# erikliland/pyMHT

Hardware: AMD Instinct MI355X
Metric: scans/sec at ~5k+ leaf hypotheses x 500 measurements (per-scan gate + cluster + ILP + N-scan prune) (higher is better)
Workload: dtype f64 state / f32 covariance (the reference's own mix); 1 GPU; BASELINE configs[2]: 500 targets, ~500 meas/scan, N-scan=5, P_d=0.9, eta2=5.99; one independent sector per GPU; targets=499, n_scan=5, ilps_branched=63, blp_dual_iters_max=8, pre_roll_scans=16

## Files before the change

pymht_amd/csrc/mht_blp.hip:

```cpp
#include "mht_kernels.h"
#include "mht_commit.h"
#include <stdlib.h>

namespace mht {

#ifndef MHT_BLP_THREADS
#define MHT_BLP_THREADS 256
#endif
constexpr int BLP_THREADS = MHT_BLP_THREADS;
constexpr int FUSED_K = 8;
constexpr double DINF = 1.0e300;
constexpr int BIG_MAXH = 2048, BIG_MAXR = 1024, BIG_MAXK = 256;

struct Red {
    double d[BLP_THREADS / 64];
    double q[BLP_THREADS / 64][4];
    int i[BLP_THREADS / 64];
};

template <int CTRL, int ROW_MASK> __device__ __forceinline__ double dpp_f64(double v) {
    int lo = __double2loint(v), hi = __double2hiint(v);
    lo = __builtin_amdgcn_update_dpp(0, lo, CTRL, ROW_MASK, 0xf, false);
    hi = __builtin_amdgcn_update_dpp(0, hi, CTRL, ROW_MASK, 0xf, false);
    return __hiloint2double(hi, lo);
}
__device__ __forceinline__ double wave_sum(double v) {
    v += dpp_f64<0x111, 0xf>(v);
    v += dpp_f64<0x112, 0xf>(v);
    v += dpp_f64<0x114, 0xf>(v);
    v += dpp_f64<0x118, 0xf>(v);
    v += dpp_f64<0x142, 0xa>(v);
    v += dpp_f64<0x143, 0xc>(v);
    return __hiloint2double(__builtin_amdgcn_readlane(__double2hiint(v), 63), __builtin_amdgcn_readlane(__double2loint(v), 63));
}

__device__ __forceinline__ double block_sum(double v, Red* r) {
    v = wave_sum(v);
    __syncthreads();
    if ((threadIdx.x & 63) == 0) r->d[threadIdx.x >> 6] = v;
    __syncthreads();
    double s = 0.0;
#pragma unroll
    for (int w = 0; w < BLP_THREADS / 64; ++w) s += r->d[w];
    return s;
}
__device__ __forceinline__ int block_or(int v, Red* r) {
    v = __any(v) ? 1 : 0;
    __syncthreads();
    if ((threadIdx.x & 63) == 0) r->i[threadIdx.x >> 6] = v;
    __syncthreads();
    int s = 0;
#pragma unroll
    for (int w = 0; w < BLP_THREADS / 64; ++w) s |= r->i[w];
    return s;
}
template <int CTRL, int ROW_MASK> __device__ __forceinline__ void dpp_min_value(double& v) {
    const int lo = __double2loint(v), hi = __double2hiint(v);
    const int nlo = __builtin_amdgcn_update_dpp(lo, lo, CTRL, ROW_MASK, 0xf, false);
    const int nhi = __builtin_amdgcn_update_dpp(hi, hi, CTRL, ROW_MASK, 0xf, false);
    v = fmin(v, __hiloint2double(nhi, nlo));
}
__device__ __forceinline__ double row16_min_value(double v) {
    dpp_min_value<0x111, 0xf>(v);
    dpp_min_value<0x112, 0xf>(v);
    dpp_min_value<0x114, 0xf>(v);
    dpp_min_value<0x118, 0xf>(v);
    return v;
}
__device__ __forceinline__ double wave_min_value(double v) {
    v = row16_min_value(v);
    dpp_min_value<0x142, 0xa>(v);
    dpp_min_value<0x143, 0xc>(v);
    return __hiloint2double(__builtin_amdgcn_readlane(__double2hiint(v), 63), __builtin_amdgcn_readlane(__double2loint(v), 63));
}
template <int CTRL, int ROW_MASK> __device__ __forceinline__ void dpp_min_pair(double& v, int& i) {
    const int lo = __double2loint(v), hi = __double2hiint(v);
    const int nlo = __builtin_amdgcn_update_dpp(lo, lo, CTRL, ROW_MASK, 0xf, false);
    const int nhi = __builtin_amdgcn_update_dpp(hi, hi, CTRL, ROW_MASK, 0xf, false);
    const int ni = __builtin_amdgcn_update_dpp(i, i, CTRL, ROW_MASK, 0xf, false);
    const double nv = __hiloint2double(nhi, nlo);
    if (ni >= 0 && (i < 0 || nv < v || (nv == v && ni < i))) { v = nv; i = ni; }
}
__device__ __forceinline__ void row16_min_pair(double& v, int& i) {
    dpp_min_pair<0x111, 0xf>(v, i);
    dpp_min_pair<0x112, 0xf>(v, i);
    dpp_min_pair<0x114, 0xf>(v, i);
    dpp_min_pair<0x118, 0xf>(v, i);
}
__device__ __forceinline__ void wave_min_pair(double& v, int& i) {
    row16_min_pair(v, i);
    dpp_min_pair<0x142, 0xa>(v, i);
    dpp_min_pair<0x143, 0xc>(v, i);
    const int hi = __builtin_amdgcn_readlane(__double2hiint(v), 63), lo = __builtin_amdgcn_readlane(__double2loint(v), 63);
    v = __hiloint2double(hi, lo);
    i = __builtin_amdgcn_readlane(i, 63);
}
__device__ __forceinline__ void block_min_pair(double& v, int& i, Red* r) {
    wave_min_pair(v, i);
    __syncthreads();
    if ((threadIdx.x & 63) == 0) { r->d[threadIdx.x >> 6] = v; r->i[threadIdx.x >> 6] = i; }
    __syncthreads();
    v = r->d[0];
    i = r->i[0];
#pragma unroll
    for (int w = 1; w < BLP_THREADS / 64; ++w) {
        const double ov = r->d[w];
        const int oi = r->i[w];
        if (oi >= 0 && (i < 0 || ov < v || (ov == v && oi < i))) { v = ov; i = oi; }
    }
}

#ifndef MHT_GS_CK
#define MHT_GS_CK 1
#endif
struct GStore {
    const BlpArgs* a; const int32_t* mem; const unsigned long long* uw; int UW, PD; size_t cap;
    double* pu; int32_t* pusage; int32_t* pmark;
    int32_t *best_h, *ub_sel, *ch, *lix; double *best_rc, *cst, *uus, *lrc, *rest, *mn;
    bool ck; const int32_t *cbL, *ceL;
    __device__ __forceinline__ int row(int m) const { return m; }
    __device__ __forceinline__ int col_begin(int k) const { return (MHT_GS_CK && ck) ? cbL[k] : a->tchild[mem[k]]; }
    __device__ __forceinline__ int col_end(int k) const { return (MHT_GS_CK && ck) ? ceL[k] : a->tcend[mem[k]]; }
    __device__ __forceinline__ double cost(int h) const { return a->cost[h]; }
    __device__ __forceinline__ int ent(int d, int h) const { return a->pds ? a->path[(size_t)h * a->pds + d] : a->path[(size_t)d * cap + h]; }
    __device__ __forceinline__ double& u(int m) const { return pu[row(m)]; }
    __device__ __forceinline__ int32_t& usage(int m) const { return pusage[row(m)]; }
    __device__ __forceinline__ int32_t& mark(int m) const { return pmark[row(m)]; }
    __device__ __forceinline__ int to_global(int h) const { return h; }
    static constexpr int FOR_ROWS_FLAT = 256;
    template <typename F> __device__ __forceinline__ void for_rows(F f) const {
        if (UW <= FOR_ROWS_FLAT) {
            for (int m = threadIdx.x; m < UW * 64; m += BLP_THREADS)
                if ((uw[m >> 6] >> (m & 63)) & 1ull) f(m);
            return;
        }
        for (int w = threadIdx.x; w < UW; w += BLP_THREADS) {
            unsigned long long bits = uw[w];
            while (bits) {
                const int m = w * 64 + __ffsll((long long)bits) - 1;
                bits &= bits - 1;
                f(m);
            }
        }
    }
};
struct EnumEnt;
struct LStore {
    double* costL; unsigned short* entL; double* uL; int32_t* usageL; int32_t* markL; int32_t* colb; int32_t* gbase;
    int32_t* gcolL;
    bool reduced;
    double* rcL; unsigned short* membL; unsigned long long* minkey;
    unsigned short* ordL;
    unsigned short* enumL;
    EnumEnt* xL;
    int nH, nR, PD, K;
    int32_t *best_h, *ub_sel, *ch, *lix; double *best_rc, *cst, *uus, *lrc, *rest, *mn;
    __device__ __forceinline__ int col_begin(int k) const { return colb[k]; }
    __device__ __forceinline__ int col_end(int k) const { return colb[k + 1]; }
    __device__ __forceinline__ double cost(int h) const { return costL[h]; }
    __device__ __forceinline__ int ent(int d, int h) const { const int e = entL[h * 8 + d]; return e == nR ? -1 : e; }
    __device__ __forceinline__ double& u(int m) const { return uL[m]; }
    __device__ __forceinline__ int32_t& usage(int m) const { return usageL[m]; }
    __device__ __forceinline__ int32_t& mark(int m) const { return markL[m]; }
    __device__ __forceinline__ int to_global(int h) const {
        if (reduced) return gcolL[h];
        int lo = 0, hi = K;
        while (hi - lo > 1) { const int mid = (lo + hi) >> 1; if (colb[mid] <= h) lo = mid; else hi = mid; }
        return gbase[lo] + (h - colb[lo]);
    }
    template <typename F> __device__ __forceinline__ void for_rows(F f) const {
        for (int m = threadIdx.x; m < nR; m += BLP_THREADS) f(m);
    }
};

#ifndef MHT_ROWS8
#define MHT_ROWS8 1
#endif
__device__ __forceinline__ void rows8(const GStore& s, int h, int (&e)[8]) {
    if (s.a->pds == 8) {
        const int4* p = reinterpret_cast<const int4*>(s.a->path + (size_t)h * 8);
        const int4 q0 = p[0], q1 = p[1];
        e[0] = q0.x; e[1] = q0.y; e[2] = q0.z; e[3] = q0.w; e[4] = q1.x; e[5] = q1.y; e[6] = q1.z; e[7] = q1.w;
    } else {
#pragma unroll
        for (int d = 0; d < 8; ++d) e[d] = (d < s.PD) ? s.ent(d, h) : -1;
    }
}
__device__ __forceinline__ double reduced_cost(const GStore& s, int h) {
    double rc = s.cost(h);
    if (s.PD <= 8 && MHT_ROWS8) {
        int e[8];
        rows8(s, h, e);
        double uv[8];
#pragma unroll
        for (int d = 0; d < 8; ++d) uv[d] = s.u(e[d] >= 0 ? e[d] : 0);
#pragma unroll
        for (int d = 0; d < 8; ++d) rc = (e[d] >= 0) ? rc + uv[d] : rc;
        return rc;
    }
    for (int d = 0; d < s.PD; ++d) {
        const int e = s.ent(d, h);
        if (e >= 0) rc += s.u(e);
    }
    return rc;
}
__device__ __forceinline__ bool compatible(const GStore& s, int h) {
    if (s.PD <= 8 && MHT_ROWS8) {
        int e[8];
        rows8(s, h, e);
        int bad = 0;
#pragma unroll
        for (int d = 0; d < 8; ++d) bad |= (e[d] >= 0) ? s.mark(e[d] >= 0 ? e[d] : 0) : 0;
        return bad == 0;
    }
    for (int d = 0; d < s.PD; ++d) {
        const int e = s.ent(d, h);
        if (e >= 0 && s.mark(e)) return false;
    }
    return true;
}
__device__ __forceinline__ void set_marks(const GStore& s, int h, int value) {
    if ((int)threadIdx.x < s.PD) {
        const int e = s.ent(threadIdx.x, h);
        if (e >= 0) s.mark(e) = value;
    }
    __threadfence_block();
    __syncthreads();
}
__device__ __forceinline__ double priced_part(const GStore& s, int h) {
    if ((int)threadIdx.x < s.PD) {
        const int e = s.ent(threadIdx.x, h);
        if (e >= 0) return s.u(e);
    }
    return 0.0;
}
__device__ __forceinline__ void add_usage(const GStore& s, int k, int d) {
    const int e = s.ent(d, s.best_h[k]);
    if (e >= 0) atomicAdd(&s.usage(e), 1);
}

struct Rows8 { unsigned short e[8]; };
__device__ __forceinline__ Rows8 rows_of(const LStore& s, int h) {
    const uint4 v = reinterpret_cast<const uint4*>(s.entL)[h];
    Rows8 r;
    r.e[0] = v.x & 0xffff; r.e[1] = v.x >> 16; r.e[2] = v.y & 0xffff; r.e[3] = v.y >> 16;
    r.e[4] = v.z & 0xffff; r.e[5] = v.z >> 16; r.e[6] = v.w & 0xffff; r.e[7] = v.w >> 16;
    return r;
}
__device__ __forceinline__ double reduced_cost(const LStore& s, int h) {
    const Rows8 r = rows_of(s, h);
    const double c = s.costL[h];
    const double u0 = s.uL[r.e[0]], u1 = s.uL[r.e[1]], u2 = s.uL[r.e[2]], u3 = s.uL[r.e[3]];
    const double u4 = s.uL[r.e[4]], u5 = s.uL[r.e[5]], u6 = s.uL[r.e[6]], u7 = s.uL[r.e[7]];
    return ((((((((c + u0) + u1) + u2) + u3) + u4) + u5) + u6) + u7);
}
__device__ __forceinline__ bool compatible(const LStore& s, int h) {
    const Rows8 r = rows_of(s, h);
    const int m = s.markL[r.e[0]] | s.markL[r.e[1]] | s.markL[r.e[2]] | s.markL[r.e[3]] | s.markL[r.e[4]] | s.markL[r.e[5]] |
                  s.markL[r.e[6]] | s.markL[r.e[7]];
    return m == 0;
}
__device__ __forceinline__ void set_marks(const LStore& s, int h, int value) {
    if (threadIdx.x < 8) {
// ... 597 lines not shown
                unsigned long long fsig = 0ull;
                while (i < he) {
                    const int idx = i + lane;
                    const bool valid = idx < he;
                    const EnumEnt en = xL[valid ? idx : he - 1];
                    const bool over = !valid || (arc + en.rc + tail > lim);
                    const bool feas = !over && !(en.sig & mask);
                    const unsigned long long mo = __ballot(over);
                    unsigned long long mf = __ballot(feas);
                    if (mo) mf &= (1ull << (__ffsll((long long)mo) - 1)) - 1ull;
                    if (mf) {
                        const int fl = __ffsll((long long)mf) - 1;
                        found = i + fl;
                        frc = __shfl(en.rc, fl);
                        fsig = __shfl(en.sig, fl);
                        break;
                    }
                    if (mo) break;
                    i += 64;
                }
                if (found >= 0) {
                    if (++nodes > ENUM_BUDGET) { if (lane == 0) *s_abort = 1; break; }
                    const double tot = acc + s.costL[s.ordL[found]];
                    if (lane == 0) s_pos[L * ENUM_W + wave] = found;
                    if (L == K - 1) {
                        record(tot, L);
                        i = found + 1;
                        continue;
                    }
                    mask |= fsig;
                    acc = tot;
                    arc = arc + frc;
                    ++L;
                    i = s.colb[s_order[L]];
                    continue;
                }
                --L;
                if (L < 1) break;
                i = s_pos[L * ENUM_W + wave] + 1;
                mask = f0.sig;
                acc = tot0;
                arc = f0.rc;
                for (int q = 1; q < L; ++q) {
                    const int pq = s_pos[q * ENUM_W + wave];
                    const EnumEnt en = xL[pq];
                    mask |= en.sig;
                    acc = acc + s.costL[s.ordL[pq]];
                    arc = arc + en.rc;
                }
            }
        }
        if (lane == 0) { s_bestc[wave] = best; s_nodes[wave] = nodes; }
    }
    __syncthreads();
    ok = ok && !*s_abort;
    if (ok) {
        int w = -1;
        for (int q = 0; q < ENUM_W; ++q) {
            if (!(s_bestc[q] < DINF)) continue;
            bool better = w < 0 || s_bestc[q] < s_bestc[w];
            if (!better && s_bestc[q] == s_bestc[w]) {
                int d = 0;
                for (int l = 0; l < K && d == 0; ++l) d = s_best[l * ENUM_W + q] - s_best[l * ENUM_W + w];
                better = d < 0;
            }
            if (better) w = q;
        }
        ok = w >= 0;
        if (ok) {
            for (int l = tid; l < K; l += BLP_THREADS) s.ub_sel[s_order[l]] = s_best[l * ENUM_W + w];
            int tn = 0;
            for (int q = 0; q < ENUM_W; ++q) tn += s_nodes[q];
            nodes_out = tn;
            ub_known = s_bestc[w];
        }
    }
    for (int m = tid; m < nR; m += BLP_THREADS) { s.usageL[m] = 0; s.markL[m] = 0; }
    __threadfence_block();
    __syncthreads();
    return ok;
}

constexpr int MHT_BLP_REDUCE = -2;
__device__ __forceinline__ bool reducible(const BlpArgs&, const LStore&, int, double, Red*) { return false; }
__device__ __forceinline__ bool reducible(const BlpArgs& a, const GStore& s, int K, double UB, Red* r) {
    if (a.force_hbm || a.no_reduce || K > a.cap_k || a.PD > 8 || !(UB < DINF)) return false;
    const int tid = threadIdx.x;
    compute_minimisers(s, K, r);
    double up = 0.0, rs = 0.0;
    s.for_rows([&](int m) { up += s.u(m); });
    for (int k = tid; k < K; k += BLP_THREADS) rs += s.best_rc[k];
    const double root = block_sum(rs, r) - block_sum(up, r);
    const double lim = UB + 1e-9 * fmax(1.0, fabs(UB));
    int total = 0;
    for (int k = 0; k < K; ++k) {
        const double thr = lim - root + s.best_rc[k];
        double c = 0.0;
        for (int h = s.col_begin(k) + tid; h < s.col_end(k); h += BLP_THREADS) c += (reduced_cost(s, h) <= thr) ? 1.0 : 0.0;
        const int ck = (int)block_sum(c, r);
        if (tid == 0) { s.mn[k] = thr; s.lix[k] = ck; }
        total += ck;
        if (total > a.cap_h) return false;
    }
    for (int k = 0; k < K; ++k) {
        const double thr = lim - root + s.best_rc[k];
        for (int h = s.col_begin(k) + tid; h < s.col_end(k); h += BLP_THREADS)
            if (reduced_cost(s, h) <= thr)
                for (int d = 0; d < s.PD; ++d) { const int e = s.ent(d, h); if (e >= 0) s.mark(e) = 1; }
    }
    __threadfence_block();
    __syncthreads();
    double nr = 0.0;
    s.for_rows([&](int m) { nr += s.mark(m) ? 1.0 : 0.0; s.mark(m) = 0; });
    const int rows = (int)block_sum(nr, r);
    __threadfence_block();
    __syncthreads();
    return rows < a.cap_r - 1;
}

struct Team {
    int q, W; unsigned long long* gub;
    int qg, Wg;
    __device__ Team(int q_, int W_, unsigned long long* g_) : q(q_), W(W_), gub(g_), qg(q_), Wg(W_) {}
    __device__ Team(int q_, int W_, unsigned long long* g_, int qg_, int Wg_) : q(q_), W(W_), gub(g_), qg(qg_), Wg(Wg_) {}
};
#ifndef MHT_TEAM_LEVEL
#define MHT_TEAM_LEVEL 5
#endif
constexpr int TEAM_LEVEL = MHT_TEAM_LEVEL;
#ifndef MHT_TEAM_LEVEL_HBM
#define MHT_TEAM_LEVEL_HBM 3
#endif
__device__ __forceinline__ constexpr int team_level(const LStore&) { return TEAM_LEVEL; }
__device__ __forceinline__ constexpr int team_level(const GStore&) { return MHT_TEAM_LEVEL_HBM; }
__device__ __forceinline__ unsigned team_hash(int c0, int c1) {
    unsigned h = (unsigned)c0 * 0x9E3779B1u ^ ((unsigned)c1 * 0x85EBCA6Bu + 0x7F4A7C15u);
    h ^= h >> 15; h *= 0x2C1B3C6Du; h ^= h >> 12;
    return h;
}
template <typename S> __device__ __forceinline__ void solve_core(const BlpArgs& a, const S& s, int K, Red* r, int& status, int& iters, int& nodes, unsigned long long* stamp,
                                                                 double& ub, const Team tm = Team(0, 1, nullptr)) {
    const int tid = threadIdx.x, lane = tid & 63, wave = tid >> 6;
    double& UB = ub;
    double best_LB = -DINF, theta = 1.0, utot = 0.0;
    int stall = 0;
    status = 0; iters = 0; nodes = 0;
    const int ca_rounds = coordinate_rounds(s, K);
    const int ca_end = a.max_iter < ca_rounds ? a.max_iter : ca_rounds;
    const int it_cap = bb_after_rounds(s, K) ? ca_end : a.max_iter;
    const int enum_after = (s.col_end(K - 1) - s.col_begin(0) > ENUM_WIDE) ? ENUM_AFTER_WIDE : ENUM_AFTER;
    const int enum_at = (ca_end > 0 && K >= 3 && K <= ENUM_MAXK) ? (ca_end < enum_after ? ca_end : enum_after) : -1;
    for (int it = 0; it <= it_cap; ++it) {
        iters = it;
        if (it == enum_at && !a.no_enum) {
            const unsigned long long e0 = wall_clock64();
            const bool solved = enumerate_small(s, K, r, nodes, stamp, UB);
            stamp[5] = wall_clock64() - e0;
            if (solved) { status = MHT_BLP_BRANCHED; return; }
        }
        if (it == ca_end && ca_end > 0 && !bb_after_rounds(s, K)) {
            s.for_rows([&](int m) { s.u(m) = 0.0; });
            __threadfence_block();
            __syncthreads();
        }
        if ((it == 24 || it == 64 || it == 128) && UB < DINF && reducible(a, s, K, UB, r)) { status = MHT_BLP_REDUCE; return; }
        compute_minimisers(s, K, r);
        if (it == 0) stamp[1] = wall_clock64();
        if (!usage_counted_by_minimisers(s, K)) {
            for (int idx = tid; idx < K * s.PD; idx += BLP_THREADS) {
                const int k = idx / s.PD, d = idx - k * s.PD;
                add_usage(s, k, d);
            }
            __threadfence_block();
            __syncthreads();
        }
        if (it == 0) stamp[2] = wall_clock64();
        const bool coord = it < ca_end;
        double nrm = 0.0, usum = 0.0, LB = 0.0;
        int conflict = 0, slack = 0;
        if (coord) {
            s.for_rows([&](int m) {
                const int us = s.usage(m);
                conflict |= (us >= 2);
                slack |= (s.u(m) > 0.0 && us == 0);
            });
            nominate(s, K);
            const int f = (__any(conflict) ? 1 : 0) | (__any(slack) ? 2 : 0);
            if (lane == 0) r->i[wave] = f;
            __threadfence_block();
            __syncthreads();
            int ff = 0;
#pragma unroll
            for (int w = 0; w < BLP_THREADS / 64; ++w) ff |= r->i[w];
            conflict = ff & 1;
            slack = (ff >> 1) & 1;
            if (it == 0) stamp[3] = wall_clock64();
            if (!conflict) {
                bool take = true;
                if (UB < DINF) {
                    double sc = 0.0;
                    for (int k = tid; k < K; k += BLP_THREADS) sc += s.cost(s.best_h[k]);
                    sc = block_sum(sc, r);
                    take = sc < UB;
                    if (take) UB = sc;
                }
                if (take)
                    for (int k = tid; k < K; k += BLP_THREADS) s.ub_sel[k] = s.best_h[k];
                __threadfence_block();
                __syncthreads();
            }
        } else {
            s.for_rows([&](int m) {
                const int us = s.usage(m);
                const double um = s.u(m);
                double g = (double)(us - 1);
                if (um <= 0.0 && g < 0.0) g = 0.0;
                nrm += g * g;
                usum += um;
                conflict |= (us >= 2);
                slack |= (um > 0.0 && us == 0);
            });
            double src = 0.0, sc = 0.0;
            for (int k = tid; k < K; k += BLP_THREADS) { src += s.best_rc[k]; sc += s.cost(s.best_h[k]); }
            {
                const double v0 = wave_sum(nrm), v1 = wave_sum(usum), v2 = wave_sum(src), v3 = wave_sum(sc);
                int f = (__any(conflict) ? 1 : 0) | (__any(slack) ? 2 : 0);
                __syncthreads();
                if (lane == 0) { r->q[wave][0] = v0; r->q[wave][1] = v1; r->q[wave][2] = v2; r->q[wave][3] = v3; r->i[wave] = f; }
                __syncthreads();
                nrm = 0.0; utot = 0.0; src = 0.0; sc = 0.0; f = 0;
#pragma unroll
                for (int w = 0; w < BLP_THREADS / 64; ++w) {
                    nrm += r->q[w][0]; utot += r->q[w][1]; src += r->q[w][2]; sc += r->q[w][3]; f |= r->i[w];
                }
                conflict = f & 1;
                slack = (f >> 1) & 1;
            }
            if (it == 0) stamp[3] = wall_clock64();
            LB = src - utot;
            if (!conflict && sc < UB) {
                UB = sc;
                for (int k = tid; k < K; k += BLP_THREADS) s.ub_sel[k] = s.best_h[k];
                __threadfence_block();
                __syncthreads();
            }
        }
        bool done = false;
        if (!conflict && !slack) { status = MHT_BLP_CERTIFIED; done = true; }
        if (!done && coord && it == 1 && K == 2 && enumerate_pair(s, r)) {
            status = MHT_BLP_CERTIFIED;
            break;
        }
        bool counters_reset = false;
        if (!done && coord) counters_reset = coordinate_step(s, K, conflict != 0, slack != 0);
        if (!done && !coord) {
            if (LB > best_LB + 1e-12) { best_LB = LB; stall = 0; }
            else if (++stall >= 10) { theta *= 0.5; stall = 0; }
            if (UB >= DINF || (conflict && (it % 4) == 0)) {
                const double g = greedy_dive(s, K, s.ch, r);
                if (g < UB) {
                    UB = g;
                    for (int k = tid; k < K; k += BLP_THREADS) s.ub_sel[k] = s.ch[k];
                    __threadfence_block();
                    __syncthreads();
                }
            }
            if (UB - best_LB <= 1e-12 * fmax(1.0, fabs(UB))) { status = MHT_BLP_CERTIFIED; done = true; }
            if (it == it_cap || nrm == 0.0) done = true;
            if (theta < 1.0 / 16.0) done = true;
        }
        if (done && status != 0 && scratch_is_private(s)) break;
        const double step = (done || coord) ? 0.0 : theta * fmax(UB - LB, 1e-6) / nrm;
        if (!counters_reset)
            s.for_rows([&](int m) {
                if (!done && !coord) {
                    const double um = s.u(m);
                    double g = (double)(s.usage(m) - 1);
                    if (um <= 0.0 && g < 0.0) g = 0.0;
                    s.u(m) = fmax(0.0, um + step * g);
                }
                s.usage(m) = 0;
                if (coord) s.mark(m) = 0;
            });
        __threadfence_block();
        __syncthreads();
        if (done) break;
    }
#ifdef MHT_BLP_TRACE
    if (tid == 0 && tm.q == 0) printf("[blp] dual phase: %d iterations, status %d, at %.2f ms\n", iters, status, 1e-5 * (double)(wall_clock64() - stamp[0]));
#endif
    if (status != 0) return;
    if (UB >= DINF) {
        UB = greedy_dive(s, K, s.ch, r);
        for (int k = tid; k < K; k += BLP_THREADS) s.ub_sel[k] = s.ch[k];
        __threadfence_block();
        __syncthreads();
    }
    if (reducible(a, s, K, UB, r)) { status = MHT_BLP_REDUCE; return; }
    int32_t* ord = reinterpret_cast<int32_t*>(s.best_rc);
    int32_t* bh = s.best_h;
    {
        compute_minimisers(s, K, r);
        if (!usage_counted_by_minimisers(s, K)) {
            for (int idx = tid; idx < K * s.PD; idx += BLP_THREADS) add_usage(s, idx / s.PD, idx % s.PD);
            __threadfence_block();
            __syncthreads();
        }
        for (int k = tid; k < K; k += BLP_THREADS) {
            int hot = 0;
            const int h = s.best_h[k];
            for (int d = 0; d < s.PD; ++d) {
                const int e = s.ent(d, h);
                if (e >= 0 && (s.usage(e) >= 2 || s.u(e) > 0.0)) ++hot;
            }
            s.lix[k] = hot;
        }
        __threadfence_block();
        __syncthreads();
        for (int k = tid; k < K; k += BLP_THREADS) {
            const int hk = s.lix[k];
            int rank = 0;
            for (int j = 0; j < K; ++j) { const int hj = s.lix[j]; rank += (hj > hk || (hj == hk && j < k)) ? 1 : 0; }
            ord[rank] = k;
        }
        s.for_rows([&](int m) { s.usage(m) = 0; });
        __threadfence_block();
        __syncthreads();
    }
    int slot = -1;
    if (a.bb_snap && a.bb_busy) {
        if (tid == 0) {
            int got = -1;
            for (int i = 0; i < BB_SLOTS && got < 0; ++i)
                if (atomicCAS(&a.bb_busy[i], 0, 1) == 0) got = i;
            r->i[0] = got;
        }
        __syncthreads();
        slot = r->i[0];
        __syncthreads();
    }
    double* snap = slot >= 0 ? a.bb_snap + (size_t)slot * BB_RE_LEVELS * a.bb_snap_rows : nullptr;
    if (tid == 0) s.cst[0] = 0.0;
    __threadfence_block();
    __syncthreads();
    int level = 0;
    bool enter = true;
#ifdef MHT_BLP_TRACE
    int tr_eval = 0, tr_upper = 0;
    unsigned long long tr_t[8] = {0, 0, 0, 0, 0, 0, 0, 0}, tr_q = 0, tr_n = wall_clock64();
#define TR_MARK(i) do { const unsigned long long _n = wall_clock64(); tr_t[i] += _n - tr_q; tr_q = _n; } while (0)
#else
#define TR_MARK(i) do {} while (0)
#endif
    status = MHT_BLP_BRANCHED;
    double own = UB;
    const bool team = tm.Wg > 1 && tm.gub != nullptr;
    if (team && tid == 0 && UB < DINF) atomicMin(tm.gub, enum_key(UB));
    while (true) {
        if (team && enter && level >= 1) {
            __syncthreads();
            if (tid == 0) r->q[0][0] = enum_val(__hip_atomic_load(tm.gub, __ATOMIC_RELAXED, __HIP_MEMORY_SCOPE_AGENT));
            __syncthreads();
            const double g = r->q[0][0];
            __syncthreads();
            if (g < UB) UB = g;
        }
        const double eps = 1e-12 * fmax(1.0, fabs(UB));
        if (enter) {
            if (++nodes > a.node_limit) { status = MHT_BLP_NODE_LIMIT; break; }
            if (a.time_limit > 0 && (nodes & 63) == 0 && block_or(wall_clock64() - stamp[0] > (unsigned long long)a.time_limit ? 1 : 0, r)) {
                status = MHT_BLP_NODE_LIMIT;
                break;
            }
            if (level == K) {
                if (s.cst[K] < UB - eps) {
                    UB = own = s.cst[K];
                    if (team && tid == 0) atomicMin(tm.gub, enum_key(UB));
                    for (int p = tid; p < K; p += BLP_THREADS) s.ub_sel[ord[p]] = s.ch[p];
                    __threadfence_block();
                    __syncthreads();
                }
// ... 106 lines not shown
                    const double step = step_on ? fmax(UB - lb, 1e-6) / nrm : 0.0;
                    s.for_rows([&](int m) {
                        if (redo) {
                            s.u(m) = sl[m];
                        } else if (!s.mark(m) && step_on) {
                            const double um = s.u(m);
                            double g = (double)(s.usage(m) - 1);
                            if (um <= 0.0 && g < 0.0) g = 0.0;
                            s.u(m) = fmax(0.0, um + step * g);
                        }
                        s.usage(m) = 0;
                    });
                    __threadfence_block();
                    __syncthreads();
                }
                TR_MARK(5);
#ifdef MHT_BLP_TRACE
                tr_n = wall_clock64();
#endif
                if (redo) { final_eval = true; continue; }
                if (stop || !step_on) break;
            }
            if (pruned) {
                if (level == 0) break;
                --level;
                set_marks(s, s.ch[level], 0);
                enter = false;
                continue;
            }
            if (tid == 0) { s.rest[level] = rs_all - s.mn[level]; s.uus[level] = usumU; s.lrc[level] = -DINF; s.lix[level] = -1; }
            __threadfence_block();
            __syncthreads();
            enter = false;
        } else if (snap && level + 1 < BB_RE_LEVELS) {
            const double* slr = snap + (size_t)level * a.bb_snap_rows;
            s.for_rows([&](int m) { s.u(m) = slr[m]; });
            __threadfence_block();
            __syncthreads();
        }
        double bv;
        int bi;
        argmin_member(s, ord[level], true, s.lrc[level], s.lix[level], bv, bi, r);
        if (bi < 0 || s.cst[level] + bv + s.rest[level] - s.uus[level] >= UB - eps) {
            if (level == 0) break;
            --level;
            set_marks(s, s.ch[level], 0);
            continue;
        }
        bool foreign = false;
        if (team && level == team_level(s)) {
            unsigned hsh = 0x9E3779B9u;
            for (int l = 0; l < team_level(s); ++l) hsh = team_hash((int)hsh, s.to_global(s.ch[l]));
            hsh = team_hash((int)hsh, s.to_global(bi));
            foreign = hsh % (unsigned)tm.Wg != (unsigned)tm.qg;
        }
        if (foreign) {
            __syncthreads();
            if (tid == 0) { s.lrc[level] = bv; s.lix[level] = bi; }
            __threadfence_block();
            __syncthreads();
            continue;
        }
        if (tid == 0) {
            s.lrc[level] = bv;
            s.lix[level] = bi;
            s.ch[level] = bi;
            s.cst[level + 1] = s.cst[level] + s.cost(bi);
        }
        set_marks(s, bi, 1);
        ++level;
        enter = true;
    }
#ifdef MHT_BLP_TRACE
    if (tid == 0 && team) printf("[blp] member %d of %d: %d nodes (%d at or above the deal-out level), %d evaluations, left at %.2f ms; us per evaluation: sweep %.1f sums %.1f usage %.1f rows %.1f keep %.1f step %.1f outside %.1f\n", tm.q, tm.W, nodes, tr_upper, tr_eval,
                                 1e-5 * (double)(wall_clock64() - stamp[0]), 1e-2 * tr_t[0] / tr_eval, 1e-2 * tr_t[1] / tr_eval, 1e-2 * tr_t[2] / tr_eval, 1e-2 * tr_t[3] / tr_eval,
                                 1e-2 * tr_t[4] / tr_eval, 1e-2 * tr_t[5] / tr_eval, 1e-2 * tr_t[6] / tr_eval);
#endif
    ub = own;
    for (int l = 0; l < level; ++l) set_marks(s, s.ch[l], 0);
    if (slot >= 0 && tid == 0) atomicExch(&a.bb_busy[slot], 0);
}

struct TgtPre { int j, rscan, rnode, id, lab, cb, ce; double rootc; uint8_t rootf; };
__device__ __forceinline__ TgtPre load_target(const BlpArgs& a, int t) {
    TgtPre p;
    const int dg = a.t_depth[t] + 1, w = a.t_window[t] & 0xff;
    p.j = dg > w ? dg - w : 0;
    p.rscan = a.t_root_scan[t]; p.rnode = a.t_root_node[t]; p.id = a.t_id[t]; p.lab = a.t_label[t];
    p.cb = a.tchild[t]; p.ce = a.tcend[t];
    p.rootc = a.t_root_cnllr[t]; p.rootf = a.t_root_f32[t];
    return p;
}
template <typename T> __device__ __forceinline__ const T* ring_ptr(const T* base0, size_t stride, int k) {
    return reinterpret_cast<const T*>(reinterpret_cast<const char*>(base0) + (size_t)k * stride);
}
constexpr int KEY_DEAD = -1, KEY_ALL = -2;
__device__ __forceinline__ void blp_publish(const BlpArgs& a, int t, int key, int j, int rf, int count, int first) {
    if (!a.rec0) return;
    asm volatile("s_waitcnt vmcnt(0)" ::: "memory");
    __hip_atomic_store(&a.rec0[t], tgt_rec(a.pub_scan, key != -1, rf, j, count, count > 0 ? first : 0), __ATOMIC_RELAXED, __HIP_MEMORY_SCOPE_AGENT);
}
__device__ __forceinline__ int finish_target(const BlpArgs& a, int t, int s, const TgtPre& p, bool store, int* rf_out = nullptr) {
    const int kc = a.kc;
    const double cn = a.cnllr[s];
    const uint8_t fl = a.flags[s];
    const int smeas = ring_ptr(a.ring0.meas, a.ring_stride, kc)[s];
    double sx[NX];
#pragma unroll
    for (int k = 0; k < NX; ++k) sx[k] = a.x[(size_t)k * a.cap + s];
    const double sx0 = sx[0], sx1 = sx[1];
    const int j = p.j;
    const int anc_l = a.apath[(size_t)s * a.pds + (j > 0 ? j - 1 : 0)];
    const int anc = (j > 0) ? anc_l : -1;
    const bool f32score = (fl & F_SCORE_F32) && p.rootf;
    const double score = f32score ? (double)((float)cn - (float)p.rootc) : cn - p.rootc;
    int status = 0;
    if (isfinite(a.radar_range)) {
        const double dx = sx0 - a.radar_x, dy = sx1 - a.radar_y;
        if (sqrt(dx * dx + dy * dy) > a.radar_range) status = 1;
    }
    if (!status) {
        const double per = f32score ? (double)((float)score / (float)(a.Nwin + 1)) : score / (double)(a.Nwin + 1);
        if (per > a.score_limit) status = 2;
        else if (cn > a.cnllr_limit) status = 3;
    }
    int rscan = p.rscan, rnode = p.rnode;
    const bool moved = status == 0 && j > 0;
    if (moved) { rscan += j; rnode = anc; }
    const int kr = rscan % a.R;
    const double* rx = ring_ptr(a.ring0.x, a.ring_stride, kr);
    const double rc_l = ring_ptr(a.ring0.cnllr, a.ring_stride, kr)[rnode];
    const uint8_t rf_l = ring_ptr(a.ring0.flags, a.ring_stride, kr)[rnode];
    double rxv[NX];
#pragma unroll
    for (int k = 0; k < NX; ++k) rxv[k] = rx[(size_t)k * a.cap + rnode];
    const int rmeas = ring_ptr(a.ring0.meas, a.ring_stride, kr)[rnode];
    const double rc = moved ? rc_l : p.rootc;
    const uint8_t rf = moved ? (uint8_t)((rf_l & F_SCORE_F32) ? 1 : 0) : p.rootf;
    if (store) {
        a.t_alive[t] = status;
        a.t_jdrop[t] = j;
        a.t_score[t] = score;
        a.w_root_scan[t] = rscan; a.w_root_node[t] = rnode; a.w_root_f32[t] = rf;
        if (a.rec0) __hip_atomic_store(reinterpret_cast<unsigned long long*>(&a.w_root_cnllr[t]), (unsigned long long)__double_as_longlong(rc), __ATOMIC_RELAXED, __HIP_MEMORY_SCOPE_AGENT);
        else a.w_root_cnllr[t] = rc;
        mht_target_report& r = a.rec[t];
        r.id = p.id;
        r.status = status;
        r.sel_node = s;
        r.sel_meas = smeas;
        r.root_scan = rscan;
        r.root_node = rnode;
#pragma unroll
        for (int k = 0; k < NX; ++k) r.sel_x[k] = sx[k];
        r.sel_cnllr = cn;
        r.score = score;
        r.root_cnllr = rc;
#pragma unroll
        for (int k = 0; k < NX; ++k) r.root_x[k] = rxv[k];
        r.root_meas = rmeas;
        r.cluster = p.lab;
    }
    if (rf_out) *rf_out = rf;
    return status ? KEY_DEAD : (j > 0 ? anc : KEY_ALL);
}

__device__ __forceinline__ int sweep_prefetch(const BlpArgs& a, int j, int cb, int ce, int lane) {
    return (j > 0 && cb + lane < ce) ? a.apath[(size_t)(cb + lane) * a.pds + (j - 1)] : -1;
}
__device__ __forceinline__ void sweep_survivors(const BlpArgs& a, int t, int j, int cb, int ce, int key, int va0, int lane, int rf = -1) {
    int count = 0, first = 0x7fffffff;
    if (key == KEY_ALL) {
        count = ce - cb;
        if (count > 0) first = cb;
    } else if (key != KEY_DEAD) {
        for (int c0 = cb; c0 < ce; c0 += 64) {
            const int c = c0 + lane;
            const int v = (c0 == cb) ? va0 : (c < ce ? a.apath[(size_t)c * a.pds + (j - 1)] : -1);
            const unsigned long long m = __ballot(c < ce && v == key);
            if (m && first == 0x7fffffff) first = c0 + __ffsll((long long)m) - 1;
            count += __popcll(m);
        }
    }
    if (lane == 0) {
        a.t_count[t] = count; a.t_firstsurv[t] = first;
        if (a.rec0) blp_publish(a, t, key, j, rf >= 0 ? rf : (int)a.w_root_f32[t], count, first);
    }
}

__device__ __forceinline__ void prune_members(const BlpArgs& a, const int32_t* mem, int K, const int32_t* key) {
    if (!a.t_alive) return;
    __threadfence_block();
    __syncthreads();
    const int lane = threadIdx.x & 63;
    for (int k = threadIdx.x >> 6; k < K; k += BLP_THREADS / 64) {
        const int t = mem[k];
        const int j = a.t_jdrop[t], cb = a.tchild[t], ce = a.tcend[t];
        sweep_survivors(a, t, j, cb, ce, key[k], sweep_prefetch(a, j, cb, ce, lane), lane);
    }
}

struct ClRef { int c, p0, K, root; };
__device__ __forceinline__ ClRef cl_ref(const BlpArgs& a, int c) { const int p0 = a.cl_ptr[c]; return ClRef{c, p0, a.cl_ptr[c + 1] - p0, -1}; }
__device__ __forceinline__ TgtPre load_target_cr(const BlpArgs& a, int t, const ClRef& cr) {
    TgtPre p = load_target(a, t);
    if (a.uf_epoch) p.lab = cr.root;
    return p;
}
__device__ __forceinline__ void solve_cluster(const BlpArgs& a, const ClRef cr, unsigned long long* uw, Red* r, unsigned char* lds,
                                              const Team tm = Team(0, 1, nullptr), const int team_idx = -1, const int my_t = -1, const TgtPre* pre_in = nullptr, const int dbg_bx = -1) {
    const int tid = threadIdx.x;
    const int c = cr.c;
    const int K = cr.K;
    const int32_t* mem = a.cl_members + cr.p0;
    const int slot = cr.p0 + c;
    const int UW = (a.n_mnodes + 63) >> 6;
    const unsigned long long t_begin = wall_clock64();
    const unsigned long long c_begin = clock64();
    TgtPre pre = {};
    const bool pre_ok = a.t_alive && K <= BLP_THREADS;
    if (pre_ok && tid < K) { if (pre_in && my_t >= 0) pre = *pre_in; else pre = load_target_cr(a, my_t >= 0 ? my_t : mem[tid], cr); }
    LStore s;
    unsigned char* q = lds;
    const int L_MAXH = a.cap_h, L_MAXR = a.cap_r, L_MAXK = a.cap_k, L_KPAD = a.cap_k + 4;
    int* s_wbase = reinterpret_cast<int*>(q); q += (size_t)a.cap_uw * 4;
    int* s_scal = reinterpret_cast<int*>(q); q += 16;
    int& s_nR = s_scal[0];
    int& s_nH = s_scal[1];
    s.entL = reinterpret_cast<unsigned short*>(q); q += (size_t)L_MAXH * 16;
    s.costL = reinterpret_cast<double*>(q); q += (size_t)L_MAXH * 8;
    s.rcL = reinterpret_cast<double*>(q); q += (size_t)L_MAXH * 8;
    s.uL = reinterpret_cast<double*>(q); q += (size_t)L_MAXR * 8;
    s.minkey = reinterpret_cast<unsigned long long*>(q); q += (size_t)L_KPAD * 8;
    s.best_rc = reinterpret_cast<double*>(q); q += (size_t)L_KPAD * 8;
    s.cst = reinterpret_cast<double*>(q); q += (size_t)L_KPAD * 8;
    s.uus = reinterpret_cast<double*>(q); q += (size_t)L_KPAD * 8;
    s.lrc = reinterpret_cast<double*>(q); q += (size_t)L_KPAD * 8;
    s.rest = reinterpret_cast<double*>(q); q += (size_t)L_KPAD * 8;
    s.mn = reinterpret_cast<double*>(q); q += (size_t)L_KPAD * 8;
    s.usageL = reinterpret_cast<int32_t*>(q); q += (size_t)L_MAXR * 4;
    s.markL = reinterpret_cast<int32_t*>(q); q += (size_t)L_MAXR * 4;
    s.colb = reinterpret_cast<int32_t*>(q); q += (size_t)L_KPAD * 4;
    s.gbase = reinterpret_cast<int32_t*>(q); q += (size_t)L_KPAD * 4;
    s.best_h = reinterpret_cast<int32_t*>(q); q += (size_t)L_KPAD * 4;
    s.ub_sel = reinterpret_cast<int32_t*>(q); q += (size_t)L_KPAD * 4;
    s.ch = reinterpret_cast<int32_t*>(q); q += (size_t)L_KPAD * 4;
    s.lix = reinterpret_cast<int32_t*>(q); q += (size_t)L_KPAD * 4;
    s.membL = reinterpret_cast<unsigned short*>(q); q += (size_t)L_MAXH * 2;
    s.ordL = reinterpret_cast<unsigned short*>(q); q += (size_t)L_MAXH * 2;
    s.enumL = reinterpret_cast<unsigned short*>(q); q += ENUM_LDS;
    s.xL = reinterpret_cast<EnumEnt*>(q); q += (size_t)L_MAXH * 16;
    s.gcolL = reinterpret_cast<int32_t*>(q); q += (size_t)L_MAXH * 4;
    s.reduced = false;
    const bool small_k = K <= L_MAXK;
    for (int w = tid; w < UW; w += BLP_THREADS) uw[w] = 0ull;
    if (small_k) {
        if (tid < 64) {
            int carry = 0;
            for (int base = 0; base < K; base += 64) {
                const int k = base + tid;
                int gb = 0, n = 0;
                if (k < K) {
                    if (pre_ok && K <= 64) { gb = pre.cb; n = pre.ce - gb; }
                    else { const int t = mem[k]; gb = a.tchild[t]; n = a.tcend[t] - gb; }
                }
                int incl = n;
#pragma unroll
                for (int o = 1; o < 64; o <<= 1) {
                    const int v = __shfl_up(incl, o);
                    if (tid >= o) incl += v;
                }
                if (k < K) { s.colb[k] = carry + incl - n; s.gbase[k] = gb; if (pre_ok && K <= 64) s.lix[k] = pre.j; }
                carry += __shfl(incl, 63);
            }
            if (tid == 0) { s.colb[K] = carry; s_nH = carry; }
        }
    } else if (tid == 0) {
        int acc = 0;
        for (int k = 0; k < K; ++k) acc += a.tcend[mem[k]] - a.tchild[mem[k]];
        s_nH = acc;
    }
    __syncthreads();
    const int nH = s_nH;
    if (a.tier == 1 && !(K <= a.t1_k && nH <= a.t1_h)) {
        if (tid == 0) a.big_list[atomicAdd(a.big_count, 1)] = c;
        __syncthreads();
        return;
    }
    const bool lds_cols = small_k && nH <= L_MAXH && a.PD <= 8 && !a.force_hbm;
    const bool anc_pf = lds_cols && pre_ok && K <= 64 && a.t_alive && a.pds == 8;
    s.nH = nH; s.PD = a.PD; s.K = K;
    if (lds_cols) {
        for (int h0 = tid; h0 < nH; h0 += 2 * BLP_THREADS) {
            int g[2], ev[2][8], jm[2], an[2];
            double cs[2];
#pragma unroll
            for (int q = 0; q < 2; ++q) {
                const int h = h0 + q * BLP_THREADS;
                g[q] = -1; jm[q] = 0;
                if (h < nH) {
                    int lo = 0, hi = K;
                    while (hi - lo > 1) { const int mid = (lo + hi) >> 1; if (s.colb[mid] <= h) lo = mid; else hi = mid; }
                    g[q] = s.gbase[lo] + (h - s.colb[lo]);
                    s.membL[h] = (unsigned short)lo;
                    if (anc_pf) jm[q] = s.lix[lo];
                }
            }
#pragma unroll
            for (int q = 0; q < 2; ++q) {
                const int gq = g[q] >= 0 ? g[q] : 0;
                cs[q] = a.cost[gq];
                an[q] = -1;
                if (anc_pf) an[q] = a.apath[(size_t)gq * 8 + (jm[q] > 0 ? jm[q] - 1 : 0)];
                if (a.pds) {
                    const int4* rec = reinterpret_cast<const int4*>(a.path + (size_t)gq * a.pds);
                    const int4 r0 = rec[0], r1 = rec[1];
                    const int rv[8] = {r0.x, r0.y, r0.z, r0.w, r1.x, r1.y, r1.z, r1.w};
#pragma unroll
                    for (int d = 0; d < 8; ++d) ev[q][d] = g[q] >= 0 ? rv[d] : -1;
                } else {
#pragma unroll
                    for (int d = 0; d < 8; ++d) {
                        const int v = (d < a.PD) ? a.path[(size_t)d * a.cap + gq] : -1;
                        ev[q][d] = g[q] >= 0 ? v : -1;
                    }
                }
            }
#pragma unroll
            for (int q = 0; q < 2; ++q) {
                const int h = h0 + q * BLP_THREADS;
                if (g[q] < 0) continue;
                s.costL[h] = cs[q];
                if (anc_pf) s.gcolL[h] = an[q];
#pragma unroll
                for (int d = 0; d < 8; ++d) {
                    s.entL[h * 8 + d] = (unsigned short)(ev[q][d] < 0 ? 0xffff : ev[q][d]);
                    if (ev[q][d] >= 0) atomicOr(&uw[ev[q][d] >> 6], 1ull << (ev[q][d] & 63));
                }
            }
        }
    } else {
        for (int k = 0; k < K; ++k) {
            const int t = mem[k];
            for (int d = 0; d < a.PD; ++d)
                for (int h = a.tchild[t] + tid; h < a.tcend[t]; h += BLP_THREADS) {
                    const int e = a.pds ? a.path[(size_t)h * a.pds + d] : a.path[(size_t)d * a.cap + h];
                    if (e >= 0) atomicOr(&uw[e >> 6], 1ull << (e & 63));
                }
        }
    }
    auto row_prefix = [&]() {
        __syncthreads();
        if (tid < 64) {
            int carry = 0;
            for (int base = 0; base < UW; base += 64) {
                const int w = base + tid;
                const int pc = (w < UW) ? __popcll(uw[w]) : 0;
                int incl = pc;
#pragma unroll
                for (int o = 1; o < 64; o <<= 1) {
                    const int v = __shfl_up(incl, o);
                    if (tid >= o) incl += v;
                }
                if (w < UW) s_wbase[w] = carry + incl - pc;
                carry += __shfl(incl, 63);
            }
            if (tid == 0) s_nR = carry;
        }
        __syncthreads();
    };
    row_prefix();
    int nR = s_nR;
    int status, iters, nodes;
    unsigned long long stamp[6] = {t_begin, 0, 0, 0, 0, 0};
    const unsigned long long t_setup = wall_clock64();
    bool use_lds = lds_cols && nR < L_MAXR;
    bool team = tm.Wg > 1 && use_lds;
    const bool team_hbm = tm.Wg > 1 && !use_lds && a.tm_sm > 0 && K <= TEAM_SEL;
    if (tm.q > 0 && !team && !team_hbm) return;
    const int32_t* final_sel = nullptr;
    int nHl = nH;
    double ub_reduced = DINF;
    double best_io = DINF;
    auto team_file = [&](const Team& tmm, int tidx, int Kk, auto sel_of, double ubv, int& st_io, int& it_io, int& nd_io, const int32_t*& fsel) -> bool {
        TeamResult* res = a.team_res + (size_t)tidx * TEAM_W;
        TeamResult& me = res[tmm.q];
        for (int k = tid; k < Kk; k += BLP_THREADS) me.sel[k] = sel_of(k);
        if (tid == 0) { me.ub = ubv; me.status = st_io; me.nodes = nd_io; me.iters = it_io; }
        __threadfence();
        __syncthreads();
        if (tid == 0) r->i[0] = atomicAdd(&a.team_state[tidx].done, 1);
        __syncthreads();
        const int before = r->i[0];
        __syncthreads();
        if (before != tmm.W - 1) return false;
        __threadfence();
        if (tid == 0) {
            int bq = 0, any_limit = 0, nsum = 0, itmax = 0;
            double bub = DINF;
            for (int q = 0; q < tmm.W; ++q) {
                const double u = __longlong_as_double((long long)__hip_atomic_load(reinterpret_cast<unsigned long long*>(&res[q].ub), __ATOMIC_RELAXED, __HIP_MEMORY_SCOPE_AGENT));
                const int st = __hip_atomic_load(&res[q].status, __ATOMIC_RELAXED, __HIP_MEMORY_SCOPE_AGENT);
                nsum += __hip_atomic_load(&res[q].nodes, __ATOMIC_RELAXED, __HIP_MEMORY_SCOPE_AGENT);
                const int itq = __hip_atomic_load(&res[q].iters, __ATOMIC_RELAXED, __HIP_MEMORY_SCOPE_AGENT);
                itmax = itq > itmax ? itq : itmax;
                any_limit |= (st == MHT_BLP_NODE_LIMIT);
                if (u < bub) { bub = u; bq = q; }
            }
            r->i[0] = bq; r->i[1] = any_limit; r->i[2] = nsum; r->i[3] = itmax; r->d[0] = bub;
        }
        __syncthreads();
        fsel = res[r->i[0]].sel;
        best_io = r->d[0];
        st_io = r->i[1] ? MHT_BLP_NODE_LIMIT : MHT_BLP_BRANCHED;
        nd_io = r->i[2];
        it_io = r->i[3];
        __syncthreads();
        return true;
    };
    const bool xteam = tm.Wg != tm.W && a.shard_team != nullptr && team_idx >= 0 && K <= TEAM_SEL;
    auto xteam_out = [&](auto sel_of, double value) {
        int32_t* o = a.shard_team + ((size_t)a.shard_i * TEAM_MAX + team_idx) * XT_WORDS;
        for (int k = tid; k < K; k += BLP_THREADS) { const int h = sel_of(k); a.sel[mem[k]] = h; o[4 + k] = h - a.tchild[mem[k]]; }
        if (tid == 0) {
            const unsigned long long key = enum_key(value);
            o[0] = (int32_t)(key >> 42); o[1] = (int32_t)((key >> 21) & 0x1fffffu); o[2] = (int32_t)(key & 0x1fffffu); o[3] = K;
        }
    };
    if (!use_lds) {
        GStore gs;
        gs.a = &a; gs.mem = mem; gs.uw = uw; gs.UW = UW; gs.PD = a.PD; gs.cap = (size_t)a.cap;
        const size_t om = team_hbm ? (size_t)tm.q * a.tm_sm : 0, os = (team_hbm ? (size_t)tm.q * a.tm_ss : 0) + (size_t)slot;
        gs.pu = a.u + om; gs.pusage = a.usage + om; gs.pmark = a.mark + om;
        gs.ck = small_k;
        gs.cbL = s.gbase; gs.ceL = s.lix;
        if (gs.ck) {
            for (int k = tid; k < K; k += BLP_THREADS) s.lix[k] = s.gbase[k] + (s.colb[k + 1] - s.colb[k]);
            __syncthreads();
        }
        gs.best_h = a.best_h + os; gs.best_rc = a.best_rc + os; gs.ub_sel = a.bb_best + os; gs.ch = a.bb_ch + os;
        gs.cst = a.bb_cost + os; gs.uus = a.bb_uused + os; gs.lrc = a.bb_last_rc + os; gs.lix = a.bb_last_idx + os;
        gs.rest = a.bb_rest + os; gs.mn = a.bb_min + os;
        gs.for_rows([&](int m) { gs.u(m) = 0.0; gs.usage(m) = 0; gs.mark(m) = 0; });
        __threadfence_block();
        __syncthreads();
        double ub = DINF;
        solve_core(a, gs, K, r, status, iters, nodes, stamp, ub, team_hbm ? tm : Team(0, 1, nullptr));
        ub_reduced = ub;
#ifdef MHT_BLP_TRACE
        if (tid == 0) printf("[blp] cluster %d K=%d nH=%d: HBM phase status %d iters %d nodes %d, %.2f ms (setup %.2f)\n", c, K, nH, status, iters, nodes,
                             1e-5 * (double)(wall_clock64() - t_begin), 1e-5 * (double)(t_setup - t_begin));
#endif
        if (status == MHT_BLP_REDUCE) {
            gs.ck = false;
            if (tid == 0) {
                int acc = 0;
                for (int k = 0; k < K; ++k) { s.colb[k] = acc; acc += gs.lix[k]; }
                s.colb[K] = acc;
                s_nH = acc;
            }
            for (int w = tid; w < UW; w += BLP_THREADS) uw[w] = 0ull;
            __syncthreads();
            nHl = s_nH;
            const int lane = tid & 63, wave = tid >> 6;
            for (int k = 0; k < K; ++k) {
                const double thr = gs.mn[k];
                int run = 0;
                for (int base = gs.col_begin(k); base < gs.col_end(k); base += BLP_THREADS) {
                    const int h = base + tid;
                    const bool keep = h < gs.col_end(k) && reduced_cost(gs, h) <= thr;
                    const unsigned long long bal = __ballot(keep);
                    if (lane == 0) r->i[wave] = __popcll(bal);
                    __syncthreads();
                    int off = run;
                    for (int w = 0; w < wave; ++w) off += r->i[w];
                    int tot = 0;
                    for (int w = 0; w < BLP_THREADS / 64; ++w) tot += r->i[w];
                    if (keep) {
                        const int pos = s.colb[k] + off + __popcll(bal & ((1ull << lane) - 1ull));
                        s.gcolL[pos] = h;
                        if (h == gs.ub_sel[k]) s.ub_sel[k] = pos;
                        s.membL[pos] = (unsigned short)k;
                        s.costL[pos] = a.cost[h];
                        for (int d = 0; d < 8; ++d) {
                            const int e = d < a.PD ? gs.ent(d, h) : -1;
                            s.entL[pos * 8 + d] = (unsigned short)(e < 0 ? 0xffff : e);
                            if (e >= 0) atomicOr(&uw[e >> 6], 1ull << (e & 63));
                        }
                    }
                    run += tot;
                    __syncthreads();
                }
            }
            row_prefix();
            nR = s_nR;
            s.reduced = true;
            s.nH = nHl;
            use_lds = true;
            team = team_hbm;
        } else {
            if (team_hbm && status == MHT_BLP_CERTIFIED) {
                if (tm.q > 0) return;
            } else if (team_hbm) {
                if (!team_file(tm, team_idx, K, [&](int k) { return gs.ub_sel[k]; }, ub, status, iters, nodes, final_sel)) return;
            }
            stamp[4] = wall_clock64();
            if (xteam) {
                xteam_out([&](int k) { return final_sel ? __hip_atomic_load(const_cast<int32_t*>(final_sel) + k, __ATOMIC_RELAXED, __HIP_MEMORY_SCOPE_AGENT) : gs.ub_sel[k]; },
                          final_sel ? best_io : ub);
            } else
            for (int k = tid; k < K; k += BLP_THREADS) {
                const int h = final_sel ? __hip_atomic_load(const_cast<int32_t*>(final_sel) + k, __ATOMIC_RELAXED, __HIP_MEMORY_SCOPE_AGENT) : gs.ub_sel[k];
                a.sel[mem[k]] = h;
                if (a.sel_rel) a.sel_rel[mem[k]] = h - a.tchild[mem[k]];
                if (a.t_alive) gs.ch[k] = finish_target(a, mem[k], h, pre_ok ? pre : load_target_cr(a, mem[k], cr), true);
            }
            if (!xteam) prune_members(a, mem, K, gs.ch);
        }
    }
    if (use_lds) {
        s.nR = nR;
        for (int m = tid; m <= nR; m += BLP_THREADS) { s.uL[m] = 0.0; s.usageL[m] = 0; s.markL[m] = 0; }
        for (int h = tid; h < nHl; h += BLP_THREADS) {
            const Rows8 g8 = rows_of(s, h);
            unsigned o[8];
#pragma unroll
            for (int d = 0; d < 8; ++d) {
                const unsigned e = g8.e[d];
                o[d] = (e == 0xffffu) ? (unsigned)nR
                                      : (unsigned)(s_wbase[e >> 6] + __popcll(uw[e >> 6] & ((1ull << (e & 63)) - 1ull)));
            }
            reinterpret_cast<uint4*>(s.entL)[h] = make_uint4(o[0] | (o[1] << 16), o[2] | (o[3] << 16), o[4] | (o[5] << 16), o[6] | (o[7] << 16));
        }
        __syncthreads();
        double ub = s.reduced ? ub_reduced : DINF;
#ifdef MHT_BLP_TRACE
        if (tid == 0 && s.reduced) printf("[blp] cluster %d: rebuilt with %d columns %d rows at %.2f ms\n", c, nHl, nR, 1e-5 * (double)(wall_clock64() - t_begin));
#endif
        solve_core(a, s, K, r, status, iters, nodes, stamp, ub, team ? tm : Team(0, 1, nullptr));
#ifdef MHT_BLP_TRACE
        if (tid == 0 && s.reduced) printf("[blp] cluster %d: LDS phase status %d iters %d nodes %d at %.2f ms\n", c, status, iters, nodes, 1e-5 * (double)(wall_clock64() - t_begin));
#endif
        if (team && status == MHT_BLP_CERTIFIED) {
            if (tm.q > 0) return;
        } else if (team) {
            if (!team_file(tm, team_idx, K, [&](int k) { return s.to_global(s.ub_sel[k]); }, ub, status, iters, nodes, final_sel)) return;
        }
        stamp[4] = wall_clock64();
        int rf_mine = -1;
        if (xteam) {
            xteam_out([&](int k) { return final_sel ? __hip_atomic_load(const_cast<int32_t*>(final_sel) + k, __ATOMIC_RELAXED, __HIP_MEMORY_SCOPE_AGENT) : s.to_global(s.ub_sel[k]); },
                      final_sel ? best_io : ub);
        } else
        for (int k = tid; k < K; k += BLP_THREADS) {
            const int h = final_sel ? __hip_atomic_load(const_cast<int32_t*>(final_sel) + k, __ATOMIC_RELAXED, __HIP_MEMORY_SCOPE_AGENT) : s.to_global(s.ub_sel[k]);
            a.sel[mem[k]] = h;
            if (a.sel_rel) a.sel_rel[mem[k]] = h - a.tchild[mem[k]];
            if (a.t_alive) {
                const TgtPre q = pre_ok ? pre : load_target_cr(a, mem[k], cr);
                s.ch[k] = finish_target(a, mem[k], h, q, true, &rf_mine);
                s.ub_sel[k] = q.j;
                s.lix[k] = 0;
                s.best_h[k] = 0x7fffffff;
            }
        }
        if (a.t_alive && s.reduced) {
            __syncthreads();
            prune_members(a, mem, K, s.ch);
        } else if (a.t_alive) {
            __syncthreads();
            for (int h = tid; h < nH; h += BLP_THREADS) {
                const int m = s.membL[h];
                const int key = s.ch[m];
                if (key == KEY_DEAD) continue;
                const int g = s.gbase[m] + (h - s.colb[m]);
                const bool sv = key == KEY_ALL || (anc_pf ? s.gcolL[h] : a.apath[(size_t)g * a.pds + (s.ub_sel[m] - 1)]) == key;
                if (sv) { atomicAdd(&s.lix[m], 1); atomicMin(&s.best_h[m], g); }
            }
            __syncthreads();
            for (int k = tid; k < K; k += BLP_THREADS) {
                a.t_count[mem[k]] = s.lix[k];
                a.t_firstsurv[mem[k]] = s.best_h[k];
                blp_publish(a, mem[k], s.ch[k], s.ub_sel[k], rf_mine, s.lix[k], s.best_h[k]);
            }
        }
    }
    if (tid == 0 && a.dbg && dbg_bx >= 0 && dbg_bx < 3900 && tm.q == 0) {
        unsigned long long* g = a.dbg + 32 + (size_t)dbg_bx * 16;
        g[8] = t_begin; g[9] = t_setup; g[10] = stamp[4]; g[11] = wall_clock64();
    }
    if (tid == 0) {
        a.cl_status[c] = status;
        a.cl_iters[c] = iters;
        a.cl_nodes[c] = nodes;
        if (a.cl_time) {
            a.cl_time[8 * c] = (int)(t_setup - t_begin);
            a.cl_time[8 * c + 1] = (int)(wall_clock64() - t_begin);
            for (int q = 1; q <= 4; ++q) a.cl_time[8 * c + 1 + q] = (int)(stamp[q] - t_begin);
            a.cl_time[8 * c + 6] = (int)(clock64() - c_begin);
            a.cl_time[8 * c + 7] = (int)stamp[5];
        }
    }
    __threadfence_block();
    __syncthreads();
}

constexpr size_t RED_SLOT = BLP_THREADS <= 512 ? 512 : 1024;
static_assert(sizeof(Red) <= RED_SLOT, "Red must fit its LDS slot");
static size_t blp_lds_bytes(int cap_h, int cap_r, int cap_k, int cap_uw) {
    const size_t kpad = (size_t)cap_k + 4;
    return (size_t)cap_uw * 8 + RED_SLOT + (size_t)cap_uw * 4 + 16 + (size_t)cap_h * 16 + (size_t)cap_h * 8 * 2 + (size_t)cap_r * 8 + 7 * kpad * 8 +
           2 * (size_t)cap_r * 4 + 6 * kpad * 4 + (size_t)cap_h * 2 * 2 + ENUM_LDS + (size_t)cap_h * 16 + (size_t)cap_h * 4;
}

struct UfPersist {
    int nT, nC, nMulti, nSingle, nTeam, my_t, pad[2];
    ClRef own[4];
    ClRef team[TEAM_MAX];
    unsigned short single[BLP_THREADS / 64][8];
};
constexpr size_t BLP_UF_PERSIST = (sizeof(UfPersist) + 15) & ~(size_t)15;
constexpr int UF_SPEC = 4;
__host__ __device__ constexpr size_t uf_prologue_bytes(size_t T) { return ((T + 7) & ~(size_t)7) * 18 + 256; }

struct UfFetch { int s_over, nT; unsigned long long nif; unsigned long long pw[UF_SPEC]; };
struct UfHead { const DevStatus* status; const int32_t* nT_dev; const unsigned long long* ni_flag; const unsigned long long* uf_parent; int uf_cap, uf_ovl; };
__device__ __forceinline__ UfFetch uf_prefetch(const UfHead& a) {
    UfFetch f;
    int z;
    asm volatile("v_mov_b32 %0, 0" : "=v"(z));
    const int32_t* sp = a.status ? &a.status->overflow : a.nT_dev;
    const int so = sp[z];
    f.nT = a.nT_dev[z];
    const unsigned long long nif = (a.uf_ovl ? a.ni_flag : a.uf_parent)[z];
#pragma unroll
    for (int q = 0; q < UF_SPEC; ++q) {
        const int t = (int)threadIdx.x + q * BLP_THREADS;
        f.pw[q] = a.uf_parent[((t < a.uf_cap) ? t : 0) + z];
    }
    f.s_over = a.status ? so : 0;
    f.nif = a.uf_ovl ? nif : 0ull;
    return f;
}
__device__ __forceinline__ bool uf_prologue(const BlpArgs& a, const UfFetch& fe, unsigned char* lds, UfPersist* ps, const int bx, const int gx, int& my_t_out, TgtPre& pre_out) {
    const int tid = threadIdx.x, lane = tid & 63, wave = tid >> 6;
#define UF_STAMP(k) do { if (a.dbg && tid == 0 && bx < 3900) a.dbg[32 + (size_t)bx * 16 + (k)] = wall_clock64(); } while (0)
    UF_STAMP(0);
    const int s_over = __builtin_amdgcn_readfirstlane(fe.s_over);
    const int nT = __builtin_amdgcn_readfirstlane(fe.nT);
    const unsigned long long nif = ((unsigned long long)(unsigned)__builtin_amdgcn_readfirstlane((int)(fe.nif >> 32)) << 32) | (unsigned)__builtin_amdgcn_readfirstlane((int)fe.nif);
    const unsigned epoch = (a.uf_ovl && (unsigned)nif == (a.uf_epoch >> 1) - 1u && ((nif >> 32) & 1ull)) ? (a.uf_epoch | 1u) : a.uf_epoch;
    unsigned long long pw[UF_SPEC];
#pragma unroll
    for (int q = 0; q < UF_SPEC; ++q) pw[q] = fe.pw[q];
    if (s_over) return false;
    const int Tp = (nT + 7) & ~7;
    unsigned short* par = reinterpret_cast<unsigned short*>(lds);
    unsigned short* lab = par + Tp;
    unsigned short* hp = lab + Tp;
    unsigned short* tmp = hp + Tp;
    unsigned short* ms = tmp + Tp;
    unsigned short* ml = ms + Tp;
    unsigned short* sl = ml + Tp / 2;
    int* cnt = reinterpret_cast<int*>(sl + Tp);
    unsigned long long* s_w = reinterpret_cast<unsigned long long*>(cnt + Tp);
    int* s_tl = reinterpret_cast<int*>(s_w + 8);
#pragma unroll
    for (int q = 0; q < UF_SPEC; ++q) {
        const int t = tid + q * BLP_THREADS;
        if (t < nT) { par[t] = (unsigned short)(((unsigned)(pw[q] >> 32) == epoch) ? 0xffffffffu - (unsigned)pw[q] : (unsigned)t); cnt[t] = 0; }
    }
    for (int t = tid + UF_SPEC * BLP_THREADS; t < nT; t += BLP_THREADS) {
        const unsigned long long w = a.uf_parent[t];
        par[t] = (unsigned short)(((unsigned)(w >> 32) == epoch) ? 0xffffffffu - (unsigned)w : (unsigned)t);
        cnt[t] = 0;
    }
    __syncthreads();
    UF_STAMP(1);
    for (int t = tid; t < nT; t += BLP_THREADS) {
        int r = t, p = par[r];
        while (p != r) { r = p; p = par[r]; }
        lab[t] = (unsigned short)r;
        atomicAdd(&cnt[r], 1);
    }
    __syncthreads();
    UF_STAMP(2);
    const int E = (nT + BLP_THREADS - 1) / BLP_THREADS;
    auto pack_of = [&](int t) -> unsigned long long {
        if (t >= nT || lab[t] != t) return 0ull;
        const unsigned long long K = (unsigned long long)cnt[t];
        return 1ull | ((K >= 2 ? 1ull : 0ull) << 14) | ((K == 1 ? 1ull : 0ull) << 27) | (K << 41) | ((K >= (unsigned long long)TEAM_MIN_K ? 1ull : 0ull) << 55);
    };
    unsigned long long mine = 0ull;
    for (int e = 0; e < E; ++e) mine += pack_of(tid * E + e);
    unsigned long long incl = mine;
#pragma unroll
    for (int o = 1; o < 64; o <<= 1) {
        const unsigned long long v = __shfl_up(incl, o);
        if (lane >= o) incl += v;
    }
    if (lane == 63) s_w[wave] = incl;
    __syncthreads();
    UF_STAMP(3);
    unsigned long long run = incl - mine, total = 0ull;
#pragma unroll
    for (int w = 0; w < BLP_THREADS / 64; ++w) { const unsigned long long v = s_w[w]; if (w < wave) run += v; total += v; }
    const int nC = (int)(total & 0x3fffu), nMulti = (int)((total >> 14) & 0x1fffu), nSingle = (int)((total >> 27) & 0x3fffu);
    const int nTeamAll = (int)(total >> 55), nTeam = (a.team_list && nTeamAll > 0) ? (nTeamAll < TEAM_MAX ? nTeamAll : TEAM_MAX) : 0;
    for (int e = 0; e < E; ++e) {
        const int t = tid * E + e;
        const unsigned long long pk = pack_of(t);
        if (pk) {
            const int c = (int)(run & 0x3fffu), mr = (int)((run >> 14) & 0x1fffu), sr = (int)((run >> 27) & 0x3fffu), p0 = (int)((run >> 41) & 0x3fffu), tr = (int)(run >> 55);
            const int K = cnt[t];
            par[t] = (unsigned short)c;
            hp[t] = (unsigned short)p0;
            if (K >= 2) ml[mr] = (unsigned short)t; else sl[sr] = (unsigned short)t;
            if (K >= TEAM_MIN_K && tr < TEAM_MAX) s_tl[tr] = t;
            run += pk;
        }
    }
    __syncthreads();
    UF_STAMP(4);
    const int writer = nMulti < gx - 1 ? nMulti : gx - 1;
    const int own_root = bx < nMulti ? (int)ml[bx] : 0;
    const int own_K = bx < nMulti ? (cnt[own_root] & 0xffff) : 0;
    const bool full = bx == writer || nTeam > 0 || bx + gx < nMulti || own_K > 64;
    auto ref_of = [&](int h) { return ClRef{(int)par[h], (int)hp[h], cnt[h] & 0xffff, h}; };
    int32_t* gmem = const_cast<int32_t*>(a.cl_members);
    if (tid == 0) { ps->nT = nT; ps->nC = nC; ps->nMulti = nMulti; ps->nSingle = nSingle; ps->nTeam = nTeam; ps->my_t = -1; }
    if (tid >= 64 && tid < 64 + BLP_THREADS / 64 * 8) {
        const int w = (tid - 64) >> 3, j = (tid - 64) & 7;
        const int i = (gx - 1 - bx) * (BLP_THREADS / 64) + w + j * gx * (BLP_THREADS / 64);
        ps->single[w][j] = (i < nSingle) ? sl[i] : (unsigned short)0xffff;
    }
    int my_t = -1;
    if (full) {
        for (int t = tid; t < nT; t += BLP_THREADS) {
            const int h = lab[t];
            const int K = cnt[h] & 0xffff;
            if (K == 1) ms[hp[h]] = (unsigned short)t;
            else tmp[hp[h] + (atomicAdd(&cnt[h], 1 << 16) >> 16)] = (unsigned short)t;
        }
        __syncthreads();
        UF_STAMP(5);
        for (int t = tid; t < nT; t += BLP_THREADS) {
            const int h = lab[t];
            const int K = cnt[h] & 0xffff, base = hp[h];
            if (K == 1) continue;
            int rank = 0;
            for (int i = 0; i < K; ++i) rank += (tmp[base + i] < t) ? 1 : 0;
            ms[base + rank] = (unsigned short)t;
        }
        __syncthreads();
        UF_STAMP(6);
        for (int q = 0; q < 4; ++q) {
            const int i = bx + q * gx;
            if (i >= nMulti) break;
            const ClRef cr = ref_of(ml[i]);
            if (tid == 0) ps->own[q] = cr;
            for (int k = tid; k < cr.K; k += BLP_THREADS) gmem[cr.p0 + k] = ms[cr.p0 + k];
        }
        for (int q = 0; q < nTeam; ++q) {
            const ClRef cr = ref_of(s_tl[q]);
            if (tid == 0) ps->team[q] = cr;
            if (bx >= nMulti) for (int k = tid; k < cr.K; k += BLP_THREADS) gmem[cr.p0 + k] = ms[cr.p0 + k];
        }
        if (bx == writer) {
            int32_t* t_label = const_cast<int32_t*>(a.t_label);
            int32_t* cl_ptr = const_cast<int32_t*>(a.cl_ptr);
            int32_t* multi = const_cast<int32_t*>(a.multi_list);
            int32_t* single = const_cast<int32_t*>(a.single_list);
            int32_t* counts = const_cast<int32_t*>(a.counts);
            for (int t = tid; t < nT; t += BLP_THREADS) {
                const int h = lab[t];
                t_label[t] = h;
                if (a.t_cluster) a.t_cluster[t] = par[h];
                gmem[t] = ms[t];
                if (h == t) cl_ptr[par[h]] = hp[h];
            }
            for (int i = tid; i < nMulti; i += BLP_THREADS) multi[i] = par[ml[i]];
            for (int i = tid; i < nSingle; i += BLP_THREADS) single[i] = sl[i];
            if (a.team_list && tid < nTeam) const_cast<int32_t*>(a.team_list)[tid] = par[s_tl[tid]];
            if (tid == 0) {
                cl_ptr[nC] = nT;
                counts[0] = nC; counts[1] = nMulti; counts[2] = nSingle; counts[3] = 0; counts[4] = 0; counts[5] = nTeam;
            }
            if (a.rec0) for (int t = nT + tid; t < a.pub_ub; t += BLP_THREADS) __hip_atomic_store(&a.rec0[t], tgt_rec(a.pub_scan, 0, 0, 0, 0, 0), __ATOMIC_RELAXED, __HIP_MEMORY_SCOPE_AGENT);
            if (a.alloc_reset && tid >= 64 && tid < 64 + FG_REGIONS) a.alloc_reset[(tid - 64) * 32] = 0u;
        }
        if (bx < nMulti && tid < own_K) my_t = ms[hp[own_root] + tid];
    } else if (wave == 0 && bx < nMulti) {
        const int p0 = hp[own_root];
        int n = 0;
        for (int t0 = 0; t0 < nT && n < own_K; t0 += 64) {
            const int t = t0 + lane;
            const bool m = t < nT && lab[t] == own_root;
            const unsigned long long bal = __ballot(m);
            if (m) ms[p0 + n + __popcll(bal & ((1ull << lane) - 1ull))] = (unsigned short)t;
            n += __popcll(bal);
        }
        __builtin_amdgcn_fence(__ATOMIC_ACQ_REL, "wavefront");
        __builtin_amdgcn_wave_barrier();
        if (lane == 0) ps->own[0] = ref_of(own_root);
        if (lane < own_K) { my_t = ms[p0 + lane]; gmem[p0 + lane] = my_t; }
    }
    if (my_t >= 0) { pre_out = load_target(a, my_t); pre_out.lab = own_root; }
    __threadfence_block();
    __syncthreads();
    UF_STAMP(7);
    my_t_out = my_t;
    return true;
}

template <bool UF> __device__ __forceinline__ void blp_singles(const BlpArgs& a, const int bx, const int gx, const int nSingle, const UfPersist* ps = nullptr);
__device__ __forceinline__ void blp_stamp_begin(const BlpArgs& a, int bx);
template <bool UF = false>
__device__ __forceinline__ void blp_body(const BlpArgs& a, unsigned char* lds, const int bx, const int gx, UfPersist* ps = nullptr, const UfFetch* fe = nullptr) {
    unsigned long long* uw = reinterpret_cast<unsigned long long*>(lds);
    Red* red = reinterpret_cast<Red*>(lds + (size_t)a.cap_uw * 8);
    if (!UF && a.dbg && threadIdx.x == 0 && bx < 3900) a.dbg[32 + (size_t)bx * 16 + 12] = wall_clock64();
    if (!UF && a.status && a.status->overflow) return;
    const bool rest = !UF && a.tier == 2;
    const int32_t* work = rest ? a.big_list : a.multi_list;
    int nMulti = UF ? 0 : (rest ? *a.big_count : a.counts[1]), nSingle = UF ? 0 : (rest ? 0 : a.counts[2]);
    int my_t = -1;
    TgtPre my_pre_v = {};
    const TgtPre* my_pre = UF ? &my_pre_v : nullptr;
    const bool xteams = a.shard_n > 1 && a.shard_team != nullptr;
    bool teams_on = a.team_list && a.tier != 1 && (xteams || (a.shard_n <= 1 && gx > nMulti));
    int nTeam = teams_on ? (UF ? 0 : a.counts[5]) : 0;
    int nIdle = gx - nMulti;
    auto team_W = [&](int ti) { const int w = nIdle > ti ? 1 + (nIdle - ti + nTeam - 1) / nTeam : 1; return w < TEAM_W ? w : TEAM_W; };
    int own_i = bx, own_q = 0;
    for (int stage = UF ? -1 : 0; stage < 3; ) {
        ClRef cr = ClRef{-1, 0, 0, -1};
        int ti = -1, mt = -1;
        Team tm = Team(0, 1, nullptr);
        if (UF && stage == -1) {
            stage = 0;
            if (!uf_prologue(a, *fe, lds, ps, bx, gx, my_t, my_pre_v)) return;
            blp_stamp_begin(a, bx);
            if (a.dbg && threadIdx.x == 0 && bx < 3900) a.dbg[32 + (size_t)bx * 16 + 12] = wall_clock64();
            nMulti = ps->nMulti; nSingle = ps->nSingle;
            teams_on = a.team_list && a.tier != 1 && (xteams || (a.shard_n <= 1 && gx > nMulti));
            nTeam = teams_on ? ps->nTeam : 0;
            nIdle = gx - nMulti;
            continue;
        } else if (stage == 0) {
            if (own_i >= nMulti) { stage = 1; continue; }
            if (UF) { cr = ps->own[own_q]; mt = own_q == 0 ? my_t : -1; ++own_q; }
            else cr = cl_ref(a, work[own_i]);
            own_i += gx;
            if (nTeam > 0 && cr.K >= TEAM_MIN_K)
                for (int q = 0; q < nTeam; ++q) if ((UF ? ps->team[q].c : a.team_list[q]) == cr.c) ti = q;
            const bool xt = xteams && ti >= 0 && cr.K <= TEAM_SEL;
            if (a.shard_n > 1 && !xt && (a.cl_owner ? a.cl_owner[cr.c] : cr.c % a.shard_n) != a.shard_i) continue;
            if (xt) tm = Team(0, team_W(ti), &a.team_state[ti].gub, a.shard_i, team_W(ti) * a.shard_n);
            else if (ti >= 0 && team_W(ti) > 1) tm = Team(0, team_W(ti), &a.team_state[ti].gub);
            else ti = -1;
        } else if (stage == 1) {
            stage = 2;
            blp_singles<UF>(a, bx, gx, nSingle, ps);
            continue;
        } else {
            stage = 3;
            if (!(nTeam > 0 && bx >= nMulti)) break;
            const int j = bx - nMulti, q = 1 + j / nTeam;
            ti = j % nTeam;
            if (q >= team_W(ti)) break;
            __syncthreads();
            cr = UF ? ps->team[ti] : cl_ref(a, a.team_list[ti]);
            tm = (xteams && cr.K <= TEAM_SEL) ? Team(q, team_W(ti), &a.team_state[ti].gub, q * a.shard_n + a.shard_i, team_W(ti) * a.shard_n) : Team(q, team_W(ti), &a.team_state[ti].gub);
        }
        if (a.dbg && threadIdx.x == 0 && bx < 3900 && stage == 0) a.dbg[32 + (size_t)bx * 16 + 13] = wall_clock64();
        solve_cluster(a, cr, uw, red, lds + (size_t)a.cap_uw * 8 + RED_SLOT, tm, ti, mt, mt >= 0 ? my_pre : nullptr, bx);
    }
}

template <bool UF>
__device__ __forceinline__ void blp_singles(const BlpArgs& a, const int bx, const int gx, const int nSingle, const UfPersist* ps) {
    const int lane = threadIdx.x & 63;
    const int gw = (gx - 1 - bx) * (BLP_THREADS / 64) + (threadIdx.x >> 6);
    int j = 0;
    for (int i = gw; i < nSingle; i += gx * (BLP_THREADS / 64), ++j) {
        const int t = UF ? (int)ps->single[threadIdx.x >> 6][j & 7] : a.single_list[i];
        if (a.shard_n > 1 && t % a.shard_n != a.shard_i) continue;
        TgtPre pre = {};
        int cb, ce;
        if (a.t_alive) { pre = load_target(a, t); if (UF) pre.lab = t; cb = pre.cb; ce = pre.ce; }
        else { cb = a.tchild[t]; ce = a.tcend[t]; }
        double bv = DINF;
        int bi = -1;
        for (int h = cb + lane; h < ce; h += 64) {
            const double v = a.cnllr[h];
            if (a.skip_dead && (a.flags[h] & F_DEAD)) continue;
            if (bi < 0 || v <= bv) { bv = v; bi = h; }
        }
        const int va0 = a.t_alive ? sweep_prefetch(a, pre.j, cb, ce, lane) : -1;
#pragma unroll
        for (int o = 32; o > 0; o >>= 1) {
            const double ov = __shfl_xor(bv, o);
            const int oi = __shfl_xor(bi, o);
            if (oi >= 0 && (bi < 0 || ov < bv || (ov == bv && oi > bi))) { bv = ov; bi = oi; }
        }
        if (lane == 0) { a.sel[t] = bi; if (a.sel_rel) a.sel_rel[t] = bi - cb; }
        if (a.t_alive) {
            int rf = 0;
            const int key = finish_target(a, t, bi, pre, lane == 0, &rf);
            sweep_survivors(a, t, pre.j, cb, ce, key, va0, lane, rf);
        }
    }
}

constexpr int LIGHT_MAXK = 8;
__device__ __forceinline__ void blp_light(const BlpArgs& a, const int bx, const int gx, const int nMulti) {
    const int lane = threadIdx.x & 63;
    const int gw = bx * (BLP_THREADS / 64) + (threadIdx.x >> 6), nw = gx * (BLP_THREADS / 64);
    for (int i = gw; i < nMulti; i += nw) {
        const int c = a.multi_list[i];
        const int p0 = a.cl_ptr[c], K = a.cl_ptr[c + 1] - p0;
        if (K > LIGHT_MAXK || a.pds != 8 || a.force_hbm) {
            if (lane == 0) a.big_list[atomicAdd(a.big_count, 1)] = c;
            continue;
        }
        const int tk = a.cl_members[p0 + (lane < K ? lane : 0)];
        const TgtPre pre = load_target(a, tk);
        double v[LIGHT_MAXK];
        int cbk[LIGHT_MAXK], cek[LIGHT_MAXK];
#pragma unroll
        for (int k = 0; k < LIGHT_MAXK; ++k) {
            cbk[k] = __shfl(pre.cb, k < K ? k : 0);
            cek[k] = __shfl(pre.ce, k < K ? k : 0);
            const int h = cbk[k] + lane;
            v[k] = a.cost[(k < K && h < cek[k]) ? h : cbk[0]];
        }
        int best = -1;
#pragma unroll
        for (int k = 0; k < LIGHT_MAXK; ++k) {
            if (k >= K) break;
            const int h0 = cbk[k] + lane;
            double bv = (h0 < cek[k]) ? v[k] : DINF;
            int bi = (h0 < cek[k]) ? h0 : -1;
            for (int h = h0 + 64; h < cek[k]; h += 64) {
                const double w = a.cost[h];
                if (bi < 0 || w < bv) { bv = w; bi = h; }
            }
#pragma unroll
            for (int o = 32; o > 0; o >>= 1) {
                const double ov = __shfl_xor(bv, o);
                const int oi = __shfl_xor(bi, o);
                if (oi >= 0 && (bi < 0 || ov < bv || (ov == bv && oi < bi))) { bv = ov; bi = oi; }
            }
            if (lane == k) best = bi;
        }
        const int mk = lane >> 3;
        const int hk = __shfl(best, mk < K ? mk : 0);
        int e = -1;
        if (mk < K && hk >= 0) e = a.path[(size_t)hk * 8 + (lane & 7)];
        int va[LIGHT_MAXK];
#pragma unroll
        for (int k = 0; k < LIGHT_MAXK; ++k) {
            const int jk = __shfl(pre.j, k < K ? k : 0);
            va[k] = (k < K) ? sweep_prefetch(a, jk, cbk[k], cek[k], lane) : -1;
        }
        bool clash = false;
        for (int q = 0; q < K * 8; ++q) {
            const int eq = __shfl(e, q);
            clash = clash || (eq >= 0 && eq == e && (q >> 3) != mk);
        }
        if (__any(clash) || __any(lane < K && best < 0)) {
            if (lane == 0) a.big_list[atomicAdd(a.big_count, 1)] = c;
            continue;
        }
        int key = KEY_DEAD;
        if (lane < K) {
            a.sel[tk] = best;
            if (a.sel_rel) a.sel_rel[tk] = best - pre.cb;
            key = finish_target(a, tk, best, pre, true);
        }
#pragma unroll
        for (int k = 0; k < LIGHT_MAXK; ++k) {
            if (k >= K) break;
            sweep_survivors(a, __shfl(tk, k), __shfl(pre.j, k), cbk[k], cek[k], __shfl(key, k), va[k], lane);
        }
        if (lane == 0) { a.cl_status[c] = MHT_BLP_CERTIFIED; a.cl_iters[c] = 0; a.cl_nodes[c] = 0; }
    }
}

__device__ __forceinline__ void blp_stamp_begin(const BlpArgs& a, int bx) {
    if (a.status && bx == 0 && threadIdx.x == 0) {
        DevStatus* st = const_cast<DevStatus*>(a.status);
        if (st->t[2] == 0) st->t[2] = wall_clock64();
    }
}
__device__ __forceinline__ void blp_stamp_end(const BlpArgs& a) {
    if (a.status && threadIdx.x == 0) atomicMax(&const_cast<DevStatus*>(a.status)->t[4], (unsigned long long)wall_clock64());
}

__global__ __launch_bounds__(BLP_THREADS) void blp_kernel(const BlpArgs a) {
    extern __shared__ __attribute__((aligned(16))) unsigned char lds[];
    if (a.dbg && threadIdx.x == 0 && blockIdx.x < 3900) a.dbg[32 + (size_t)blockIdx.x * 16] = wall_clock64();
    blp_stamp_begin(a, blockIdx.x);
    blp_body(a, lds, blockIdx.x, gridDim.x);
    blp_stamp_end(a);
    if (a.dbg && threadIdx.x == 0 && blockIdx.x < 3900) a.dbg[32 + (size_t)blockIdx.x * 16 + 15] = wall_clock64();
}
__global__ __launch_bounds__(BLP_THREADS) void blp_uf_kernel(const BlpArgs a_in) {
    extern __shared__ __attribute__((aligned(16))) unsigned char lds[];
    const UfFetch fe = uf_prefetch(UfHead{a_in.status, a_in.nT_dev, a_in.ni_flag, a_in.uf_parent, a_in.uf_cap, a_in.uf_ovl});
    typedef const __attribute__((address_space(4))) BlpArgs* KArgP;
    KArgP kp = (KArgP)__builtin_amdgcn_kernarg_segment_ptr();
    asm volatile("" : "+s"(kp) : : "memory");
    BlpArgs a;
    __builtin_memcpy(&a, kp, sizeof(BlpArgs));
    UfPersist* ps = reinterpret_cast<UfPersist*>(lds + a.uf_lds_off);
    if (a.status && blockIdx.x == 0 && threadIdx.x == 0) const_cast<DevStatus*>(a.status)->t[1] = wall_clock64();
    if (a.begun && blockIdx.x == 0 && threadIdx.x == 0) __hip_atomic_store(a.begun, (unsigned long long)a.pub_scan, __ATOMIC_RELAXED, __HIP_MEMORY_SCOPE_AGENT);
    const int gx = (int)gridDim.x, pb = (int)blockIdx.x, bx = pb;
    blp_body<true>(a, lds, bx, gx, ps, &fe);
    if (!fe.s_over) blp_stamp_end(a);
    if (a.blp_done) {
        __syncthreads();
        if (threadIdx.x == 0) {
            __builtin_amdgcn_fence(__ATOMIC_RELEASE, "agent");
            asm volatile("s_waitcnt vmcnt(0)" ::: "memory");
            atomicAdd(a.blp_done, 1ull);
        }
    }
    if (a.dbg && threadIdx.x == 0 && bx < 3900) { a.dbg[32 + (size_t)bx * 16 + 15] = wall_clock64(); a.dbg[32 + (size_t)bx * 16 + 14] = ((unsigned long long)pb << 8) | (unsigned long long)(__builtin_amdgcn_s_getreg((3 << 11) | 20) & 7); }
}
__global__ __launch_bounds__(BLP_THREADS) void blp_batch_kernel(const PBatch av) {
    extern __shared__ __attribute__((aligned(16))) unsigned char lds[];
    BlpArgs a;
    const int n = gridDim.y, lin = blockIdx.y * gridDim.x + blockIdx.x;
    const int sector = lin % n, bx = lin / n;
    load_args(a, static_cast<const BlpArgs*>(av.p[sector]));
    blp_stamp_begin(a, bx);
    blp_body(a, lds, bx, gridDim.x);
    blp_stamp_end(a);
}

__global__ __launch_bounds__(BLP_THREADS) void blp_light_batch_kernel(const PBatch av) {
    BlpArgs a;
    const int n = gridDim.y, lin = blockIdx.y * gridDim.x + blockIdx.x;
    const int sector = lin % n, bx = lin / n;
    load_args(a, static_cast<const BlpArgs*>(av.p[sector]));
    blp_stamp_begin(a, bx);
    if (!(a.status && a.status->overflow)) {
        blp_light(a, bx, gridDim.x, a.counts[1]);
        blp_singles<false>(a, bx, gridDim.x, a.counts[2]);
    }
    blp_stamp_end(a);
}
int launch_blp_light_batch(mht_ctx* ctx, const PBatch& av, int n_sectors, int grid_x) {
    return launch_kernel(ctx, K_BLP_LIGHT_BATCH, blp_light_batch_kernel, dim3(grid_x, n_sectors), dim3(BLP_THREADS), 0, false, av);
}

__global__ __launch_bounds__(TEAM_SEL) void shard_team_resolve_kernel(const BlpArgs a, const int shard_n) {
    if (a.status && a.status->overflow) return;
    const int ti = blockIdx.x;
    if (ti >= a.counts[5]) return;
    const ClRef cr = cl_ref(a, a.team_list[ti]);
    int best = -1;
    unsigned long long bk = ~0ull;
    for (int d = 0; d < shard_n; ++d) {
        const int32_t* o = a.shard_team + ((size_t)d * TEAM_MAX + ti) * XT_WORDS;
        if (o[3] != cr.K) continue;
        const unsigned long long key = ((unsigned long long)(unsigned)o[0] << 42) | ((unsigned long long)(unsigned)o[1] << 21) | (unsigned long long)(unsigned)o[2];
        if (best < 0 || key < bk) { best = d; bk = key; }
    }
    if (best < 0) return;
    const int32_t* o = a.shard_team + ((size_t)best * TEAM_MAX + ti) * XT_WORDS;
    for (int k = threadIdx.x; k < cr.K; k += blockDim.x) a.sel_rel[a.cl_members[cr.p0 + k]] = o[4 + k];
}

int launch_shard_team_resolve(mht_ctx* ctx, const BlpArgs& a, int shard_n) {
    hipLaunchKernelGGL(shard_team_resolve_kernel, dim3(TEAM_MAX), dim3(TEAM_SEL), 0, ctx->stream, a, shard_n);
    MHT_HIP_CHECK(hipGetLastError());
    return MHT_OK;
}

__global__ __launch_bounds__(BLP_THREADS) void blp_epilogue_kernel(const BlpArgs a, const int32_t* nT_dev) {
    if (a.status && a.status->overflow) return;
    const int nT = *nT_dev, lane = threadIdx.x & 63;
    for (int t = blockIdx.x * (BLP_THREADS / 64) + (threadIdx.x >> 6); t < nT; t += gridDim.x * (BLP_THREADS / 64)) {
        const TgtPre pre = load_target(a, t);
        const int s = pre.cb + a.sel_rel[t];
        if (lane == 0) a.sel[t] = s;
        const int va0 = sweep_prefetch(a, pre.j, pre.cb, pre.ce, lane);
        const int key = finish_target(a, t, s, pre, lane == 0);
        sweep_survivors(a, t, pre.j, pre.cb, pre.ce, key, va0, lane);
    }
    blp_stamp_end(a);
}

int launch_blp_epilogue(mht_ctx* ctx, const BlpArgs& a, const int32_t* nT_dev, int n_targets_ub) {
    int grid = (n_targets_ub + BLP_THREADS / 64 - 1) / (BLP_THREADS / 64);
    if (grid < 1) grid = 1;
    hipLaunchKernelGGL(blp_epilogue_kernel, dim3(grid), dim3(BLP_THREADS), 0, ctx->stream, a, nT_dev);
    MHT_HIP_CHECK(hipGetLastError());
    return MHT_OK;
}

int launch_blp_batch(mht_ctx* ctx, const PBatch& av, int n_sectors, int grid_x, size_t lds) {
    return launch_kernel(ctx, K_BLP_BATCH, blp_batch_kernel, dim3(grid_x, n_sectors), dim3(BLP_THREADS), lds, false, av);
}

static size_t blp_set_tier_bytes(const BlpArgs& a) { return blp_lds_bytes(a.cap_h, a.cap_r, a.cap_k, a.cap_uw); }
size_t blp_set_tier(BlpArgs& a, int tier) {
    const int uw = (((a.n_mnodes + 63) / 64) + 1) & ~1;
    a.tier = tier;
    a.t1_h = 512; a.t1_k = 16;
    if (tier == 1) { a.cap_h = a.t1_h; a.cap_r = 256; a.cap_k = a.t1_k; }
    else { a.cap_h = BIG_MAXH; a.cap_r = BIG_MAXR; a.cap_k = BIG_MAXK; }
    if (tier == 0) {
        static int eh = -1, er = 0, ek = 0;
        if (eh < 0) { const char* e = getenv("MHT_BLP_CAPS"); eh = 0; if (e) sscanf(e, "%d,%d,%d", &eh, &er, &ek); }
        if (eh > 0) { a.cap_h = eh; a.cap_r = er; a.cap_k = ek; }
    }
    a.cap_uw = uw;
    return blp_lds_bytes(a.cap_h, a.cap_r, a.cap_k, a.cap_uw);
}

bool blp_uf_fits(int Tcap, int n_mnodes) {
    BlpArgs b = {};
    b.n_mnodes = n_mnodes;
    const size_t lds = blp_set_tier(b, 0), pro = uf_prologue_bytes((size_t)Tcap);
    return Tcap <= 8192 && (((lds > pro ? lds : pro) + 15) & ~(size_t)15) + BLP_UF_PERSIST <= 158 * 1024;
}

int launch_blp(mht_ctx* ctx, const BlpArgs& a, int grid) {
    BlpArgs b = a;
    const size_t lds = blp_set_tier(b, 0);
    if (lds > 158 * 1024) {
        set_error("blp: %d measurement nodes do not fit the solver's LDS tables", a.n_mnodes);
        return MHT_E_CAPACITY;
    }
    if (b.uf_epoch) {
        size_t body = lds > uf_prologue_bytes((size_t)b.uf_cap) ? lds : uf_prologue_bytes((size_t)b.uf_cap);
        body = (body + 15) & ~(size_t)15;
        b.uf_lds_off = (unsigned)body;
        const size_t lds_uf = body + BLP_UF_PERSIST;
        if (lds_uf > 158 * 1024) {
            set_error("blp: the union-find prologue of %d targets does not fit the launch's LDS (%zu bytes)", b.uf_cap, lds_uf);
            return MHT_E_CAPACITY;
        }
        return launch_kernel(ctx, K_BLP_UF, blp_uf_kernel, dim3(grid), dim3(BLP_THREADS), lds_uf, false, b);
    }
    return launch_kernel(ctx, K_BLP, blp_kernel, dim3(grid), dim3(BLP_THREADS), lds, false, b);
}

__global__ void blp_objective_kernel(const int32_t* sel, const double* cost, int nT, const int32_t* st, const int32_t* it,
                                     const int32_t* nd, double* out) {
    if (threadIdx.x || blockIdx.x) return;
    double s = 0.0;
    for (int t = 0; t < nT; ++t) s += cost[sel[t]];
    out[0] = s;
    out[1] = (double)st[0];
    out[2] = (double)it[0];
    out[3] = (double)nd[0];
}
}

using namespace mht;

extern "C" int mht_solve_blp(mht_ctx* ctx, int32_t nHyp, int32_t nT, int32_t nRows, int32_t depth, const int32_t* group_ptr,
                             const int32_t* rows, const double* cost, int32_t max_iter, int32_t node_limit,
                             int32_t* selected, double* objective, int32_t* status, int32_t* iterations, int32_t* nodes) {
    MHT_REQUIRE(ctx && group_ptr && cost && selected, "mht_solve_blp: null argument");
    MHT_REQUIRE(nT >= 1 && nHyp >= nT && nRows >= 0 && depth >= 0 && depth <= MAXPD, "mht_solve_blp: bad sizes");
    MHT_REQUIRE(rows || depth == 0, "mht_solve_blp: rows is null");
    MHT_HIP_CHECK(hipSetDevice(ctx->device));
    bool seam_team = nT >= TEAM_MIN_K && nT <= TEAM_SEL;
    { const char* e = getenv("MHT_BLP_NO_TEAMS"); if (e && e[0] == '1') seam_team = false; }
    const size_t W1 = seam_team ? (size_t)TEAM_W : 1;
    const size_t S1 = (size_t)2 * nT + 2, nR1 = (size_t)(nRows > 0 ? nRows : 1);
    const size_t S = S1 * W1;
    const size_t nR = nR1 * W1;
    const size_t snap_rows = nR1 > (size_t)BIG_MAXR ? nR1 : (size_t)BIG_MAXR;
    const size_t n_d = nR + 6 * S + 4 + (size_t)BB_SLOTS * BB_RE_LEVELS * snap_rows;
    const size_t n_i = 2 * nR + 4 * S + 2 + nT + 2 + 8 + 3 + BB_SLOTS;
    int rc = ctx->hitmask.ensure(n_d * 8 + n_i * 4 + 64);
    if (rc) return rc;
    double* d = static_cast<double*>(ctx->hitmask.ptr);
    int32_t* q = reinterpret_cast<int32_t*>(d + n_d);
    MHT_HIP_CHECK(hipMemsetAsync(ctx->hitmask.ptr, 0, n_d * 8 + n_i * 4, ctx->stream));
    BlpArgs a = {};
    a.u = d; a.best_rc = d + nR; a.bb_cost = a.best_rc + S; a.bb_uused = a.bb_cost + S; a.bb_last_rc = a.bb_uused + S;
    a.bb_rest = a.bb_last_rc + S; a.bb_min = a.bb_rest + S;
    double* out = a.bb_min + S;
    a.bb_snap = out + 4; a.bb_snap_rows = (int)snap_rows;
    a.usage = q; a.mark = q + nR; a.best_h = a.mark + nR; a.bb_ch = a.best_h + S; a.bb_best = a.bb_ch + S; a.bb_last_idx = a.bb_best + S;
    int32_t* cl_ptr = a.bb_last_idx + S;
    int32_t* members = cl_ptr + 2;
    int32_t* multi = members + nT;
    int32_t* single = multi + 1;
    int32_t* counts = single + 1;
    int32_t* st = counts + 8;
    a.cl_ptr = cl_ptr; a.cl_members = members; a.multi_list = multi; a.single_list = single; a.counts = counts;
    a.cl_status = st; a.cl_iters = st + 1; a.cl_nodes = st + 2;
    a.bb_busy = st + 3;
    a.tchild = group_ptr; a.tcend = group_ptr + 1; a.cost = cost; a.cnllr = cost; a.path = rows; a.cap = nHyp; a.PD = depth; a.n_mnodes = (int)nR1;
    if (seam_team) { a.tm_sm = nR1; a.tm_ss = S1; }
    a.sel = selected;
    a.max_iter = max_iter < 0 ? 200 : max_iter;
    { const char* e = getenv("MHT_BLP_NO_ENUM"); a.no_enum = (e && e[0] == '1') ? 1 : 0; }
    { const char* e = getenv("MHT_BLP_NO_REDUCE"); a.no_reduce = (e && e[0] == '1') ? 1 : 0; }
    a.node_limit = node_limit <= 0 ? (1 << 20) : node_limit;
    { const char* e = getenv("MHT_BLP_TIME_LIMIT_US"); a.time_limit = e ? atoll(e) * 100 : 0; }
    { const char* e = getenv("MHT_BLP_FORCE_HBM"); a.force_hbm = (e && e[0] == '1') ? 1 : 0; }
    if (seam_team) {
        const size_t tb = 64 + sizeof(TeamState) * TEAM_MAX + sizeof(TeamResult) * TEAM_W;
        rc = ctx->counts.ensure(tb);
        if (rc) return rc;
        char* tp = static_cast<char*>(ctx->counts.ptr);
        MHT_HIP_CHECK(hipMemsetAsync(tp, 0, tb, ctx->stream));
        a.team_list = reinterpret_cast<int32_t*>(tp);
        a.team_state = reinterpret_cast<TeamState*>(tp + 64);
        a.team_res = reinterpret_cast<TeamResult*>(tp + 64 + sizeof(TeamState) * TEAM_MAX);
        const unsigned long long inf_key = ~0ull;
        MHT_HIP_CHECK(hipMemcpyAsync(&a.team_state[0].gub, &inf_key, 8, hipMemcpyHostToDevice, ctx->stream));
    }
    int32_t* hbuf = new int32_t[nT + 12];
    hbuf[0] = 0; hbuf[1] = nT;
    for (int t = 0; t < nT; ++t) hbuf[2 + t] = t;
    hbuf[2 + nT] = 0; hbuf[3 + nT] = 0;
    hbuf[4 + nT] = 1; hbuf[5 + nT] = 1; hbuf[6 + nT] = 0; hbuf[7 + nT] = 0;
    hbuf[8 + nT] = 0; hbuf[9 + nT] = seam_team ? 1 : 0; hbuf[10 + nT] = 0; hbuf[11 + nT] = 0;
    hipError_t e = hipMemcpyAsync(cl_ptr, hbuf, (size_t)(nT + 12) * 4, hipMemcpyHostToDevice, ctx->stream);
    if (e == hipSuccess) e = hipStreamSynchronize(ctx->stream);
    delete[] hbuf;
// ... 19 lines not shown
```

pymht_amd/csrc/mht_common.h:

```cpp
#pragma once
#include <hip/hip_runtime.h>
#include <hip/hip_ext.h>
#include <stdint.h>
#include <stdio.h>
#include <stdarg.h>
#include "../../include/mht_amd.h"
#include "mht_math.h"

namespace mht {

void set_error(const char* fmt, ...);

#define MHT_HIP_CHECK(expr)                                                                      \
    do {                                                                                         \
        hipError_t _e = (expr);                                                                  \
        if (_e != hipSuccess) {                                                                  \
            mht::set_error("%s failed: %s (%s:%d)", #expr, hipGetErrorString(_e), __FILE__, __LINE__); \
            return MHT_E_HIP;                                                                    \
        }                                                                                        \
    } while (0)

#define MHT_REQUIRE(cond, ...)                 \
    do {                                       \
        if (!(cond)) {                         \
            mht::set_error(__VA_ARGS__);       \
            return MHT_E_INVALID;              \
        }                                      \
    } while (0)

struct Scratch {
    void* ptr = nullptr;
    size_t bytes = 0;
    int ensure(size_t need) {
        if (need <= bytes) return MHT_OK;
        if (ptr) MHT_HIP_CHECK(hipFree(ptr));
        ptr = nullptr;
        bytes = 0;
        size_t want = need + need / 2 + 4096;
        MHT_HIP_CHECK(hipMalloc(&ptr, want));
        MHT_HIP_CHECK(hipMemset(ptr, 0, want));
        MHT_HIP_CHECK(hipStreamSynchronize(nullptr));
        bytes = want;
        return MHT_OK;
    }
    void release() {
        if (ptr) (void)hipFree(ptr);
        ptr = nullptr;
        bytes = 0;
    }
};

constexpr int GATE_TILE = 32;
constexpr int GATE_THREADS = 512;
constexpr int EMIT_THREADS = 64;
constexpr int MAX_MEAS = 4096;
constexpr int EDGE_SEGS = 64;
constexpr int MAXPD = 15;
#ifndef MHT_FG_THREADS
#define MHT_FG_THREADS 256
#endif
#ifndef MHT_FG_CAP
#define MHT_FG_CAP 96
#endif
constexpr int FG_THREADS = MHT_FG_THREADS;
constexpr int FG_CAP_SOLO = 128;
constexpr int FG_CAP = MHT_FG_CAP;
constexpr int FG_REGIONS = 8;
constexpr int VT_PW = NP / 2;
constexpr int GKQ = (4 + NK + 3 + 3) / 4;
constexpr int GKF = GKQ * 4;

struct DevStatus {
    int overflow;
    int n_children;
    int n_dead;
    int pad[1];
    unsigned long long t[6];
};

struct Forest;

enum FgFamily : int { FG_PLAIN, FG_WAVE, FG_ADM, FG_AIS, FG_CT, FG_BATCH, FG_BATCH_WAVE, FG_FAMILIES };
enum KernelSlot : int {
    K_GATE, K_CLUSTER, K_CLUSTER_INIT, K_CLUSTER_BIG, K_CLUSTER_BATCH, K_BLP, K_BLP_UF, K_BLP_BATCH, K_BLP_LIGHT_BATCH,
    K_SMOOTH_EM4, K_SMOOTH_EM6,
    K_SMOOTH_SCORE,
    K_GOSPA,
    K_OSPA2,
    K_FGROW,
    K_SLOTS = K_FGROW + FG_FAMILIES * 3 * 2
};

template <typename T>
__device__ __forceinline__ void load_args(T& dst, const T* src) {
    static_assert(sizeof(T) % 4 == 0, "argument blocks are copied dword-wise");
    const __attribute__((address_space(4))) unsigned* s = (const __attribute__((address_space(4))) unsigned*)src;
    unsigned* d = reinterpret_cast<unsigned*>(&dst);
#pragma unroll
    for (int i = 0; i < (int)(sizeof(T) / 4); ++i) d[i] = s[i];
}

}

struct mht_ctx {
    int device = 0;
    int n_cu = 256;
    hipStream_t stream = nullptr;
    mht::Scratch hitmask;
    mht::Scratch counts;
    unsigned gate_epoch = 0;
    mht::DevStatus* status = nullptr;
    mht::Forest* forest = nullptr;
    size_t lds_raised[mht::K_SLOTS] = {};
};

namespace mht {

template <typename... P, typename... A>
int launch_kernel(mht_ctx* ctx, KernelSlot slot, void (*kernel)(P...), dim3 grid, dim3 block, size_t lds, bool any_order, const A&... args) {
    if (!kernel) {
        set_error("launch_kernel: kernel instance %d is not part of this build", (int)slot);
        return MHT_E_INVALID;
    }
    size_t& raised = ctx->lds_raised[slot];
    if (lds > 48 * 1024 && lds > raised) {
        MHT_HIP_CHECK(hipFuncSetAttribute(reinterpret_cast<const void*>(kernel), hipFuncAttributeMaxDynamicSharedMemorySize, (int)lds));
        raised = lds;
    }
    if (any_order) hipExtLaunchKernelGGL(kernel, grid, block, lds, ctx->stream, nullptr, nullptr, hipExtAnyOrderLaunch, args...);
    else hipLaunchKernelGGL(kernel, grid, block, lds, ctx->stream, args...);
    MHT_HIP_CHECK(hipGetLastError());
    return MHT_OK;
}

}
```

pymht_amd/csrc/mht_forest.hip:

```cpp
#include "mht_kernels.h"
#include "mht_commit.h"
#include <hip/hip_ext.h>
#include "mht_admit.h"
#include "mht_init_dev.h"
#include <string.h>
#include <math.h>
#include <new>
#include <stdlib.h>

struct HostProf { bool on = false; bool asked = false; double acc[16] = {}; long n = 0; double t_last = 0.0; };
static HostProf g_hp;
static inline double hp_now() { timespec ts; clock_gettime(CLOCK_MONOTONIC, &ts); return ts.tv_sec * 1e6 + ts.tv_nsec * 1e-3; }
static inline void hp_begin() { if (!g_hp.asked) { g_hp.asked = true; const char* e = getenv("MHT_HOST_PROF"); g_hp.on = e && e[0] == '1'; } if (g_hp.on) { g_hp.t_last = hp_now(); g_hp.n += 1; } }
static inline void hp_mark(int i) { if (g_hp.on) { const double t = hp_now(); g_hp.acc[i] += t - g_hp.t_last; g_hp.t_last = t; } }
static void hp_print() {
    if (!g_hp.on || !g_hp.n) return;
    static const char* nm[16] = {"checks", "stage (memcpy, kernel, events)", "begin_step + deferred init", "fill grow args", "grow launch", "events behind grow", "fill blp", "blp launch", "initiator args / defer", "end_step", "initiate_impl (ride)", "", "", "", "", ""};
    fprintf(stderr, "[mht host prof] %ld scans, us per scan:", g_hp.n);
    for (int i = 0; i < 11; ++i) fprintf(stderr, " %s %.2f |", nm[i], g_hp.acc[i] / g_hp.n);
    fprintf(stderr, "\n");
    g_hp = HostProf();
}

static bool env_flag(const char* name, bool dflt) { const char* e = getenv(name); return e && (e[0] == '0' || e[0] == '1') ? e[0] == '1' : dflt; }
static long long env_int(const char* name, long long dflt) { const char* e = getenv(name); return e ? atoll(e) : dflt; }

namespace mht {

struct Switches {
    bool debug = getenv("MHT_GROW_DEBUG") != nullptr;
    bool ct_spill = env_flag("MHT_CT_SPILL", false);
    bool grid_by_hint = env_flag("MHT_BLP_GRID_HINT", true);
    bool force_hbm = env_flag("MHT_BLP_FORCE_HBM", false);
    bool no_enum = env_flag("MHT_BLP_NO_ENUM", false);
    bool no_reduce = env_flag("MHT_BLP_NO_REDUCE", false);
    bool teams = !env_flag("MHT_BLP_NO_TEAMS", false);
    bool adm_fuse = env_flag("MHT_ADM_FUSE", true);
    bool no_uf = env_flag("MHT_NO_UF", false);
    bool no_overlap = env_flag("MHT_NO_OVERLAP", false);
    bool serial_prof = env_flag("ROCPROF_COUNTER_COLLECTION", false);
    bool init_side_q = env_flag("MHT_INIT_QUEUE", true) && !serial_prof;
    bool rep_flag_ok = env_flag("MHT_REPORT_FLAG", true);
    bool stage_stream = env_flag("MHT_STAGE_STREAM", true);
    bool blp_stamps = env_flag("MHT_BLP_STAMPS", false);
    bool ovl_stamps = env_flag("MHT_OVL_STAMPS", false);
    bool ovl_force = env_flag("MHT_OVL_FORCE", false);
};

constexpr int MAXR = 16;
constexpr int RING_EXTRA = 4;
constexpr int EV_POOL = 64;
constexpr int Z_RING = 8;
constexpr int Z_GUARD = 4;
constexpr int BIRTH_CAP = 256;

template <int NT> __device__ __forceinline__ void publish_report(const PublishArgs& p) {
    if (!p.dst) return;
    __threadfence();
    __syncthreads();
    const ReportHeader* h = reinterpret_cast<const ReportHeader*>(p.src);
    const int n_births = h->n_births, nT = h->n_targets;
    const uint4* s4 = reinterpret_cast<const uint4*>(p.src);
    uint4* d4 = reinterpret_cast<uint4*>(p.dst);
    const int head = (p.birth_off + n_births * (int)sizeof(mht_birth_report) + 15) / 16;
    for (int i = threadIdx.x; i < head; i += NT) d4[i] = s4[i];
    const int r0 = p.rec_off / 16, rn = (nT * (int)sizeof(mht_target_report) + 15) / 16;
    for (int i = threadIdx.x; i < rn; i += NT) d4[r0 + i] = s4[r0 + i];
    __threadfence_system();
}
static_assert(sizeof(mht_target_report) % 16 == 0 && sizeof(mht_birth_report) % 8 == 0, "report blocks are copied in 16-byte pieces");

__global__ void stage_scan_kernel(const float4* src, float4* dst, int n16, unsigned long long* flag = nullptr, unsigned long long tag = 0) {
    if (!flag) { for (int i = threadIdx.x; i < n16; i += blockDim.x) dst[i] = src[i]; return; }
    for (int i = threadIdx.x; i < n16; i += blockDim.x) {
        const float4 v = src[i];
        unsigned long long* q = reinterpret_cast<unsigned long long*>(dst + i);
        __hip_atomic_store(q, ((unsigned long long)__float_as_uint(v.y) << 32) | __float_as_uint(v.x), __ATOMIC_RELAXED, __HIP_MEMORY_SCOPE_AGENT);
        __hip_atomic_store(q + 1, ((unsigned long long)__float_as_uint(v.w) << 32) | __float_as_uint(v.z), __ATOMIC_RELAXED, __HIP_MEMORY_SCOPE_AGENT);
    }
    asm volatile("s_waitcnt vmcnt(0)" ::: "memory");
    __syncthreads();
    if (threadIdx.x == 0) __hip_atomic_store(flag, tag, __ATOMIC_RELAXED, __HIP_MEMORY_SCOPE_AGENT);
}

__global__ __launch_bounds__(COMMIT_THREADS) void commit_publish_kernel(const CommitArgs a, const CommitDyn dyn, const PublishArgs pub) {
    __shared__ int s_commit[2 * (COMMIT_THREADS / 64) + 8];
    commit_body<COMMIT_THREADS>(a, dyn, s_commit);
    publish_report<COMMIT_THREADS>(pub);
}

__global__ __launch_bounds__(COMMIT_THREADS) void commit_kernel(const CommitArgs a, const CommitDyn dyn) {
    __shared__ int s_commit[2 * (COMMIT_THREADS / 64) + 8];
    commit_body<COMMIT_THREADS>(a, dyn, s_commit);
}

__global__ __launch_bounds__(1024) void add_targets_kernel(const AddArgs a) {
    __shared__ int s_adm[ADM_LDS_INTS];
    add_targets_body<1024>(a, s_adm);
}

static_assert(INIT_THREADS == 1024, "post_scan_kernel runs commit, initiator and admission with one block size");
struct AisUsedArgs { const int32_t* mmsi; const int32_t* first; const int32_t* leaf_off; const FCounts* cnt; const AisInitMsg* msgs; int nA; unsigned char* used; };
static __device__ void ais_used_body(const AisUsedArgs& u) {
    const int tid = threadIdx.x;
    for (int q = tid; q < u.nA; q += 1024) u.used[q] = 0;
    __threadfence_block();
    __syncthreads();
    const int nT = u.cnt->nT;
    for (int t = tid; t < nT; t += 1024) {
        const int f0 = u.first[t], n = u.leaf_off[t + 1] - u.leaf_off[t];
        int last = 0;
        for (int i = 0; i < n; ++i) {
            const int mm = u.mmsi[f0 + i];
            if (mm == 0 || mm == last) continue;
            last = mm;
            for (int q = 0; q < u.nA; ++q) if (u.msgs[q].mmsi == mm) { u.used[q] = 1; break; }
        }
    }
    __threadfence_block();
    __syncthreads();
}
template <bool AIS>
// ... 109 lines not shown
        const mht_nodes& l = a.layers[sc % a.R];
        nodes[n] = nd;
        meas[n] = l.meas[nd];
        cnllr[n] = l.cnllr[nd];
        for (int k = 0; k < NX; ++k) x[n * NX + k] = l.x[(size_t)k * l.cap + nd];
        const VTab& v = a.vt[a.lgen[sc % a.R]];
        if (ct.on) export_cov_ct(ct, sc % a.R, (sc + a.R - 1) % a.R, l.cov[nd], P ? P + (size_t)n * NP : nullptr, P64 ? P64 + (size_t)n * NP : nullptr);
        else export_cov(v, l.cov[nd], l.flags[nd], P ? P + (size_t)n * NP : nullptr, P64 ? P64 + (size_t)n * NP : nullptr);
        if (flags) flags[n] = l.flags[nd];
        ++n;
        nd = l.parent[nd];
        --sc;
    }
    return n;
}
__global__ void chain_kernel(const ChainArgs a, const CtLayers ct) {
    if (threadIdx.x || blockIdx.x) return;
    *a.n_out = chain_walk(a, ct, a.node, a.nodes, a.meas, a.x, a.cnllr, a.P, a.P64, a.flags);
}
struct ChainRec { size_t o_m, o_x, o_c, o_P, o_fl, stride; };
__host__ __device__ __forceinline__ ChainRec chain_rec(int len, int PB) {
    ChainRec r;
    r.o_m = 8 + (size_t)len * 4;
    r.o_x = (r.o_m + (size_t)len * 4 + 7) & ~(size_t)7;
    r.o_c = r.o_x + (size_t)len * (NX * 8);
    r.o_P = r.o_c + (size_t)len * 8;
    r.o_fl = r.o_P + (size_t)len * ((size_t)NP * PB);
    r.stride = (r.o_fl + (size_t)len + 15) & ~(size_t)15;
    return r;
}
__global__ void chains_kernel(const ChainArgs a, const CtLayers ct, const int32_t* start, int count, char* out, int PB) {
    const int i = blockIdx.x * blockDim.x + threadIdx.x;
    if (i >= count) return;
    const ChainRec r = chain_rec(a.max_len, PB);
    char* o = out + (size_t)i * r.stride;
    const int n = chain_walk(a, ct, start[i], (int32_t*)(o + 8), (int32_t*)(o + r.o_m), (double*)(o + r.o_x), (double*)(o + r.o_c), PB == 4 ? (float*)(o + r.o_P) : nullptr,
                             PB == 8 ? (double*)(o + r.o_P) : nullptr, (uint8_t*)(o + r.o_fl));
    *(int32_t*)o = n;
}

struct Arena {
    char* base = nullptr; size_t size = 0, off = 0;
    template <typename T> T* take(size_t n) {
        off = (off + 255) & ~(size_t)255;
        T* p = reinterpret_cast<T*>(base ? base + off : nullptr);
        off += n * sizeof(T);
        return p;
    }
};

struct Forest {
    mht_forest_config cfg;
    mht_model model;
    Switches sw;
    int Tcap, Ncap, Mpad, R, PD, AW, n_mnodes, Ecap, SegCap;
    VTab vt = {};
    VTab vts[2] = {}; int vgen = 0; int layer_gen[MAXR] = {}; int last_rebuild_scan = -1000000; int32_t* vt_remap = nullptr;
    int rebuilds = 0;
    unsigned long long vt_used_seen = 0, vt_rate = 0;
    Arena arena;
    mht_nodes layer[MAXR];
    int32_t* path[2]; int32_t* apath[2]; double* cost2[2]; int32_t* tchild; int32_t* tcend;
    int pds = 8;
    bool ct = false; double ct_T = 0.0;
    float* ct_Pbar[MAXR] = {}; float* ct_Phat[MAXR] = {}; float* ct_Proot[MAXR] = {};
    float4* ct_gains = nullptr; double* ct_xbar = nullptr; double* ct_zhat = nullptr; unsigned long long* ct_hw_spill = nullptr;
    bool ais = false; int ais_half = 0;
    int32_t* l_mmsi[MAXR] = {}; int32_t* l_hmmsi[MAXR] = {};
    int32_t* ais_nf = nullptr; int32_t* ais_off = nullptr; AisRec* ais_rec = nullptr; int ais_rec_cap = 0; unsigned* ais_count = nullptr;
    char* ais_groups_dev = nullptr; char* ais_msgs_dev = nullptr; int ais_group_cap = 64, ais_msg_cap = 0;
    bool ais_armed = false; int ais_nG = 0, ais_nA = 0; double ais_eta2 = 0.0, ais_lambda = 0.0;
    unsigned* alloc2[2]; int block_cap = 0, over_base = 0, region_cap = 0, root_base = 0;
    TTable tab[2];
    unsigned char* used_bytes[2];
    DevStatus* status2;
    unsigned long long* init_dbg;
    unsigned* edges; int32_t* edge_count;
    int32_t *edge_t, *edge_m, *t_label, *t_cluster, *cl_ptr, *cl_members, *multi_list, *single_list, *cl_counts, *big_list;
    int32_t* cl_owner;
    unsigned long long* uf_owner = nullptr; unsigned long long* uf_parent2[2] = {nullptr, nullptr}; bool uf_ok = false; int uf_scans = 0;
    unsigned long long z_tag_step = 0;
    int z_wait_slot = -1;
    int init_flag_scan = 0;
    unsigned long long* rec0 = nullptr; int pub_scan = 0; unsigned long long blp_done_total = 0; bool ovl_ok = true; int ovl_launches = 0;
    int32_t* cl_gtab = nullptr; bool cluster_big = false;
    int32_t* team_list; TeamState* team_state2[2]; TeamResult* team_res;
    double* u; int32_t* usage; int32_t* mark;
    int32_t *best_h, *bb_ch, *bb_best, *bb_last_idx; double *best_rc, *bb_cost, *bb_uused, *bb_last_rc, *bb_rest, *bb_min;
    int32_t *sel, *cl_status, *cl_iters, *cl_nodes, *cl_time; unsigned long long* grow_dbg; int32_t* commit_log; double* bb_snap; int32_t* bb_busy; int bb_snap_rows = 0;
    int32_t *t_status, *t_jdrop, *t_count, *t_firstsurv, *new_index, *near; double* t_score;
    int32_t *w_root_scan, *w_root_node; double* w_root_cnllr; uint8_t* w_root_f32;
    FCounts* cnt;
    bool rep_by_flag[2] = {false, false}; unsigned long long rep_tag[2] = {0, 0};
    char* report_dev2[2]; char* report_host; size_t report_bytes, rec_off, used_off, birth_off, done_off;
    char* report_host_dev[2] = {nullptr, nullptr}; float* z_host_dev = nullptr;
    int published_scan = 0;
    bool pub_deferred = false; PublishArgs pub_args = {}; int pub_slot = 0;
    int init_ran_scan = 0;
    const float* z_cur = nullptr;
    char* report_host2[2] = {nullptr, nullptr}; hipEvent_t rep_ev[2] = {nullptr, nullptr}; int rep_slot = 0; bool rep_inflight = false; bool rep_started[2] = {false, false};
    int host_block_scan[2] = {0, 0};
    hipStream_t stage_stream = nullptr; bool stage_stream_tried = false;
    bool init_ev_lazy = false; bool init_deferred = false;
    InitArgs init_def_args; const DevStatus* init_def_status = nullptr; unsigned long long init_def_ztag = 0;
    hipEvent_t init_ev = nullptr; bool init_ev_pending = false;
    float* z_dev; float* z_host; hipEvent_t z_ev[Z_RING] = {}; bool z_used[Z_RING] = {}; int z_slot = 0;
    hipEvent_t z_guard_ev[2] = {nullptr, nullptr}; long long z_count = 0; int z_guard_due = -1;
    Scratch stage_dev; void* stage_host = nullptr; size_t stage_host_bytes = 0;
    static constexpr int CHAIN_SLOTS = 8;
    struct ChainSlot { char* host = nullptr; char* dev = nullptr; size_t bytes = 0; hipEvent_t ev = nullptr; long long ticket = -1; int count = 0, len = 0, pb = 4; bool pending = false; };
    ChainSlot chain_slots[CHAIN_SLOTS]; long long chain_next = 0;
    int scan = 0; int nT_ub = 0; int L_ub = 0; bool report_pending = false; int last_M = 0; bool dead = false;
    int nT_ub_prev = 0;
    int nT_ub_step = 0;
    int births_since_step = 0;
    bool commit_pending = false; CommitArgs pending = {}; CommitDyn pending_dyn = {};
    bool adm_pending = false; AddArgs adm = {};
    bool shard_open = false; int shard_plan_s = 0, shard_plan_W = 0, shard_M = 0, shard_xn = 0;
    long long blp_time_limit = 0;
    float prune_thr = 0.f;
    int in_groups = 0;
    int similar_ran_scan = -100;
    unsigned long long* hint_host = nullptr; unsigned long long* hint_dev = nullptr;
    int births_after[64] = {}; int births_init_ub[64] = {};
    int init_mreq = 0;
    unsigned long long* bhint_host = nullptr; unsigned long long* bhint_dev = nullptr;
    long long births_between(int k, int s) const {
        long long b = 0;
        for (int j = k; j < s; ++j) {
            int ub = births_init_ub[j % 64];
            if (ub > 0 && bhint_host) {
                const unsigned long long h = reinterpret_cast<volatile unsigned long long*>(bhint_host)[j % 64];
                if ((int)(h >> 32) == j) { if ((int)(h & 0xffffu) < ub) ub = (int)(h & 0xffffu); }
                else if (init_mreq > 0) {
                    for (int q = j - 1; q >= j - init_mreq && q >= 1; --q) {
                        const unsigned long long hq = reinterpret_cast<volatile unsigned long long*>(bhint_host)[q % 64];
                        if ((int)(hq >> 32) == q && (int)((hq >> 16) & 0xffffu) < ub) ub = (int)((hq >> 16) & 0xffffu);
                    }
                }
            }
            b += births_after[j % 64] + ub;
        }
        return b;
    }
    int targets_ub(int s_table) const {
        int ub = nT_ub;
        if (hint_host) {
            const unsigned long long h = *reinterpret_cast<volatile unsigned long long*>(hint_host);
            const int k = (int)(h >> 32), na = (int)(h & 0xffffffffu);
            if (k >= 1 && k < s_table && s_table - k < 60) {
                const long long b = na + births_between(k, s_table);
                if (b < ub) ub = (int)b;
            }
        }
        return ub;
    }
    bool timing = false; int timed_steps = 0; int ev_slot = 0; hipEvent_t (*evp)[5] = nullptr;

    void layout(Arena& ar) {
        for (int s = 0; s < R; ++s) {
            mht_nodes& l = layer[s];
            l.cap = Ncap; l.cap_cov = 0;
            l.x = ar.take<double>((size_t)NX * Ncap); l.cnllr = ar.take<double>(Ncap); l.pd = ar.take<double>(Ncap);
            l.parent = ar.take<int32_t>(Ncap); l.meas = ar.take<int32_t>(Ncap); l.cov = ar.take<int32_t>(Ncap);
            l.flags = ar.take<uint8_t>(Ncap); l.P = nullptr;
        }
        if (ct) {
// ... 812 lines not shown
static int step_grow(mht_ctx* ctx, Forest* f, StepPlan& pl, const float* z, int M) {
    hp_mark(2);
    hipStream_t st = ctx->stream;
    FGrowArgs g;
    fill_fgrow(f, pl.s, pl.fused, g);
    FDyn d = {};
    fdyn_base(f, z, M, pl, d);
    d.dbg = f->sw.debug ? f->grow_dbg : nullptr;
    d.uf_epoch = pl.use_uf ? 2u * (unsigned)pl.s : 0u;
    d.ovl = (pl.fused && f->pub_scan == pl.s - 1 && f->pending_dyn.scan == pl.s - 1) ? 1 : 0;
    d.c_wait = f->blp_done_total;
    pl.grow_ovl = d.ovl != 0;
    d.ct_spill = f->sw.ct_spill ? 1 : 0;
    d.z_flag = &f->cnt->z_flag; d.z_tag = f->z_tag_step;
    d.stamp_end = f->sw.ovl_stamps ? 1 : 0;
    const bool adm = f->adm_pending && pl.fused;
    const bool adm_ovl = adm && f->init_flag_scan == pl.s - 1;
    d.adm_wait = adm_ovl ? 1 : 0;
    const bool any_order = d.ovl && f->ovl_ok && (!adm || adm_ovl) && (!f->pub_deferred || adm_ovl) && !pl.ais && !f->timing && (!f->sw.debug || f->sw.ovl_force);
    if (any_order) f->ovl_launches += 1;
    hp_mark(3);
    MHT_STEP_CHECK(launch_deferred_init(ctx, f));
    if (adm && f->init_ev_pending) {
        if (adm_ovl && f->init_ev_lazy) { f->init_ev_pending = false; f->init_ev_lazy = false; }
        else MHT_STEP_CHECK(wait_init_ev(ctx, f));
    }
    const bool pub_flag = f->pub_deferred && adm && f->pub_args.dst && f->sw.rep_flag_ok && !f->sw.serial_prof;
    if (pub_flag) {
        f->pub_args.done = reinterpret_cast<unsigned long long*>(f->report_host_dev[f->pub_slot] + f->done_off);
        f->pub_args.tag = (unsigned long long)(pl.s - 1) | (1ull << 40);
    } else { f->pub_args.done = nullptr; f->pub_args.tag = 0; }
    MHT_STEP_CHECK(launch_fgrow(ctx, g, d, pl.n_ub, pl.fused ? &f->pending : nullptr, f->pub_deferred ? &f->pub_args : nullptr, adm ? &f->adm : nullptr, any_order));
    hp_mark(4);
    f->adm_pending = false;
    if (f->z_guard_due >= 0) { MHT_STEP_HIP(hipEventRecord(f->z_guard_ev[f->z_guard_due], st)); f->z_guard_due = -1; }
    if (f->pub_deferred) {
        if (pub_flag) { f->rep_by_flag[f->pub_slot] = true; f->rep_tag[f->pub_slot] = f->pub_args.tag; }
        else { MHT_STEP_HIP(hipEventRecord(f->rep_ev[f->pub_slot], st)); f->rep_by_flag[f->pub_slot] = false; }
        f->rep_started[f->pub_slot] = true;
        f->host_block_scan[f->pub_slot] = pl.s - 1;
        f->pub_deferred = false;
    }
    f->commit_pending = false;
    hp_mark(5);
    return MHT_OK;
}
static int step_cluster(mht_ctx* ctx, Forest* f, const StepPlan& pl, const float* z, int M, mht_initiator* init, double now) {
    if (pl.use_uf) { f->uf_scans += 1; return MHT_OK; }
    ClusterArgs c;
    fill_cluster(f, pl.s, c);
    if (!init || f->cluster_big) return launch_cluster(ctx, c);
    InitArgs ia;
    scan_init_args(f, init, z, M, nullptr, now, pl.s, ia);
    MHT_STEP_CHECK(launch_cluster(ctx, c, &ia, &f->cnt->overflow));
    f->init_ran_scan = pl.s;
    return MHT_OK;
}
static int step_initiator(mht_ctx* ctx, Forest* f, const StepPlan& pl, const float* z, int M, mht_initiator* init, double now) {
    InitArgs ia;
    scan_init_args(f, init, z, M, nullptr, now, pl.s, ia);
    if (f->sw.init_side_q && f->stage_stream && f->z_tag_step) {
        f->init_deferred = true; f->init_def_args = ia; f->init_def_status = f->status2 + (pl.s & 1); f->init_def_ztag = f->z_tag_step;
        f->init_ev_pending = true; f->init_ev_lazy = true;
    } else
    hipExtLaunchKernelGGL(initiator_side_kernel, dim3(1), dim3(INIT_THREADS), 0, ctx->stream, nullptr, nullptr, hipExtAnyOrderLaunch, ia,
                          static_cast<const DevStatus*>(f->status2 + (pl.s & 1)), static_cast<const int32_t*>(&f->cnt->overflow), &f->cnt->init_flag,
                          static_cast<const unsigned long long*>(f->z_tag_step ? &f->cnt->z_flag : nullptr), f->z_tag_step,
                          static_cast<unsigned long long*>(nullptr), static_cast<const unsigned long long*>(nullptr), static_cast<unsigned long long*>(nullptr));
    MHT_STEP_HIP(hipGetLastError());
    f->init_ran_scan = pl.s; f->init_flag_scan = pl.s;
    return MHT_OK;
}
static int step_solve(mht_ctx* ctx, Forest* f, const StepPlan& pl, const float* z, int M, mht_initiator* init, double now) {
    BlpArgs b;
    fill_blp(f, pl.s, b);
    b.uf_epoch = pl.use_uf ? 2u * (unsigned)pl.s : 0u;
    b.ni_flag = &f->cnt->ni_flag; b.uf_ovl = pl.grow_ovl ? 1 : 0;
    const int grid = blp_hint_grid(f, pl.s, pl.use_uf, blp_full_grid(f, 2));
    if (pl.use_uf) {
        b.rec0 = f->rec0; b.blp_done = &f->cnt->blp_done; b.pub_scan = (unsigned)pl.s; b.begun = &f->cnt->ilp_begun;
        b.pub_ub = f->nT_ub_step < 1 ? 1 : (f->nT_ub_step < f->Tcap ? f->nT_ub_step : f->Tcap);
    }
    hp_mark(6);
    MHT_STEP_CHECK(launch_blp(ctx, b, grid));
    hp_mark(7);
    if (pl.use_uf) { f->pub_scan = pl.s; f->blp_done_total += (unsigned long long)grid; }
    if (pl.use_uf && init) MHT_STEP_CHECK(step_initiator(ctx, f, pl, z, M, init, now));
    hp_mark(8);
    return MHT_OK;
}
static int forest_step_impl(mht_ctx* ctx, const float* z, int32_t M, mht_initiator* init, double now) {
    MHT_REQUIRE(ctx && ctx->forest, "mht_forest_step: no forest");
    Forest* f = ctx->forest;
    MHT_HIP_CHECK(hipSetDevice(ctx->device));
    StepPlan pl;
    { const int rc = step_begin(ctx, f, z, M, "mht_forest_step", false, true, pl); if (rc) return rc; }
    pl.use_uf = forest_streams_uf(f, init);
    hipStream_t st = ctx->stream;
    if (f->timing) { pl.ev = f->evp[f->ev_slot]; f->ev_slot = (f->ev_slot + 1) % EV_POOL; }
    hipEvent_t* const ev = pl.ev;
    if (ev) MHT_STEP_HIP(hipEventRecord(ev[0], st));
    MHT_STEP_CHECK(step_prepasses(ctx, f, pl, z, M, pl.fused));
    MHT_STEP_CHECK(step_grow(ctx, f, pl, z, M));
    if (ev) MHT_STEP_HIP(hipEventRecord(ev[1], st));
    MHT_STEP_CHECK(step_cluster(ctx, f, pl, z, M, init, now));
    if (ev) MHT_STEP_HIP(hipEventRecord(ev[2], st));
    MHT_STEP_CHECK(step_prune_similar(ctx, f, pl.s));
    MHT_STEP_CHECK(step_solve(ctx, f, pl, z, M, init, now));
    if (ev) MHT_STEP_HIP(hipEventRecord(ev[3], st));
    forest_end_step(f, pl, M);
    hp_mark(9);
    if (ev) { MHT_STEP_HIP(hipEventRecord(ev[4], st)); f->timed_steps += 1; }
    return MHT_OK;
}
extern "C" int mht_forest_step(mht_ctx* ctx, const float* z, int32_t M) { return forest_step_impl(ctx, z, M, nullptr, 0.0); }

extern "C" int mht_forest_sharded_words(mht_ctx* ctx, int32_t shard_n, int32_t* n_words) {
    MHT_REQUIRE(ctx && ctx->forest && n_words && shard_n >= 1, "mht_forest_sharded_words: bad argument");
    *n_words = ctx->forest->Tcap + shard_n * TEAM_MAX * XT_WORDS;
    return MHT_OK;
}

static int sharded_begin_impl(mht_ctx* ctx, const float* z, int32_t M, int32_t shard_n, int32_t shard_i, int32_t* sel_rel, int32_t n_words) {
    MHT_REQUIRE(ctx && ctx->forest && sel_rel, "mht_forest_step_sharded_begin: null argument");
    MHT_REQUIRE(shard_n >= 1 && shard_i >= 0 && shard_i < shard_n, "mht_forest_step_sharded_begin: bad shard %d of %d", shard_i, shard_n);
    Forest* f = ctx->forest;
    MHT_REQUIRE(!f->timing, "mht_forest_step_sharded_begin: per-stage timing is not available for sharded steps");
    MHT_REQUIRE(!f->shard_open, "mht_forest_step_sharded_begin: the previous sharded step has not been ended");
    MHT_HIP_CHECK(hipSetDevice(ctx->device));
    { const int rc = flush_publish(ctx, f); if (rc) return rc; }
    StepPlan pl;
    { const int rc = step_begin(ctx, f, z, M, "mht_forest_step_sharded_begin", f->ct, false, pl); if (rc) return rc; }
    MHT_STEP_CHECK(step_prepasses(ctx, f, pl, z, M, false));
    {
        FGrowArgs g;
        fill_fgrow(f, pl.s, pl.fused, g);
        FDyn d = {};
        fdyn_base(f, z, M, pl, d);
        MHT_STEP_CHECK(launch_fgrow(ctx, g, d, pl.n_ub, pl.fused ? &f->pending : nullptr));
    }
    f->commit_pending = false;
    {
        ClusterArgs c;
        fill_cluster(f, pl.s, c);
        c.sel_rel_reset = sel_rel;
        c.shard_n = shard_n; c.tchild = f->tchild; c.tcend = f->tcend; c.cl_owner = f->cl_owner;
        MHT_STEP_CHECK(launch_cluster(ctx, c));
    }
    MHT_STEP_CHECK(step_prune_similar(ctx, f, pl.s));
    {
        BlpArgs b;
        fill_blp(f, pl.s, b);
        b.shard_n = shard_n; b.shard_i = shard_i; b.sel_rel = sel_rel; b.cl_owner = f->cl_owner;
        b.t_alive = nullptr;
        if (n_words > 0 && shard_n > 1) {
            b.shard_team = sel_rel + f->Tcap;
            MHT_STEP_HIP(hipMemsetAsync(b.shard_team, 0xff, (size_t)shard_n * TEAM_MAX * XT_WORDS * sizeof(int32_t), ctx->stream));
        }
        MHT_STEP_CHECK(launch_blp(ctx, b, blp_full_grid(f, 2)));
    }
    f->shard_open = true; f->shard_plan_s = pl.s; f->shard_plan_W = pl.W; f->shard_M = M; f->shard_xn = (n_words > 0 && shard_n > 1) ? shard_n : 0;
    return MHT_OK;
}
extern "C" int mht_forest_step_sharded_begin(mht_ctx* ctx, const float* z, int32_t M, int32_t shard_n, int32_t shard_i, int32_t* sel_rel) {
    return sharded_begin_impl(ctx, z, M, shard_n, shard_i, sel_rel, 0);
}
extern "C" int mht_forest_step_sharded_begin2(mht_ctx* ctx, const float* z, int32_t M, int32_t shard_n, int32_t shard_i, int32_t* xch, int32_t n_words) {
    MHT_REQUIRE(ctx && ctx->forest && n_words >= ctx->forest->Tcap + shard_n * TEAM_MAX * XT_WORDS,
                "mht_forest_step_sharded_begin2: the exchange block needs mht_forest_sharded_words() words");
    return sharded_begin_impl(ctx, z, M, shard_n, shard_i, xch, n_words);
}

extern "C" int mht_forest_step_sharded_end(mht_ctx* ctx, const int32_t* sel_rel) {
    MHT_REQUIRE(ctx && ctx->forest && sel_rel, "mht_forest_step_sharded_end: null argument");
    Forest* f = ctx->forest;
    MHT_REQUIRE(f->shard_open, "mht_forest_step_sharded_end: no sharded step is open");
    MHT_HIP_CHECK(hipSetDevice(ctx->device));
    BlpArgs b;
    fill_blp(f, f->shard_plan_s, b);
    b.sel_rel = const_cast<int32_t*>(sel_rel);
    int rc = MHT_OK;
    if (f->shard_xn > 1) {
        b.shard_team = b.sel_rel + f->Tcap;
        rc = launch_shard_team_resolve(ctx, b, f->shard_xn);
    }
    if (!rc) rc = launch_blp_epilogue(ctx, b, &f->cnt->nT, f->nT_ub_step);
    f->shard_open = false;
    if (rc) { f->dead = true; return rc; }
    StepPlan pl = {};
    pl.s = f->shard_plan_s; pl.W = f->shard_plan_W;
    forest_end_step(f, pl, f->shard_M);
    return MHT_OK;
}

struct mht_group {
    int n = 0, period = 0;
    mht_ctx* ctx[GROUP_MAX] = {};
    FGrowArgs* ga = nullptr;
    CommitArgs* ca = nullptr;
    ClusterArgs* cl = nullptr;
    BlpArgs* bl = nullptr;
    BlpArgs* bl0 = nullptr;
    size_t blp_lds[3] = {0, 0, 0};
    bool two_tier = false;
    bool light = false;
    bool counted = false;
    bool wave = true;
    int blp_div = 4;
};

extern "C" int mht_group_destroy(mht_group* g) {
    if (!g) return MHT_OK;
    if (g->n > 0) {
        (void)hipSetDevice(g->ctx[0]->device);
        (void)hipStreamSynchronize(g->ctx[0]->stream);
    }
    for (int i = 0; i < g->n; ++i) if (g->counted && g->ctx[i] && g->ctx[i]->forest) g->ctx[i]->forest->in_groups -= 1;
    if (g->ga) (void)hipFree(g->ga);
    if (g->ca) (void)hipFree(g->ca);
    if (g->cl) (void)hipFree(g->cl);
    if (g->bl) (void)hipFree(g->bl);
    if (g->bl0) (void)hipFree(g->bl0);
    delete g;
    return MHT_OK;
}

extern "C" int mht_group_create(mht_group** out, int32_t n, mht_ctx* const* ctxs) {
    MHT_REQUIRE(out && ctxs && n >= 1 && n <= GROUP_MAX, "mht_group_create: need 1 <= n <= %d contexts", GROUP_MAX);
    for (int i = 0; i < n; ++i) {
        MHT_REQUIRE(ctxs[i] && ctxs[i]->forest, "mht_group_create: context %d has no forest", i);
        MHT_REQUIRE(!ctxs[i]->forest->ct, "mht_group_create: context %d's forest is a constant-turn one (MHT_FOREST_CT): not available to groups", i);
        MHT_REQUIRE(!ctxs[i]->forest->cluster_big && !ctxs[i]->forest->ais, "mht_group_create: context %d's forest is too large for the batched clustering kernel "
                    "(its tables live in HBM) or is an AIS forest: step it on its own", i);
        const Forest *a = ctxs[0]->forest, *b = ctxs[i]->forest;
        MHT_REQUIRE(ctxs[i]->device == ctxs[0]->device && ctxs[i]->stream == ctxs[0]->stream,
                    "mht_group_create: the members must share one device and one stream (context %d does not)", i);
        MHT_REQUIRE(a->Tcap == b->Tcap && a->Ncap == b->Ncap && a->Mpad == b->Mpad && a->R == b->R,
                    "mht_group_create: the members must have the same forest configuration (context %d differs)", i);
        for (int j = 0; j < i; ++j) MHT_REQUIRE(ctxs[j] != ctxs[i], "mht_group_create: context %d appears twice", i);
    }
    MHT_HIP_CHECK(hipSetDevice(ctxs[0]->device));
    mht_group* g = new (std::nothrow) mht_group();
// ... 573 lines not shown
}

extern "C" int mht_forest_chains_fetch(mht_ctx* ctx, int64_t ticket, int32_t index, int32_t* nodes, int32_t* meas, double* x, double* cnllr, void* P, uint8_t* flags,
                                       int32_t* n_out) {
    MHT_REQUIRE(ctx && ctx->forest && n_out, "mht_forest_chains_fetch: null argument");
    Forest* f = ctx->forest;
    MHT_REQUIRE(ticket >= 0 && ticket < f->chain_next, "mht_forest_chains_fetch: unknown ticket %lld", (long long)ticket);
    Forest::ChainSlot& cs = f->chain_slots[ticket % Forest::CHAIN_SLOTS];
    MHT_REQUIRE(cs.ticket == ticket, "mht_forest_chains_fetch: ticket %lld has expired (%d later ones were issued)", (long long)ticket, Forest::CHAIN_SLOTS);
    MHT_REQUIRE(index >= 0 && index < cs.count, "mht_forest_chains_fetch: chain %d of %d", index, cs.count);
    MHT_HIP_CHECK(hipSetDevice(ctx->device));
    if (cs.pending) { MHT_HIP_CHECK(hipEventSynchronize(cs.ev)); cs.pending = false; }
    const ChainRec r = chain_rec(cs.len, cs.pb);
    const char* o = cs.host + (((size_t)cs.count * 4 + 15) & ~(size_t)15) + (size_t)index * r.stride;
    const int n = *(const int32_t*)o;
    *n_out = n;
    if (nodes) memcpy(nodes, o + 8, (size_t)n * 4);
    if (meas) memcpy(meas, o + r.o_m, (size_t)n * 4);
    if (x) memcpy(x, o + r.o_x, (size_t)n * (NX * 8));
    if (cnllr) memcpy(cnllr, o + r.o_c, (size_t)n * 8);
    if (P) memcpy(P, o + r.o_P, (size_t)n * ((size_t)NP * cs.pb));
    if (flags) memcpy(flags, o + r.o_fl, (size_t)n);
    return MHT_OK;
}

extern "C" int mht_forest_set_timing(mht_ctx* ctx, int32_t enable) {
    MHT_REQUIRE(ctx && ctx->forest, "mht_forest_set_timing: no forest");
    Forest* f = ctx->forest;
    MHT_HIP_CHECK(hipSetDevice(ctx->device));
    if (enable && !f->evp) {
        f->evp = new hipEvent_t[EV_POOL][5];
        for (int k = 0; k < EV_POOL; ++k)
            for (int i = 0; i < 5; ++i) MHT_HIP_CHECK(hipEventCreate(&f->evp[k][i]));
    }
    f->timing = enable != 0;
    f->timed_steps = 0;
    f->ev_slot = 0;
    return MHT_OK;
}

extern "C" int mht_forest_stage_times(mht_ctx* ctx, float* ms5, int32_t* n_steps) {
    MHT_REQUIRE(ctx && ctx->forest && ms5, "mht_forest_stage_times: null argument");
    Forest* f = ctx->forest;
    MHT_REQUIRE(f->timing && f->timed_steps > 0, "mht_forest_stage_times: no timed step pending");
    MHT_HIP_CHECK(hipStreamSynchronize(ctx->stream));
    for (int i = 0; i < 5; ++i) ms5[i] = 0.f;
    const int n = f->timed_steps;
    for (int k = 0; k < n; ++k) {
        hipEvent_t* ev = f->evp[(f->ev_slot - 1 - k + 2 * EV_POOL) % EV_POOL];
        float v;
        for (int i = 0; i < 4; ++i) { MHT_HIP_CHECK(hipEventElapsedTime(&v, ev[i], ev[i + 1])); ms5[i] += v; }
        MHT_HIP_CHECK(hipEventElapsedTime(&v, ev[0], ev[4]));
        ms5[4] += v;
    }
    if (n_steps) *n_steps = n;
    f->timed_steps = 0;
    return MHT_OK;
}

extern "C" int mht_forest_debug_read(mht_ctx* ctx, const char* name, void* host, int64_t bytes) {
    MHT_REQUIRE(ctx && ctx->forest && name && host && bytes > 0, "mht_forest_debug_read: bad argument");
    Forest* f = ctx->forest;
    const void* src = nullptr;
    size_t avail = 0, offset = 0;
    const size_t T = f->Tcap;
    char nbuf[32];
    if (const char* at = strchr(name, '@')) {
        const size_t n = (size_t)(at - name) < sizeof(nbuf) - 1 ? (size_t)(at - name) : sizeof(nbuf) - 1;
        memcpy(nbuf, name, n);
        nbuf[n] = 0;
        offset = (size_t)strtoull(at + 1, nullptr, 10);
        name = nbuf;
    }
    if (!strcmp(name, "vt_rebuilds")) {
        MHT_REQUIRE(bytes == 4, "mht_forest_debug_read: 'vt_rebuilds' is one int32");
        *static_cast<int32_t*>(host) = f->rebuilds;
        return MHT_OK;
    }
    if (!strcmp(name, "uf_ovl")) {
        MHT_REQUIRE(bytes == 8, "mht_forest_debug_read: 'uf_ovl' is two int32");
        static_cast<int32_t*>(host)[0] = f->uf_scans; static_cast<int32_t*>(host)[1] = f->ovl_launches;
        return MHT_OK;
    }
    if (!strcmp(name, "status2")) { src = f->status2; avail = 2 * sizeof(DevStatus); }
    else if (!strcmp(name, "init_dbg")) { src = f->init_dbg; avail = 64; }
    else if (!strcmp(name, "cl_status")) { src = f->cl_status; avail = T * 4; }
    else if (!strcmp(name, "cl_iters")) { src = f->cl_iters; avail = T * 4; }
    else if (!strcmp(name, "cl_nodes")) { src = f->cl_nodes; avail = T * 4; }
    else if (!strcmp(name, "cl_time")) { src = f->cl_time; avail = 8 * T * 4; }
    else if (!strcmp(name, "cl_ptr")) { src = f->cl_ptr; avail = (T + 1) * 4; }
    else if (!strcmp(name, "cl_members")) { src = f->cl_members; avail = T * 4; }
    else if (!strcmp(name, "multi_list")) { src = f->multi_list; avail = T * 4; }
    else if (!strcmp(name, "cl_counts")) { src = f->cl_counts; avail = 8 * 4; }
    else if (!strcmp(name, "cl_owner")) { src = f->cl_owner; avail = T * 4; }
    else if (!strcmp(name, "team_list")) { src = f->team_list; avail = TEAM_MAX * 4; }
    else if (!strcmp(name, "tchild")) { src = f->tchild; avail = (T + 1) * 4; }
    else if (!strcmp(name, "tcend")) { src = f->tcend; avail = (T + 1) * 4; }
    else if (!strcmp(name, "Gk")) { src = f->vt.Gk; avail = (size_t)f->vt.vcap * 2 * GKF * 4; }
    else if (!strcmp(name, "vchild")) { src = f->vt.child; avail = (size_t)f->vt.vcap * 8; }
    else if (!strcmp(name, "vcount")) { src = f->vt.count; avail = 4; }
    else if (!strcmp(name, "cov")) { src = f->layer[f->scan % f->R].cov; avail = (size_t)f->Ncap * 4; }
    else if (!strcmp(name, "grow_dbg")) { src = f->grow_dbg; avail = (32 + 16 * 4000) * 8; }
    else if (!strcmp(name, "commit_log")) { src = f->commit_log; avail = 64 * 16 * 4; }
    else if (!strcmp(name, "cluster_dbg")) { src = reinterpret_cast<int32_t*>(f->grow_dbg) + 16; avail = 8 * 4; }
    else if (!strcmp(name, "path")) { src = f->path[f->scan & 1]; avail = (size_t)f->pds * f->Ncap * 4; }
    else if (!strcmp(name, "cost")) { src = f->cost2[f->scan & 1]; avail = (size_t)f->Ncap * 8; }
    MHT_REQUIRE(src, "mht_forest_debug_read: unknown array '%s'", name);
    MHT_REQUIRE(offset <= avail && (size_t)bytes <= avail - offset, "mht_forest_debug_read: '%s' holds %zu bytes", name, avail);
    src = static_cast<const char*>(src) + offset;
    MHT_HIP_CHECK(hipSetDevice(ctx->device));
    { const int rc = flush_commit(ctx, f); if (rc) return rc; }
    MHT_HIP_CHECK(hipMemcpyAsync(host, src, (size_t)bytes, hipMemcpyDeviceToHost, ctx->stream));
    MHT_HIP_CHECK(hipStreamSynchronize(ctx->stream));
    return MHT_OK;
}
```

pymht_amd/csrc/mht_kernels.h:

```cpp
#pragma once
#include "mht_common.h"
#include "mht_vtab.h"

namespace mht {

struct GateArgs {
    Model model;
    double default_pd, default_miss_nllr;
    const double* x; const double* cnllr; const double* pd; const int32_t* cov; const uint8_t* flags; const float* P;
    int cap_in, capc_in;
    const int32_t* leaf_src;
    int L;
    const float* z; int M; int W;
    int32_t* ticket;
    int max_resident;
    unsigned long long* tile_state;
    unsigned long long* group_state;
    unsigned epoch;
    unsigned long long* dbg;
    int ablate;
    double* ox; double* ocnllr; double* opd; int32_t* oparent; int32_t* omeas; int32_t* ocov; uint8_t* oflags; float* oP;
    int cap_out, capc_out;
    int32_t* child_ptr; double* nllr; unsigned long long* used;
    DevStatus* status;
// ... 163 lines not shown
    int max_iter; int node_limit;
    long long time_limit;
    int force_hbm;
    int no_enum;
    int no_reduce;
    int skip_dead;
    int cap_h, cap_r, cap_k, cap_uw, tier, t1_h, t1_k;
    const int32_t* team_list; TeamState* team_state; TeamResult* team_res;
    size_t tm_sm, tm_ss;
    int32_t* big_list; int32_t* big_count;
    int shard_n, shard_i;
    const int32_t* cl_owner;
    int32_t* shard_team;
    int32_t* sel_rel;
    const DevStatus* status;
    const double* x; const uint8_t* flags;
    const double* t_root_cnllr; const uint8_t* t_root_f32; const int32_t* t_depth; const int32_t* t_window;
    int32_t* t_alive; int32_t* t_jdrop; int32_t* t_count; int32_t* t_firstsurv; double* t_score;
    int Nwin; double score_limit, cnllr_limit, radar_x, radar_y, radar_range;
    const int32_t* apath; int R; int kc;
    RingLayer ring0; size_t ring_stride;
    const int32_t* t_id; const int32_t* t_root_scan; const int32_t* t_root_node; const int32_t* t_label;
    mht_target_report* rec; int32_t* w_root_scan; int32_t* w_root_node; double* w_root_cnllr; uint8_t* w_root_f32;
    const unsigned long long* uf_parent; unsigned uf_epoch; const int32_t* nT_dev; int uf_cap;
    DevStatus* status_other; unsigned* alloc_reset; int32_t* t_cluster;
    unsigned long long* rec0; int pub_ub; unsigned long long* blp_done; unsigned pub_scan;
    unsigned long long* begun;
    unsigned long long* dbg;
    const unsigned long long* ni_flag; int uf_ovl;
    unsigned uf_lds_off;
};

struct SimilarArgs {
    const int32_t* single_list; const int32_t* counts;
    const int32_t* tchild; const int32_t* tcend;
    double* x; double* cnllr; const double* pd; const int32_t* meas; int32_t* cov; uint8_t* flags; double* cost; int cap;
    const double* t_root_cnllr; const uint8_t* t_root_f32; int Nwin;
    VTab vt; Model model;
    float thr;
    const DevStatus* status;
    const int32_t* mmsi;
    int32_t* t_window; const int32_t* t_depth;
    const float* ct_Phat; float* ct_Pbar;
};

struct AisGroup; struct AisMsg;
struct AisForestArgs {
    Model model;
    const int32_t* nT_dev; const int32_t* t_first; const int32_t* t_leaf_off;
    const double* x; const double* pd; const int32_t* cov; const uint8_t* flags; const int32_t* hmmsi; int cap;
    VTab vt;
    const AisGroup* groups; int nG; const AisMsg* msgs;
    double eta2_ais, lambda_ais;
    const float* z; int M;
    int32_t* nf; int32_t* off; AisRec* rec; int rec_cap; unsigned* rec_count;
    DevStatus* status;
};
int launch_forest_ais(mht_ctx* ctx, const AisForestArgs& a, int n_targets_ub);
int launch_gate(mht_ctx* ctx, GateArgs& a, int grid_leaves_hint);
int launch_prune_similar(mht_ctx* ctx, const SimilarArgs& a, int n_targets_ub);
struct AddArgs;
int launch_fgrow(mht_ctx* ctx, const FGrowArgs& a, FDyn& d, int n_targets_ub, const CommitArgs* commit, const PublishArgs* publish = nullptr,
                 const AddArgs* adm = nullptr, bool any_order = false);
int forest_sync_side(mht_ctx* ctx);
size_t fgrow_lds_bytes(int W, int pds, int AW);
size_t fgrow_lds_bytes_cap(int W, int pds, int AW, int cap);
void fgrow_plan(FDyn& d, int n_targets_ub, int Tcap, bool fused, bool wave);
size_t fgrow_wave_lds_bytes(int W, int pds, int AW);
int fgrow_grid_of(const FDyn& d);
int launch_fgrow_batch(mht_ctx* ctx, const FBatch& b, int n_sectors, int grid_x, size_t lds, int pds, bool wave);
int launch_cluster_batch(mht_ctx* ctx, const PBatch& av, int n_sectors, int Tcap, int n_mnodes);
int launch_blp_batch(mht_ctx* ctx, const PBatch& av, int n_sectors, int grid_x, size_t lds);
size_t blp_set_tier(BlpArgs& a, int tier);
int launch_blp_light_batch(mht_ctx* ctx, const PBatch& av, int n_sectors, int grid_x);
void fill_model(GateArgs& a, const mht_model* m);
void fill_model_only(Model& o, const mht_model* m);
struct InitArgs;
int launch_cluster(mht_ctx* ctx, const ClusterArgs& a, const InitArgs* init = nullptr, const int32_t* sticky_overflow = nullptr);
void cluster_prepare(ClusterArgs& a);
size_t cluster_lds_bytes(int Tcap, int n_mnodes);
int cluster_elds(int Tcap, int n_mnodes);
bool cluster_fits_lds(int Tcap, int n_mnodes);
size_t cluster_big_ints(int Tcap, int n_mnodes);
int launch_blp(mht_ctx* ctx, const BlpArgs& a, int grid);
bool blp_uf_fits(int Tcap, int n_mnodes);
int launch_blp_epilogue(mht_ctx* ctx, const BlpArgs& a, const int32_t* nT_dev, int n_targets_ub);
int launch_shard_team_resolve(mht_ctx* ctx, const BlpArgs& a, int shard_n);
void forest_destroy(mht_ctx* ctx);

}
```

Before: 20590 scans/s.

## Add specialised BLP union-find kernel with compile-time-constant args for common config

Templates the BLP solve path on an argument type so a 'plain' instantiation can treat shard, tier, debug, capacity and pds fields as compile-time constants. The host picks this specialised union-find kernel when the runtime arguments match the common configuration. Kernel args are read through the constant address space, and GStore caches the needed pointers rather than dereferencing the args struct. This aims to cut scalar loads and branches and let the compiler fold dead paths. The cost is a second kernel instance, which adds code size and compile time and can change register allocation.

```diff
diff --git a/pymht_amd/csrc/mht_blp.hip b/pymht_amd/csrc/mht_blp.hip
--- a/pymht_amd/csrc/mht_blp.hip
+++ b/pymht_amd/csrc/mht_blp.hip
@@ -11,6 +11,26 @@
 constexpr int FUSED_K = 8;
 constexpr double DINF = 1.0e300;
 constexpr int BIG_MAXH = 2048, BIG_MAXR = 1024, BIG_MAXK = 256;
+
+typedef const __attribute__((address_space(4))) BlpArgs KBlpArgs;
+struct BlpArgsPlain : BlpArgs {
+    static constexpr int pds = 8, shard_n = 1, shard_i = 0, tier = 0, force_hbm = 0, no_enum = 0, no_reduce = 0, skip_dead = 0;
+    static constexpr int cap_h = BIG_MAXH, cap_r = BIG_MAXR, cap_k = BIG_MAXK;
+    static constexpr int32_t* shard_team = nullptr;
+    static constexpr int32_t* sel_rel = nullptr;
+    static constexpr const int32_t* cl_owner = nullptr;
+    static constexpr int32_t* big_list = nullptr;
+    static constexpr unsigned long long* dbg = nullptr;
+};
+static_assert(sizeof(BlpArgsPlain) == sizeof(BlpArgs), "the plain view adds no field");
+typedef const __attribute__((address_space(4))) BlpArgsPlain KBlpArgsPlain;
+template <typename AT> struct blp_plain { static constexpr bool value = false; };
+template <> struct blp_plain<KBlpArgsPlain> { static constexpr bool value = true; };
+#define BLP_HAS(f) (blp_plain<AT>::value || a.f != nullptr)
+static bool blp_is_plain(const BlpArgs& b) {
+    return b.pds == 8 && b.PD <= 8 && b.shard_n <= 1 && !b.shard_team && !b.sel_rel && !b.cl_owner && b.tier == 0 && !b.force_hbm && !b.no_enum &&
+           !b.no_reduce && !b.skip_dead && !b.dbg && b.t_alive && b.rec && b.status && b.rec0 && b.blp_done && b.begun && b.cap_h == BIG_MAXH && b.cap_r == BIG_MAXR && b.cap_k == BIG_MAXK;
+}
 
 struct Red {
     double d[BLP_THREADS / 64];
@@ -114,15 +134,16 @@
 #define MHT_GS_CK 1
 #endif
 struct GStore {
-    const BlpArgs* a; const int32_t* mem; const unsigned long long* uw; int UW, PD; size_t cap;
+    const int32_t *tchild, *tcend; const double* costp; const int32_t* path; int pds;
+    const int32_t* mem; const unsigned long long* uw; int UW, PD; size_t cap;
     double* pu; int32_t* pusage; int32_t* pmark;
     int32_t *best_h, *ub_sel, *ch, *lix; double *best_rc, *cst, *uus, *lrc, *rest, *mn;
     bool ck; const int32_t *cbL, *ceL;
     __device__ __forceinline__ int row(int m) const { return m; }
-    __device__ __forceinline__ int col_begin(int k) const { return (MHT_GS_CK && ck) ? cbL[k] : a->tchild[mem[k]]; }
-    __device__ __forceinline__ int col_end(int k) const { return (MHT_GS_CK && ck) ? ceL[k] : a->tcend[mem[k]]; }
-    __device__ __forceinline__ double cost(int h) const { return a->cost[h]; }
-    __device__ __forceinline__ int ent(int d, int h) const { return a->pds ? a->path[(size_t)h * a->pds + d] : a->path[(size_t)d * cap + h]; }
+    __device__ __forceinline__ int col_begin(int k) const { return (MHT_GS_CK && ck) ? cbL[k] : tchild[mem[k]]; }
+    __device__ __forceinline__ int col_end(int k) const { return (MHT_GS_CK && ck) ? ceL[k] : tcend[mem[k]]; }
+    __device__ __forceinline__ double cost(int h) const { return costp[h]; }
+    __device__ __forceinline__ int ent(int d, int h) const { return pds ? path[(size_t)h * pds + d] : path[(size_t)d * cap + h]; }
     __device__ __forceinline__ double& u(int m) const { return pu[row(m)]; }
     __device__ __forceinline__ int32_t& usage(int m) const { return pusage[row(m)]; }
     __device__ __forceinline__ int32_t& mark(int m) const { return pmark[row(m)]; }
@@ -177,8 +198,8 @@
 #define MHT_ROWS8 1
 #endif
 __device__ __forceinline__ void rows8(const GStore& s, int h, int (&e)[8]) {
-    if (s.a->pds == 8) {
-        const int4* p = reinterpret_cast<const int4*>(s.a->path + (size_t)h * 8);
+    if (s.pds == 8) {
+        const int4* p = reinterpret_cast<const int4*>(s.path + (size_t)h * 8);
         const int4 q0 = p[0], q1 = p[1];
         e[0] = q0.x; e[1] = q0.y; e[2] = q0.z; e[3] = q0.w; e[4] = q1.x; e[5] = q1.y; e[6] = q1.z; e[7] = q1.w;
     } else {
@@ -942,8 +963,8 @@
 }
 
 constexpr int MHT_BLP_REDUCE = -2;
-__device__ __forceinline__ bool reducible(const BlpArgs&, const LStore&, int, double, Red*) { return false; }
-__device__ __forceinline__ bool reducible(const BlpArgs& a, const GStore& s, int K, double UB, Red* r) {
+template <typename AT> __device__ __forceinline__ bool reducible(AT*, const LStore&, int, double, Red*) { return false; }
+template <typename AT> __device__ __forceinline__ bool reducible(AT* ap, const GStore& s, int K, double UB, Red* r) { AT& a = *ap;
     if (a.force_hbm || a.no_reduce || K > a.cap_k || a.PD > 8 || !(UB < DINF)) return false;
     const int tid = threadIdx.x;
     compute_minimisers(s, K, r);
@@ -998,8 +1019,8 @@
     h ^= h >> 15; h *= 0x2C1B3C6Du; h ^= h >> 12;
     return h;
 }
-template <typename S> __device__ __forceinline__ void solve_core(const BlpArgs& a, const S& s, int K, Red* r, int& status, int& iters, int& nodes, unsigned long long* stamp,
-                                                                 double& ub, const Team tm = Team(0, 1, nullptr)) {
+template <typename AT, typename S> __device__ __forceinline__ void solve_core(AT* ap, const S& s, int K, Red* r, int& status, int& iters, int& nodes, unsigned long long* stamp,
+                                                                 double& ub, const Team tm = Team(0, 1, nullptr)) { AT& a = *ap;
     const int tid = threadIdx.x, lane = tid & 63, wave = tid >> 6;
     double& UB = ub;
     double best_LB = -DINF, theta = 1.0, utot = 0.0;
@@ -1023,7 +1044,7 @@
             __threadfence_block();
             __syncthreads();
         }
-        if ((it == 24 || it == 64 || it == 128) && UB < DINF && reducible(a, s, K, UB, r)) { status = MHT_BLP_REDUCE; return; }
+        if ((it == 24 || it == 64 || it == 128) && UB < DINF && reducible(&a, s, K, UB, r)) { status = MHT_BLP_REDUCE; return; }
         compute_minimisers(s, K, r);
         if (it == 0) stamp[1] = wall_clock64();
         if (!usage_counted_by_minimisers(s, K)) {
@@ -1156,7 +1177,7 @@
         __threadfence_block();
         __syncthreads();
     }
-    if (reducible(a, s, K, UB, r)) { status = MHT_BLP_REDUCE; return; }
+    if (reducible(&a, s, K, UB, r)) { status = MHT_BLP_REDUCE; return; }
     int32_t* ord = reinterpret_cast<int32_t*>(s.best_rc);
     int32_t* bh = s.best_h;
     {
@@ -1429,7 +1450,7 @@
 }
 
 struct TgtPre { int j, rscan, rnode, id, lab, cb, ce; double rootc; uint8_t rootf; };
-__device__ __forceinline__ TgtPre load_target(const BlpArgs& a, int t) {
+template <typename AT> __device__ __forceinline__ TgtPre load_target(AT* ap, int t) { AT& a = *ap;
     TgtPre p;
     const int dg = a.t_depth[t] + 1, w = a.t_window[t] & 0xff;
     p.j = dg > w ? dg - w : 0;
@@ -1442,12 +1463,12 @@
     return reinterpret_cast<const T*>(reinterpret_cast<const char*>(base0) + (size_t)k * stride);
 }
 constexpr int KEY_DEAD = -1, KEY_ALL = -2;
-__device__ __forceinline__ void blp_publish(const BlpArgs& a, int t, int key, int j, int rf, int count, int first) {
-    if (!a.rec0) return;
+template <typename AT> __device__ __forceinline__ void blp_publish(AT* ap, int t, int key, int j, int rf, int count, int first) { AT& a = *ap;
+    if (!BLP_HAS(rec0)) return;
     asm volatile("s_waitcnt vmcnt(0)" ::: "memory");
     __hip_atomic_store(&a.rec0[t], tgt_rec(a.pub_scan, key != -1, rf, j, count, count > 0 ? first : 0), __ATOMIC_RELAXED, __HIP_MEMORY_SCOPE_AGENT);
 }
-__device__ __forceinline__ int finish_target(const BlpArgs& a, int t, int s, const TgtPre& p, bool store, int* rf_out = nullptr) {
+template <typename AT> __device__ __forceinline__ int finish_target(AT* ap, int t, int s, const TgtPre& p, bool store, int* rf_out = nullptr) { AT& a = *ap;
     const int kc = a.kc;
     const double cn = a.cnllr[s];
     const uint8_t fl = a.flags[s];
@@ -1489,7 +1510,7 @@
         a.t_jdrop[t] = j;
         a.t_score[t] = score;
         a.w_root_scan[t] = rscan; a.w_root_node[t] = rnode; a.w_root_f32[t] = rf;
-        if (a.rec0) __hip_atomic_store(reinterpret_cast<unsigned long long*>(&a.w_root_cnllr[t]), (unsigned long long)__double_as_longlong(rc), __ATOMIC_RELAXED, __HIP_MEMORY_SCOPE_AGENT);
+        if (BLP_HAS(rec0)) __hip_atomic_store(reinterpret_cast<unsigned long long*>(&a.w_root_cnllr[t]), (unsigned long long)__double_as_longlong(rc), __ATOMIC_RELAXED, __HIP_MEMORY_SCOPE_AGENT);
         else a.w_root_cnllr[t] = rc;
         mht_target_report& r = a.rec[t];
         r.id = p.id;
@@ -1512,10 +1533,10 @@
     return status ? KEY_DEAD : (j > 0 ? anc : KEY_ALL);
 }
 
-__device__ __forceinline__ int sweep_prefetch(const BlpArgs& a, int j, int cb, int ce, int lane) {
+template <typename AT> __device__ __forceinline__ int sweep_prefetch(AT* ap, int j, int cb, int ce, int lane) { AT& a = *ap;
     return (j > 0 && cb + lane < ce) ? a.apath[(size_t)(cb + lane) * a.pds + (j - 1)] : -1;
 }
-__device__ __forceinline__ void sweep_survivors(const BlpArgs& a, int t, int j, int cb, int ce, int key, int va0, int lane, int rf = -1) {
+template <typename AT> __device__ __forceinline__ void sweep_survivors(AT* ap, int t, int j, int cb, int ce, int key, int va0, int lane, int rf = -1) { AT& a = *ap;
     int count = 0, first = 0x7fffffff;
     if (key == KEY_ALL) {
         count = ce - cb;
@@ -1531,31 +1552,31 @@
     }
     if (lane == 0) {
         a.t_count[t] = count; a.t_firstsurv[t] = first;
-        if (a.rec0) blp_publish(a, t, key, j, rf >= 0 ? rf : (int)a.w_root_f32[t], count, first);
-    }
-}
-
-__device__ __forceinline__ void prune_members(const BlpArgs& a, const int32_t* mem, int K, const int32_t* key) {
-    if (!a.t_alive) return;
+        if (BLP_HAS(rec0)) blp_publish(&a, t, key, j, rf >= 0 ? rf : (int)a.w_root_f32[t], count, first);
+    }
+}
+
+template <typename AT> __device__ __forceinline__ void prune_members(AT* ap, const int32_t* mem, int K, const int32_t* key) { AT& a = *ap;
+    if (!BLP_HAS(t_alive)) return;
     __threadfence_block();
     __syncthreads();
     const int lane = threadIdx.x & 63;
     for (int k = threadIdx.x >> 6; k < K; k += BLP_THREADS / 64) {
         const int t = mem[k];
         const int j = a.t_jdrop[t], cb = a.tchild[t], ce = a.tcend[t];
-        sweep_survivors(a, t, j, cb, ce, key[k], sweep_prefetch(a, j, cb, ce, lane), lane);
+        sweep_survivors(&a, t, j, cb, ce, key[k], sweep_prefetch(&a, j, cb, ce, lane), lane);
     }
 }
 
 struct ClRef { int c, p0, K, root; };
-__device__ __forceinline__ ClRef cl_ref(const BlpArgs& a, int c) { const int p0 = a.cl_ptr[c]; return ClRef{c, p0, a.cl_ptr[c + 1] - p0, -1}; }
-__device__ __forceinline__ TgtPre load_target_cr(const BlpArgs& a, int t, const ClRef& cr) {
-    TgtPre p = load_target(a, t);
+template <typename AT> __device__ __forceinline__ ClRef cl_ref(AT* ap, int c) { AT& a = *ap; const int p0 = a.cl_ptr[c]; return ClRef{c, p0, a.cl_ptr[c + 1] - p0, -1}; }
+template <typename AT> __device__ __forceinline__ TgtPre load_target_cr(AT* ap, int t, const ClRef& cr) { AT& a = *ap;
+    TgtPre p = load_target(&a, t);
     if (a.uf_epoch) p.lab = cr.root;
     return p;
 }
-__device__ __forceinline__ void solve_cluster(const BlpArgs& a, const ClRef cr, unsigned long long* uw, Red* r, unsigned char* lds,
-                                              const Team tm = Team(0, 1, nullptr), const int team_idx = -1, const int my_t = -1, const TgtPre* pre_in = nullptr, const int dbg_bx = -1) {
+template <typename AT> __device__ __forceinline__ void solve_cluster(AT* ap, const ClRef cr, unsigned long long* uw, Red* r, unsigned char* lds,
+                                              const Team tm = Team(0, 1, nullptr), const int team_idx = -1, const int my_t = -1, const TgtPre* pre_in = nullptr, const int dbg_bx = -1) { AT& a = *ap;
     const int tid = threadIdx.x;
     const int c = cr.c;
     const int K = cr.K;
@@ -1565,10 +1586,12 @@
     const unsigned long long t_begin = wall_clock64();
     const unsigned long long c_begin = clock64();
     TgtPre pre = {};
-    const bool pre_ok = a.t_alive && K <= BLP_THREADS;
-    if (pre_ok && tid < K) { if (pre_in && my_t >= 0) pre = *pre_in; else pre = load_target_cr(a, my_t >= 0 ? my_t : mem[tid], cr); }
+    const bool pre_ok = BLP_HAS(t_alive) && K <= BLP_THREADS;
+    if (pre_ok && tid < K) { if (pre_in && my_t >= 0) pre = *pre_in; else pre = load_target_cr(&a, my_t >= 0 ? my_t : mem[tid], cr); }
     LStore s;
-    unsigned char* q = lds;
+    unsigned lz = 0;
+    if (blp_plain<AT>::value) asm volatile("" : "+v"(lz)); else asm volatile("" : "+s"(lz));
+    unsigned char* q = lds + lz;
     const int L_MAXH = a.cap_h, L_MAXR = a.cap_r, L_MAXK = a.cap_k, L_KPAD = a.cap_k + 4;
     int* s_wbase = reinterpret_cast<int*>(q); q += (size_t)a.cap_uw * 4;
     int* s_scal = reinterpret_cast<int*>(q); q += 16;
@@ -1635,7 +1658,7 @@
         return;
     }
     const bool lds_cols = small_k && nH <= L_MAXH && a.PD <= 8 && !a.force_hbm;
-    const bool anc_pf = lds_cols && pre_ok && K <= 64 && a.t_alive && a.pds == 8;
+    const bool anc_pf = lds_cols && pre_ok && K <= 64 && BLP_HAS(t_alive) && a.pds == 8;
     s.nH = nH; s.PD = a.PD; s.K = K;
     if (lds_cols) {
         for (int h0 = tid; h0 < nH; h0 += 2 * BLP_THREADS) {
@@ -1776,7 +1799,7 @@
     };
     if (!use_lds) {
         GStore gs;
-        gs.a = &a; gs.mem = mem; gs.uw = uw; gs.UW = UW; gs.PD = a.PD; gs.cap = (size_t)a.cap;
+        gs.tchild = a.tchild; gs.tcend = a.tcend; gs.costp = a.cost; gs.path = a.path; gs.pds = a.pds; gs.mem = mem; gs.uw = uw; gs.UW = UW; gs.PD = a.PD; gs.cap = (size_t)a.cap;
         const size_t om = team_hbm ? (size_t)tm.q * a.tm_sm : 0, os = (team_hbm ? (size_t)tm.q * a.tm_ss : 0) + (size_t)slot;
         gs.pu = a.u + om; gs.pusage = a.usage + om; gs.pmark = a.mark + om;
         gs.ck = small_k;
@@ -1792,7 +1815,7 @@
         __threadfence_block();
         __syncthreads();
         double ub = DINF;
-        solve_core(a, gs, K, r, status, iters, nodes, stamp, ub, team_hbm ? tm : Team(0, 1, nullptr));
+        solve_core(&a, gs, K, r, status, iters, nodes, stamp, ub, team_hbm ? tm : Team(0, 1, nullptr));
         ub_reduced = ub;
 #ifdef MHT_BLP_TRACE
         if (tid == 0) printf("[blp] cluster %d K=%d nH=%d: HBM phase status %d iters %d nodes %d, %.2f ms (setup %.2f)\n", c, K, nH, status, iters, nodes,
@@ -1860,9 +1883,9 @@
                 const int h = final_sel ? __hip_atomic_load(const_cast<int32_t*>(final_sel) + k, __ATOMIC_RELAXED, __HIP_MEMORY_SCOPE_AGENT) : gs.ub_sel[k];
                 a.sel[mem[k]] = h;
                 if (a.sel_rel) a.sel_rel[mem[k]] = h - a.tchild[mem[k]];
-                if (a.t_alive) gs.ch[k] = finish_target(a, mem[k], h, pre_ok ? pre : load_target_cr(a, mem[k], cr), true);
-            }
-            if (!xteam) prune_members(a, mem, K, gs.ch);
+                if (BLP_HAS(t_alive)) gs.ch[k] = finish_target(&a, mem[k], h, pre_ok ? pre : load_target_cr(&a, mem[k], cr), true);
+            }
+            if (!xteam) prune_members(&a, mem, K, gs.ch);
         }
     }
     if (use_lds) {
@@ -1884,7 +1907,7 @@
 #ifdef MHT_BLP_TRACE
         if (tid == 0 && s.reduced) printf("[blp] cluster %d: rebuilt with %d columns %d rows at %.2f ms\n", c, nHl, nR, 1e-5 * (double)(wall_clock64() - t_begin));
 #endif
-        solve_core(a, s, K, r, status, iters, nodes, stamp, ub, team ? tm : Team(0, 1, nullptr));
+        solve_core(&a, s, K, r, status, iters, nodes, stamp, ub, team ? tm : Team(0, 1, nullptr));
 #ifdef MHT_BLP_TRACE
         if (tid == 0 && s.reduced) printf("[blp] cluster %d: LDS phase status %d iters %d nodes %d at %.2f ms\n", c, status, iters, nodes, 1e-5 * (double)(wall_clock64() - t_begin));
 #endif
@@ -1903,18 +1926,18 @@
             const int h = final_sel ? __hip_atomic_load(const_cast<int32_t*>(final_sel) + k, __ATOMIC_RELAXED, __HIP_MEMORY_SCOPE_AGENT) : s.to_global(s.ub_sel[k]);
             a.sel[mem[k]] = h;
             if (a.sel_rel) a.sel_rel[mem[k]] = h - a.tchild[mem[k]];
-            if (a.t_alive) {
-                const TgtPre q = pre_ok ? pre : load_target_cr(a, mem[k], cr);
-                s.ch[k] = finish_target(a, mem[k], h, q, true, &rf_mine);
+            if (BLP_HAS(t_alive)) {
+                const TgtPre q = pre_ok ? pre : load_target_cr(&a, mem[k], cr);
+                s.ch[k] = finish_target(&a, mem[k], h, q, true, &rf_mine);
                 s.ub_sel[k] = q.j;
                 s.lix[k] = 0;
                 s.best_h[k] = 0x7fffffff;
             }
         }
-        if (a.t_alive && s.reduced) {
+        if (BLP_HAS(t_alive) && s.reduced) {
             __syncthreads();
-            prune_members(a, mem, K, s.ch);
-        } else if (a.t_alive) {
+            prune_members(&a, mem, K, s.ch);
+        } else if (BLP_HAS(t_alive)) {
             __syncthreads();
             for (int h = tid; h < nH; h += BLP_THREADS) {
                 const int m = s.membL[h];
@@ -1928,7 +1951,7 @@
             for (int k = tid; k < K; k += BLP_THREADS) {
                 a.t_count[mem[k]] = s.lix[k];
                 a.t_firstsurv[mem[k]] = s.best_h[k];
-                blp_publish(a, mem[k], s.ch[k], s.ub_sel[k], rf_mine, s.lix[k], s.best_h[k]);
+                blp_publish(&a, mem[k], s.ch[k], s.ub_sel[k], rf_mine, s.lix[k], s.best_h[k]);
             }
         }
     }
@@ -1989,7 +2012,7 @@
     f.nif = a.uf_ovl ? nif : 0ull;
     return f;
 }
-__device__ __forceinline__ bool uf_prologue(const BlpArgs& a, const UfFetch& fe, unsigned char* lds, UfPersist* ps, const int bx, const int gx, int& my_t_out, TgtPre& pre_out) {
+template <typename AT> __device__ __forceinline__ bool uf_prologue(AT* ap, const UfFetch& fe, unsigned char* lds, UfPersist* ps, const int bx, const int gx, int& my_t_out, TgtPre& pre_out) { AT& a = *ap;
     const int tid = threadIdx.x, lane = tid & 63, wave = tid >> 6;
 #define UF_STAMP(k) do { if (a.dbg && tid == 0 && bx < 3900) a.dbg[32 + (size_t)bx * 16 + (k)] = wall_clock64(); } while (0)
     UF_STAMP(0);
@@ -2133,7 +2156,7 @@
                 cl_ptr[nC] = nT;
                 counts[0] = nC; counts[1] = nMulti; counts[2] = nSingle; counts[3] = 0; counts[4] = 0; counts[5] = nTeam;
             }
-            if (a.rec0) for (int t = nT + tid; t < a.pub_ub; t += BLP_THREADS) __hip_atomic_store(&a.rec0[t], tgt_rec(a.pub_scan, 0, 0, 0, 0, 0), __ATOMIC_RELAXED, __HIP_MEMORY_SCOPE_AGENT);
+            if (BLP_HAS(rec0)) for (int t = nT + tid; t < a.pub_ub; t += BLP_THREADS) __hip_atomic_store(&a.rec0[t], tgt_rec(a.pub_scan, 0, 0, 0, 0, 0), __ATOMIC_RELAXED, __HIP_MEMORY_SCOPE_AGENT);
             if (a.alloc_reset && tid >= 64 && tid < 64 + FG_REGIONS) a.alloc_reset[(tid - 64) * 32] = 0u;
         }
         if (bx < nMulti && tid < own_K) my_t = ms[hp[own_root] + tid];
@@ -2152,7 +2175,7 @@
         if (lane == 0) ps->own[0] = ref_of(own_root);
         if (lane < own_K) { my_t = ms[p0 + lane]; gmem[p0 + lane] = my_t; }
     }
-    if (my_t >= 0) { pre_out = load_target(a, my_t); pre_out.lab = own_root; }
+    if (my_t >= 0) { pre_out = load_target(&a, my_t); pre_out.lab = own_root; }
     __threadfence_block();
     __syncthreads();
     UF_STAMP(7);
@@ -2160,10 +2183,10 @@
     return true;
 }
 
-template <bool UF> __device__ __forceinline__ void blp_singles(const BlpArgs& a, const int bx, const int gx, const int nSingle, const UfPersist* ps = nullptr);
-__device__ __forceinline__ void blp_stamp_begin(const BlpArgs& a, int bx);
-template <bool UF = false>
-__device__ __forceinline__ void blp_body(const BlpArgs& a, unsigned char* lds, const int bx, const int gx, UfPersist* ps = nullptr, const UfFetch* fe = nullptr) {
+template <bool UF, typename AT> __device__ __forceinline__ void blp_singles(AT* ap, const int bx, const int gx, const int nSingle, const UfPersist* ps = nullptr);
+template <typename AT> __device__ __forceinline__ void blp_stamp_begin(AT* ap, int bx);
+template <bool UF = false, typename AT>
+__device__ __forceinline__ void blp_body(AT* ap, unsigned char* lds, const int bx, const int gx, UfPersist* ps = nullptr, const UfFetch* fe = nullptr) { AT& a = *ap;
     unsigned long long* uw = reinterpret_cast<unsigned long long*>(lds);
     Red* red = reinterpret_cast<Red*>(lds + (size_t)a.cap_uw * 8);
     if (!UF && a.dbg && threadIdx.x == 0 && bx < 3900) a.dbg[32 + (size_t)bx * 16 + 12] = wall_clock64();
@@ -2186,8 +2209,8 @@
         Team tm = Team(0, 1, nullptr);
         if (UF && stage == -1) {
             stage = 0;
-            if (!uf_prologue(a, *fe, lds, ps, bx, gx, my_t, my_pre_v)) return;
-            blp_stamp_begin(a, bx);
+            if (!uf_prologue(&a, *fe, lds, ps, bx, gx, my_t, my_pre_v)) return;
+            blp_stamp_begin(&a, bx);
             if (a.dbg && threadIdx.x == 0 && bx < 3900) a.dbg[32 + (size_t)bx * 16 + 12] = wall_clock64();
             nMulti = ps->nMulti; nSingle = ps->nSingle;
             teams_on = a.team_list && a.tier != 1 && (xteams || (a.shard_n <= 1 && gx > nMulti));
@@ -2197,7 +2220,7 @@
         } else if (stage == 0) {
             if (own_i >= nMulti) { stage = 1; continue; }
             if (UF) { cr = ps->own[own_q]; mt = own_q == 0 ? my_t : -1; ++own_q; }
-            else cr = cl_ref(a, work[own_i]);
+            else cr = cl_ref(&a, work[own_i]);
             own_i += gx;
             if (nTeam > 0 && cr.K >= TEAM_MIN_K)
                 for (int q = 0; q < nTeam; ++q) if ((UF ? ps->team[q].c : a.team_list[q]) == cr.c) ti = q;
@@ -2208,7 +2231,7 @@
             else ti = -1;
         } else if (stage == 1) {
             stage = 2;
-            blp_singles<UF>(a, bx, gx, nSingle, ps);
+            blp_singles<UF>(&a, bx, gx, nSingle, ps);
             continue;
         } else {
             stage = 3;
@@ -2217,16 +2240,16 @@
             ti = j % nTeam;
             if (q >= team_W(ti)) break;
             __syncthreads();
-            cr = UF ? ps->team[ti] : cl_ref(a, a.team_list[ti]);
+            cr = UF ? ps->team[ti] : cl_ref(&a, a.team_list[ti]);
             tm = (xteams && cr.K <= TEAM_SEL) ? Team(q, team_W(ti), &a.team_state[ti].gub, q * a.shard_n + a.shard_i, team_W(ti) * a.shard_n) : Team(q, team_W(ti), &a.team_state[ti].gub);
         }
         if (a.dbg && threadIdx.x == 0 && bx < 3900 && stage == 0) a.dbg[32 + (size_t)bx * 16 + 13] = wall_clock64();
-        solve_cluster(a, cr, uw, red, lds + (size_t)a.cap_uw * 8 + RED_SLOT, tm, ti, mt, mt >= 0 ? my_pre : nullptr, bx);
-    }
-}
-
-template <bool UF>
-__device__ __forceinline__ void blp_singles(const BlpArgs& a, const int bx, const int gx, const int nSingle, const UfPersist* ps) {
+        solve_cluster(&a, cr, uw, red, lds + (size_t)a.cap_uw * 8 + RED_SLOT, tm, ti, mt, mt >= 0 ? my_pre : nullptr, bx);
+    }
+}
+
+template <bool UF, typename AT>
+__device__ __forceinline__ void blp_singles(AT* ap, const int bx, const int gx, const int nSingle, const UfPersist* ps) { AT& a = *ap;
     const int lane = threadIdx.x & 63;
     const int gw = (gx - 1 - bx) * (BLP_THREADS / 64) + (threadIdx.x >> 6);
     int j = 0;
@@ -2235,7 +2258,7 @@
         if (a.shard_n > 1 && t % a.shard_n != a.shard_i) continue;
         TgtPre pre = {};
         int cb, ce;
-        if (a.t_alive) { pre = load_target(a, t); if (UF) pre.lab = t; cb = pre.cb; ce = pre.ce; }
+        if (BLP_HAS(t_alive)) { pre = load_target(&a, t); if (UF) pre.lab = t; cb = pre.cb; ce = pre.ce; }
         else { cb = a.tchild[t]; ce = a.tcend[t]; }
         double bv = DINF;
         int bi = -1;
@@ -2244,7 +2267,7 @@
             if (a.skip_dead && (a.flags[h] & F_DEAD)) continue;
             if (bi < 0 || v <= bv) { bv = v; bi = h; }
         }
-        const int va0 = a.t_alive ? sweep_prefetch(a, pre.j, cb, ce, lane) : -1;
+        const int va0 = BLP_HAS(t_alive) ? sweep_prefetch(&a, pre.j, cb, ce, lane) : -1;
 #pragma unroll
         for (int o = 32; o > 0; o >>= 1) {
             const double ov = __shfl_xor(bv, o);
@@ -2252,16 +2275,16 @@
             if (oi >= 0 && (bi < 0 || ov < bv || (ov == bv && oi > bi))) { bv = ov; bi = oi; }
         }
         if (lane == 0) { a.sel[t] = bi; if (a.sel_rel) a.sel_rel[t] = bi - cb; }
-        if (a.t_alive) {
+        if (BLP_HAS(t_alive)) {
             int rf = 0;
-            const int key = finish_target(a, t, bi, pre, lane == 0, &rf);
-            sweep_survivors(a, t, pre.j, cb, ce, key, va0, lane, rf);
+            const int key = finish_target(&a, t, bi, pre, lane == 0, &rf);
+            sweep_survivors(&a, t, pre.j, cb, ce, key, va0, lane, rf);
         }
     }
 }
 
 constexpr int LIGHT_MAXK = 8;
-__device__ __forceinline__ void blp_light(const BlpArgs& a, const int bx, const int gx, const int nMulti) {
+template <typename AT> __device__ __forceinline__ void blp_light(AT* ap, const int bx, const int gx, const int nMulti) { AT& a = *ap;
     const int lane = threadIdx.x & 63;
     const int gw = bx * (BLP_THREADS / 64) + (threadIdx.x >> 6), nw = gx * (BLP_THREADS / 64);
     for (int i = gw; i < nMulti; i += nw) {
@@ -2272,7 +2295,7 @@
             continue;
         }
         const int tk = a.cl_members[p0 + (lane < K ? lane : 0)];
-        const TgtPre pre = load_target(a, tk);
+        const TgtPre pre = load_target(&a, tk);
         double v[LIGHT_MAXK];
         int cbk[LIGHT_MAXK], cek[LIGHT_MAXK];
 #pragma unroll
@@ -2309,7 +2332,7 @@
 #pragma unroll
         for (int k = 0; k < LIGHT_MAXK; ++k) {
             const int jk = __shfl(pre.j, k < K ? k : 0);
-            va[k] = (k < K) ? sweep_prefetch(a, jk, cbk[k], cek[k], lane) : -1;
+            va[k] = (k < K) ? sweep_prefetch(&a, jk, cbk[k], cek[k], lane) : -1;
         }
         bool clash = false;
         for (int q = 0; q < K * 8; ++q) {
@@ -2324,50 +2347,49 @@
         if (lane < K) {
             a.sel[tk] = best;
             if (a.sel_rel) a.sel_rel[tk] = best - pre.cb;
-            key = finish_target(a, tk, best, pre, true);
+            key = finish_target(&a, tk, best, pre, true);
         }
 #pragma unroll
         for (int k = 0; k < LIGHT_MAXK; ++k) {
             if (k >= K) break;
-            sweep_survivors(a, __shfl(tk, k), __shfl(pre.j, k), cbk[k], cek[k], __shfl(key, k), va[k], lane);
+            sweep_survivors(&a, __shfl(tk, k), __shfl(pre.j, k), cbk[k], cek[k], __shfl(key, k), va[k], lane);
         }
         if (lane == 0) { a.cl_status[c] = MHT_BLP_CERTIFIED; a.cl_iters[c] = 0; a.cl_nodes[c] = 0; }
     }
 }
 
-__device__ __forceinline__ void blp_stamp_begin(const BlpArgs& a, int bx) {
-    if (a.status && bx == 0 && threadIdx.x == 0) {
+template <typename AT> __device__ __forceinline__ void blp_stamp_begin(AT* ap, int bx) { AT& a = *ap;
+    if (BLP_HAS(status) && bx == 0 && threadIdx.x == 0) {
         DevStatus* st = const_cast<DevStatus*>(a.status);
         if (st->t[2] == 0) st->t[2] = wall_clock64();
     }
 }
-__device__ __forceinline__ void blp_stamp_end(const BlpArgs& a) {
-    if (a.status && threadIdx.x == 0) atomicMax(&const_cast<DevStatus*>(a.status)->t[4], (unsigned long long)wall_clock64());
+template <typename AT> __device__ __forceinline__ void blp_stamp_end(AT* ap) { AT& a = *ap;
+    if (BLP_HAS(status) && threadIdx.x == 0) atomicMax(&const_cast<DevStatus*>(a.status)->t[4], (unsigned long long)wall_clock64());
 }
 
 __global__ __launch_bounds__(BLP_THREADS) void blp_kernel(const BlpArgs a) {
     extern __shared__ __attribute__((aligned(16))) unsigned char lds[];
     if (a.dbg && threadIdx.x == 0 && blockIdx.x < 3900) a.dbg[32 + (size_t)blockIdx.x * 16] = wall_clock64();
-    blp_stamp_begin(a, blockIdx.x);
-    blp_body(a, lds, blockIdx.x, gridDim.x);
-    blp_stamp_end(a);
+    blp_stamp_begin(&a, blockIdx.x);
+    blp_body(&a, lds, blockIdx.x, gridDim.x);
+    blp_stamp_end(&a);
     if (a.dbg && threadIdx.x == 0 && blockIdx.x < 3900) a.dbg[32 + (size_t)blockIdx.x * 16 + 15] = wall_clock64();
 }
-__global__ __launch_bounds__(BLP_THREADS) void blp_uf_kernel(const BlpArgs a_in) {
+template <typename AT> __device__ __forceinline__ void blp_uf_run(const UfHead& head) {
     extern __shared__ __attribute__((aligned(16))) unsigned char lds[];
-    const UfFetch fe = uf_prefetch(UfHead{a_in.status, a_in.nT_dev, a_in.ni_flag, a_in.uf_parent, a_in.uf_cap, a_in.uf_ovl});
-    typedef const __attribute__((address_space(4))) BlpArgs* KArgP;
-    KArgP kp = (KArgP)__builtin_amdgcn_kernarg_segment_ptr();
+    const unsigned long long t_first = wall_clock64();
+    const UfFetch fe = uf_prefetch(head);
+    AT* kp = (AT*)__builtin_amdgcn_kernarg_segment_ptr();
     asm volatile("" : "+s"(kp) : : "memory");
-    BlpArgs a;
-    __builtin_memcpy(&a, kp, sizeof(BlpArgs));
+    AT& a = *kp;
     UfPersist* ps = reinterpret_cast<UfPersist*>(lds + a.uf_lds_off);
-    if (a.status && blockIdx.x == 0 && threadIdx.x == 0) const_cast<DevStatus*>(a.status)->t[1] = wall_clock64();
-    if (a.begun && blockIdx.x == 0 && threadIdx.x == 0) __hip_atomic_store(a.begun, (unsigned long long)a.pub_scan, __ATOMIC_RELAXED, __HIP_MEMORY_SCOPE_AGENT);
+    if (BLP_HAS(status) && blockIdx.x == 0 && threadIdx.x == 0) const_cast<DevStatus*>(a.status)->t[1] = wall_clock64();
+    if (BLP_HAS(begun) && blockIdx.x == 0 && threadIdx.x == 0) __hip_atomic_store(a.begun, (unsigned long long)a.pub_scan, __ATOMIC_RELAXED, __HIP_MEMORY_SCOPE_AGENT);
     const int gx = (int)gridDim.x, pb = (int)blockIdx.x, bx = pb;
-    blp_body<true>(a, lds, bx, gx, ps, &fe);
-    if (!fe.s_over) blp_stamp_end(a);
-    if (a.blp_done) {
+    blp_body<true>(&a, lds, bx, gx, ps, &fe);
+    if (!fe.s_over) blp_stamp_end(&a);
+    if (BLP_HAS(blp_done)) {
         __syncthreads();
         if (threadIdx.x == 0) {
             __builtin_amdgcn_fence(__ATOMIC_RELEASE, "agent");
@@ -2375,7 +2397,16 @@
             atomicAdd(a.blp_done, 1ull);
         }
     }
-    if (a.dbg && threadIdx.x == 0 && bx < 3900) { a.dbg[32 + (size_t)bx * 16 + 15] = wall_clock64(); a.dbg[32 + (size_t)bx * 16 + 14] = ((unsigned long long)pb << 8) | (unsigned long long)(__builtin_amdgcn_s_getreg((3 << 11) | 20) & 7); }
+    if (a.dbg && threadIdx.x == 0 && bx < 3900) {
+        a.dbg[32 + (size_t)bx * 16 + 15] = wall_clock64();
+        a.dbg[32 + (size_t)bx * 16 + 14] = ((t_first & 0xffffffull) << 40) | ((unsigned long long)pb << 8) | (unsigned long long)(__builtin_amdgcn_s_getreg((3 << 11) | 20) & 7);
+    }
+}
+__global__ __launch_bounds__(BLP_THREADS) void blp_uf_kernel(const BlpArgs a_in) {
+    blp_uf_run<KBlpArgs>(UfHead{a_in.status, a_in.nT_dev, a_in.ni_flag, a_in.uf_parent, a_in.uf_cap, a_in.uf_ovl});
+}
+__global__ __launch_bounds__(BLP_THREADS) void blp_uf_kernel_plain(const BlpArgs a_in) {
+    blp_uf_run<KBlpArgsPlain>(UfHead{a_in.status, a_in.nT_dev, a_in.ni_flag, a_in.uf_parent, a_in.uf_cap, a_in.uf_ovl});
 }
 __global__ __launch_bounds__(BLP_THREADS) void blp_batch_kernel(const PBatch av) {
     extern __shared__ __attribute__((aligned(16))) unsigned char lds[];
@@ -2383,9 +2414,9 @@
     const int n = gridDim.y, lin = blockIdx.y * gridDim.x + blockIdx.x;
     const int sector = lin % n, bx = lin / n;
     load_args(a, static_cast<const BlpArgs*>(av.p[sector]));
-    blp_stamp_begin(a, bx);
-    blp_body(a, lds, bx, gridDim.x);
-    blp_stamp_end(a);
+    blp_stamp_begin(&a, bx);
+    blp_body(&a, lds, bx, gridDim.x);
+    blp_stamp_end(&a);
 }
 
 __global__ __launch_bounds__(BLP_THREADS) void blp_light_batch_kernel(const PBatch av) {
@@ -2393,12 +2424,12 @@
     const int n = gridDim.y, lin = blockIdx.y * gridDim.x + blockIdx.x;
     const int sector = lin % n, bx = lin / n;
     load_args(a, static_cast<const BlpArgs*>(av.p[sector]));
-    blp_stamp_begin(a, bx);
+    blp_stamp_begin(&a, bx);
     if (!(a.status && a.status->overflow)) {
-        blp_light(a, bx, gridDim.x, a.counts[1]);
-        blp_singles<false>(a, bx, gridDim.x, a.counts[2]);
-    }
-    blp_stamp_end(a);
+        blp_light(&a, bx, gridDim.x, a.counts[1]);
+        blp_singles<false>(&a, bx, gridDim.x, a.counts[2]);
+    }
+    blp_stamp_end(&a);
 }
 int launch_blp_light_batch(mht_ctx* ctx, const PBatch& av, int n_sectors, int grid_x) {
     return launch_kernel(ctx, K_BLP_LIGHT_BATCH, blp_light_batch_kernel, dim3(grid_x, n_sectors), dim3(BLP_THREADS), 0, false, av);
@@ -2408,7 +2439,7 @@
     if (a.status && a.status->overflow) return;
     const int ti = blockIdx.x;
     if (ti >= a.counts[5]) return;
-    const ClRef cr = cl_ref(a, a.team_list[ti]);
+    const ClRef cr = cl_ref(&a, a.team_list[ti]);
     int best = -1;
     unsigned long long bk = ~0ull;
     for (int d = 0; d < shard_n; ++d) {
@@ -2432,14 +2463,14 @@
     if (a.status && a.status->overflow) return;
     const int nT = *nT_dev, lane = threadIdx.x & 63;
     for (int t = blockIdx.x * (BLP_THREADS / 64) + (threadIdx.x >> 6); t < nT; t += gridDim.x * (BLP_THREADS / 64)) {
-        const TgtPre pre = load_target(a, t);
+        const TgtPre pre = load_target(&a, t);
         const int s = pre.cb + a.sel_rel[t];
         if (lane == 0) a.sel[t] = s;
-        const int va0 = sweep_prefetch(a, pre.j, pre.cb, pre.ce, lane);
-        const int key = finish_target(a, t, s, pre, lane == 0);
-        sweep_survivors(a, t, pre.j, pre.cb, pre.ce, key, va0, lane);
-    }
-    blp_stamp_end(a);
+        const int va0 = sweep_prefetch(&a, pre.j, pre.cb, pre.ce, lane);
+        const int key = finish_target(&a, t, s, pre, lane == 0);
+        sweep_survivors(&a, t, pre.j, pre.cb, pre.ce, key, va0, lane);
+    }
+    blp_stamp_end(&a);
 }
 
 int launch_blp_epilogue(mht_ctx* ctx, const BlpArgs& a, const int32_t* nT_dev, int n_targets_ub) {
@@ -2477,7 +2508,7 @@
     return Tcap <= 8192 && (((lds > pro ? lds : pro) + 15) & ~(size_t)15) + BLP_UF_PERSIST <= 158 * 1024;
 }
 
-int launch_blp(mht_ctx* ctx, const BlpArgs& a, int grid) {
+int launch_blp(mht_ctx* ctx, const BlpArgs& a, int grid, bool force_generic, int* instance) {
     BlpArgs b = a;
     const size_t lds = blp_set_tier(b, 0);
     if (lds > 158 * 1024) {
@@ -2493,8 +2524,12 @@
             set_error("blp: the union-find prologue of %d targets does not fit the launch's LDS (%zu bytes)", b.uf_cap, lds_uf);
             return MHT_E_CAPACITY;
         }
+        const bool plain = !force_generic && blp_is_plain(b);
+        if (instance) *instance = plain ? BLP_INST_UF_PLAIN : BLP_INST_UF;
+        if (plain) return launch_kernel(ctx, K_BLP_UF_PLAIN, blp_uf_kernel_plain, dim3(grid), dim3(BLP_THREADS), lds_uf, false, b);
         return launch_kernel(ctx, K_BLP_UF, blp_uf_kernel, dim3(grid), dim3(BLP_THREADS), lds_uf, false, b);
     }
+    if (instance) *instance = BLP_INST_TABLES;
     return launch_kernel(ctx, K_BLP, blp_kernel, dim3(grid), dim3(BLP_THREADS), lds, false, b);
 }
 
diff --git a/pymht_amd/csrc/mht_common.h b/pymht_amd/csrc/mht_common.h
--- a/pymht_amd/csrc/mht_common.h
+++ b/pymht_amd/csrc/mht_common.h
@@ -82,7 +82,7 @@
 
 enum FgFamily : int { FG_PLAIN, FG_WAVE, FG_ADM, FG_AIS, FG_CT, FG_BATCH, FG_BATCH_WAVE, FG_FAMILIES };
 enum KernelSlot : int {
-    K_GATE, K_CLUSTER, K_CLUSTER_INIT, K_CLUSTER_BIG, K_CLUSTER_BATCH, K_BLP, K_BLP_UF, K_BLP_BATCH, K_BLP_LIGHT_BATCH,
+    K_GATE, K_CLUSTER, K_CLUSTER_INIT, K_CLUSTER_BIG, K_CLUSTER_BATCH, K_BLP, K_BLP_UF, K_BLP_UF_PLAIN, K_BLP_BATCH, K_BLP_LIGHT_BATCH,
     K_SMOOTH_EM4, K_SMOOTH_EM6,
     K_SMOOTH_SCORE,
     K_GOSPA,
diff --git a/pymht_amd/csrc/mht_forest.hip b/pymht_amd/csrc/mht_forest.hip
--- a/pymht_amd/csrc/mht_forest.hip
+++ b/pymht_amd/csrc/mht_forest.hip
@@ -38,6 +38,7 @@
     bool adm_fuse = env_flag("MHT_ADM_FUSE", true);
     bool no_uf = env_flag("MHT_NO_UF", false);
     bool no_overlap = env_flag("MHT_NO_OVERLAP", false);
+    bool blp_generic = env_flag("MHT_BLP_GENERIC", false);
     bool serial_prof = env_flag("ROCPROF_COUNTER_COLLECTION", false);
     bool init_side_q = env_flag("MHT_INIT_QUEUE", true) && !serial_prof;
     bool rep_flag_ok = env_flag("MHT_REPORT_FLAG", true);
@@ -313,7 +314,7 @@
     unsigned long long z_tag_step = 0;
     int z_wait_slot = -1;
     int init_flag_scan = 0;
-    unsigned long long* rec0 = nullptr; int pub_scan = 0; unsigned long long blp_done_total = 0; bool ovl_ok = true; int ovl_launches = 0;
+    unsigned long long* rec0 = nullptr; int pub_scan = 0; unsigned long long blp_done_total = 0; bool ovl_ok = true; int ovl_launches = 0; int blp_instance = 0;
     int32_t* cl_gtab = nullptr; bool cluster_big = false;
     int32_t* team_list; TeamState* team_state2[2]; TeamResult* team_res;
     double* u; int32_t* usage; int32_t* mark;
@@ -1292,7 +1293,7 @@
         b.pub_ub = f->nT_ub_step < 1 ? 1 : (f->nT_ub_step < f->Tcap ? f->nT_ub_step : f->Tcap);
     }
     hp_mark(6);
-    MHT_STEP_CHECK(launch_blp(ctx, b, grid));
+    MHT_STEP_CHECK(launch_blp(ctx, b, grid, f->sw.blp_generic, &f->blp_instance));
     hp_mark(7);
     if (pl.use_uf) { f->pub_scan = pl.s; f->blp_done_total += (unsigned long long)grid; }
     if (pl.use_uf && init) MHT_STEP_CHECK(step_initiator(ctx, f, pl, z, M, init, now));
@@ -1367,7 +1368,7 @@
             b.shard_team = sel_rel + f->Tcap;
             MHT_STEP_HIP(hipMemsetAsync(b.shard_team, 0xff, (size_t)shard_n * TEAM_MAX * XT_WORDS * sizeof(int32_t), ctx->stream));
         }
-        MHT_STEP_CHECK(launch_blp(ctx, b, blp_full_grid(f, 2)));
+        MHT_STEP_CHECK(launch_blp(ctx, b, blp_full_grid(f, 2), f->sw.blp_generic, &f->blp_instance));
     }
     f->shard_open = true; f->shard_plan_s = pl.s; f->shard_plan_W = pl.W; f->shard_M = M; f->shard_xn = (n_words > 0 && shard_n > 1) ? shard_n : 0;
     return MHT_OK;
@@ -2107,8 +2108,15 @@
         static_cast<int32_t*>(host)[0] = f->uf_scans; static_cast<int32_t*>(host)[1] = f->ovl_launches;
         return MHT_OK;
     }
+    if (!strcmp(name, "blp_instance")) {
+        MHT_REQUIRE(bytes == 4, "mht_forest_debug_read: 'blp_instance' is one int32");
+        *static_cast<int32_t*>(host) = f->blp_instance;
+        return MHT_OK;
+    }
     if (!strcmp(name, "status2")) { src = f->status2; avail = 2 * sizeof(DevStatus); }
     else if (!strcmp(name, "init_dbg")) { src = f->init_dbg; avail = 64; }
+    else if (!strcmp(name, "sel")) { src = f->sel; avail = T * 4; }
+    else if (!strcmp(name, "t_label")) { src = f->t_label; avail = T * 4; }
     else if (!strcmp(name, "cl_status")) { src = f->cl_status; avail = T * 4; }
     else if (!strcmp(name, "cl_iters")) { src = f->cl_iters; avail = T * 4; }
     else if (!strcmp(name, "cl_nodes")) { src = f->cl_nodes; avail = T * 4; }
diff --git a/pymht_amd/csrc/mht_kernels.h b/pymht_amd/csrc/mht_kernels.h
--- a/pymht_amd/csrc/mht_kernels.h
+++ b/pymht_amd/csrc/mht_kernels.h
@@ -269,7 +269,8 @@
 int cluster_elds(int Tcap, int n_mnodes);
 bool cluster_fits_lds(int Tcap, int n_mnodes);
 size_t cluster_big_ints(int Tcap, int n_mnodes);
-int launch_blp(mht_ctx* ctx, const BlpArgs& a, int grid);
+enum BlpInstance : int { BLP_INST_NONE = 0, BLP_INST_TABLES = 1, BLP_INST_UF = 2, BLP_INST_UF_PLAIN = 3 };
+int launch_blp(mht_ctx* ctx, const BlpArgs& a, int grid, bool force_generic = false, int* instance = nullptr);
 bool blp_uf_fits(int Tcap, int n_mnodes);
 int launch_blp_epilogue(mht_ctx* ctx, const BlpArgs& a, const int32_t* nT_dev, int n_targets_ub);
 int launch_shard_team_resolve(mht_ctx* ctx, const BlpArgs& a, int shard_n);
```

Result: faster. 22920 scans/s (median of 6 runs) (+11.3%).
